# gutiKristian/VolumeRendering

Hardware: AMD Instinct MI355X
Metric: Gsamples/s (higher is better)
Workload: dtype f32

## Files before the change

include/vr.h:

```cpp
#ifndef VR_H_
#define VR_H_

#include <stdint.h>
#include <stddef.h>

#ifdef __cplusplus
extern "C" {
#endif

#define VR_ABI_VERSION 1

typedef enum vr_status {
    VR_OK = 0,
    VR_ERR_INVALID_ARG = -1,
    VR_ERR_HIP = -2,
    VR_ERR_NOT_READY = -3,
    VR_ERR_UNSUPPORTED = -4,
    VR_ERR_OOM = -5
} vr_status;

typedef enum vr_variant {
    VR_VARIANT_BASIC = 0,
    VR_VARIANT_LIGHT = 1,
    VR_VARIANT_VOLUME_MASK = 2,
    VR_VARIANT_THREE_FILES = 3,
    VR_VARIANT_MULTI_CTRT = 4,
    VR_VARIANT_TF_CALIB = 5,
    VR_VARIANT_ILLUSTRATIVE = 6,
    VR_VARIANT_LIGHT_INSHADER = 7,
    VR_VARIANT_MIP = 8,
    VR_VARIANT_MINIP = 9,
    VR_VARIANT_AVERAGE = 10,
    VR_VARIANT_ISO = 11,
    VR_VARIANT_COUNT = 12
} vr_variant;

#define VR_MAX_VOLUMES 3
#define VR_MAX_TFS 2


typedef struct vr_uniforms {
    float model[16];
    float view[16];
    float proj[16];
    float view_inv[16];
    float proj_inv[16];
    float camera_pos[3];
    int32_t fragment_mode;
    int32_t steps_count;
    float step_size;
    float clip_x[2];
    float clip_y[2];
    float clip_z[2];
    int32_t toggles[4];
    float light_pos[4];
    float light_ambient[4];
    float light_diffuse[4];
} vr_uniforms;

typedef struct vr_ctx vr_ctx;


int vr_create(vr_ctx** out, uint32_t width, uint32_t height, int device_id);

int vr_resize(vr_ctx* ctx, uint32_t width, uint32_t height);

void vr_destroy(vr_ctx* ctx);

const char* vr_last_error(const vr_ctx* ctx);

int vr_abi_version(void);


int vr_volume_upload(vr_ctx* ctx, int slot, const float* vec4_voxels, uint16_t nx, uint16_t ny, uint16_t nz);

int vr_volume_upload_device(vr_ctx* ctx, int slot, const void* d_vec4_voxels, uint16_t nx, uint16_t ny, uint16_t nz);

int vr_volume_upload_raw16(vr_ctx* ctx, int slot, const uint16_t* raw, uint16_t nx, uint16_t ny, uint16_t nz);
int vr_volume_upload_raw32(vr_ctx* ctx, int slot, const uint32_t* raw, uint16_t nx, uint16_t ny, uint16_t nz);
int vr_volume_normalize(vr_ctx* ctx, int slot, int normalization_value, int* used_value);
int vr_volume_precompute_gradient(vr_ctx* ctx, int slot, int norm_to_zero_one);
int vr_volume_download(vr_ctx* ctx, int slot, float* vec4_voxels);

int vr_tf_upload(vr_ctx* ctx, int slot, const float* opacity, const float* color_rgba, uint32_t resolution);

int vr_tf_upload_opacity(vr_ctx* ctx, int slot, const float* opacity, uint32_t resolution);
int vr_tf_upload_color(vr_ctx* ctx, int slot, const float* color_rgba, uint32_t resolution);

int vr_tf_upload_opacity_async(vr_ctx* ctx, int slot, const float* opacity, uint32_t resolution, void* stream);
int vr_tf_upload_color_async(vr_ctx* ctx, int slot, const float* color_rgba, uint32_t resolution, void* stream);

int vr_set_uniforms(vr_ctx* ctx, const vr_uniforms* u);


int vr_render(vr_ctx* ctx, int variant);

int vr_render_tiles(vr_ctx* ctx, int variant, int rank, int world);
int vr_tile_count(const vr_ctx* ctx, int rank, int world);

int vr_render_async(vr_ctx* ctx, int variant, void* d_frame, void* stream);

void* vr_stream(vr_ctx* ctx, int index);

int vr_hint_frames_in_flight(vr_ctx* ctx, int frames);
int vr_render_tiles_async(vr_ctx* ctx, int variant, int rank, int world, void* d_tiles, void* stream);

int vr_unpack_tiles_async(vr_ctx* ctx, const void* d_gathered, int world, void* d_frame, void* stream);

int vr_render_batch_async(vr_ctx* ctx, int variant, int n_frames, const vr_uniforms* uniforms, void* const* d_frames, void* stream);
int vr_render_tiles_batch_async(vr_ctx* ctx, int variant, int rank, int world, int n_frames, const vr_uniforms* uniforms,
                                void* const* d_tiles, void* stream);

int vr_unpack_tiles_strided_async(vr_ctx* ctx, const void* d_gathered, int world, int rank_stride_tiles, void* d_frame, void* stream);

int vr_download(vr_ctx* ctx, float* frag_rgba, uint8_t* present_bgra8, uint64_t* composited_samples);

int vr_present_async(vr_ctx* ctx, const void* d_frame, void* d_bgra8, void* stream);

int vr_present_tiles_async(vr_ctx* ctx, const void* d_gathered, int world, int rank_stride_tiles, void* d_bgra8, void* stream);

int vr_present_packed_async(vr_ctx* ctx, const void* d_tiles_rgba, int n_tiles, void* d_tiles_bgra8, void* stream);
int vr_unpack_tiles_bgra8_async(vr_ctx* ctx, const void* d_gathered_bgra8, int world, int rank_stride_tiles, void* d_bgra8, void* stream);

int vr_download_tiles(vr_ctx* ctx, float* tiles_rgba, uint64_t* composited_samples);


int vr_last_timing(vr_ctx* ctx, float* kernel_ms, float* total_ms);

int vr_kernel_times(vr_ctx* ctx, float* out_ms, int capacity);

#define VR_TIMING_RECORDS 0
#define VR_TIMING_EVENTS 1
int vr_set_kernel_timing(vr_ctx* ctx, int mode);
int vr_reset_kernel_times(vr_ctx* ctx);

int vr_viewport(const vr_ctx* ctx, uint32_t* width, uint32_t* height, int* device_id);

void* vr_frame_device_ptr(vr_ctx* ctx);

int vr_last_covered_pixels(vr_ctx* ctx, uint64_t* covered);

int vr_last_counters(vr_ctx* ctx, uint64_t out[3]);

int vr_last_block_trace(vr_ctx* ctx, uint64_t* out, int capacity);

int vr_set_kernel_flavour(vr_ctx* ctx, int flavour);

int vr_kernel_choice(vr_ctx* ctx, int flavours[6], float ms_per_launch[6], int* chosen);

#define VR_ARITH_SEPARATE 0
#define VR_ARITH_FUSED 1
int vr_set_arithmetic(vr_ctx* ctx, int mode);

int vr_set_iso_value(vr_ctx* ctx, float iso);

int vr_set_shadows(vr_ctx* ctx, int grid_divisor, float opacity_scale);

int vr_shadow_volume(vr_ctx* ctx, float* out, size_t capacity, int dims[3]);

int vr_set_volume_layout(vr_ctx* ctx, int mode);
int vr_volume_layout(vr_ctx* ctx, int slot, int* flags);

int vr_last_kernel_flavour(vr_ctx* ctx);

int vr_skip_field(vr_ctx* ctx, int variant, uint8_t* dist, size_t capacity, int dims[3], int box[6], uint64_t* active);

int64_t vr_unbounded_box_launches(vr_ctx* ctx);

#ifdef __cplusplus
}
#endif
#endif
```

volumerendering_amd/build.py:

```python
from __future__ import annotations

import os
import shutil
import subprocess

HERE = os.path.dirname(os.path.abspath(__file__))
CSRC = os.path.join(HERE, "csrc")
HIPCC = shutil.which("hipcc") or "/opt/rocm/bin/hipcc"

HIP_ARCH = os.environ.get("VR_HIP_ARCH", "gfx950:xnack-")
HIP_FLAGS = ["-O3", "--offload-arch=" + HIP_ARCH, "-ffp-contract=off", "-fno-fast-math", "-fPIC", "-shared",
             "-std=c++17", "-Wall", "-Wno-unused-function"]
HOST_FLAGS = ["-O2", "-std=c++20", "-fPIC", "-shared", "-ffp-contract=off", "-fno-fast-math", "-Wall"]


def _newer(target: str, sources: list[str]) -> bool:
    if not os.path.exists(target):
        return True
    t = os.path.getmtime(target)
    return any(os.path.getmtime(s) > t for s in sources)


def _sources(d: str, exts: tuple[str, ...]) -> list[str]:
    out = []
    for dp, _, fs in os.walk(d):
        out += [os.path.join(dp, f) for f in fs if f.endswith(exts)]
    return sorted(out)


def build_hip(force: bool = False) -> str:
    target = os.path.join(HERE, "libvr_hip.so")
    hdrs = [os.path.join(CSRC, f) for f in ("vr_kernels.h", "vr_dp.h", "vr_pw.h", "vr_p2.h", "vr_lt.h", "vr_proj.h", "vr_iso.h", "vr_shadow.h", "vr_device.h", "vr_launch.h")]
    hdrs.append(os.path.join(os.path.dirname(HERE), "include", "vr.h"))
    flags = [f for f in HIP_FLAGS if f != "-shared"] + os.environ.get("VR_EXTRA_HIPCC_FLAGS", "").split()
    stamp = os.path.join(CSRC, ".build_flags")
    want = " ".join(flags)
    if not os.path.exists(stamp) or open(stamp).read() != want:
        force = True
    objs, procs = [], []
    for name in ("vr_api", "vr_fused"):
        src, obj = os.path.join(CSRC, name + ".hip"), os.path.join(CSRC, name + ".o")
        objs.append(obj)
        if force or _newer(obj, hdrs + [src]):
            procs.append((name, subprocess.Popen([HIPCC, *flags, "-c", "-o", obj, src])))
    for name, pr in procs:
        if pr.wait() != 0:
            raise subprocess.CalledProcessError(pr.returncode, f"hipcc {name}.hip")
    if procs or force or _newer(target, objs):
        subprocess.run([HIPCC, "--offload-arch=" + HIP_ARCH, "-fPIC", "-shared", "-o", target, *objs], check=True)
    with open(stamp, "w") as fh:
        fh.write(want)
    return target


def build_host(force: bool = False) -> str | None:
    hostdir = os.path.join(CSRC, "host")
    cpps = _sources(hostdir, (".cpp",))
    if not cpps:
        return None
    target = os.path.join(HERE, "libvr_host.so")
    deps = _sources(hostdir, (".cpp", ".h")) + [os.path.join(os.path.dirname(HERE), "include", "vr.h")]
    if force or _newer(target, deps):
        subprocess.run(["g++", *HOST_FLAGS, "-I", os.path.join(os.path.dirname(HERE), "include"), "-o", target, *cpps,
                        "-L", HERE, "-lvr_hip", "-Wl,-rpath,$ORIGIN"], check=True)
    return target


def build_mgpu(force: bool = False) -> str:
    target = os.path.join(HERE, "libvr_mgpu.so")
    src = os.path.join(CSRC, "mgpu", "vr_mgpu.cpp")
    inc = os.path.join(os.path.dirname(HERE), "include")
    deps = [src, os.path.join(inc, "vr_mgpu.h"), os.path.join(inc, "vr.h")]
    rocm = os.environ.get("ROCM_PATH", "/opt/rocm")
    if force or _newer(target, deps):
        subprocess.run(["g++", "-O2", "-std=c++17", "-fPIC", "-shared", "-Wall", "-D__HIP_PLATFORM_AMD__", "-I", inc,
                        "-I", os.path.join(rocm, "include"), "-o", target, src, "-L", HERE, "-lvr_hip",
                        "-L", os.path.join(rocm, "lib"), "-lamdhip64", "-lrccl",
                        "-Wl,-rpath,$ORIGIN", "-Wl,-rpath," + os.path.join(rocm, "lib")], check=True)
    return target


def build_all(force: bool = False):
    build_hip(force)
    build_host(force)
    build_mgpu(force)
```

volumerendering_amd/capi.py:

```python
from __future__ import annotations

import ctypes as C
import os

import numpy as np

_HERE = os.path.dirname(os.path.abspath(__file__))
LIB_PATH = os.path.join(_HERE, "libvr_hip.so")

VR_OK = 0
VR_ERR_INVALID_ARG = -1
VR_ERR_HIP = -2
VR_ERR_NOT_READY = -3
VR_ERR_UNSUPPORTED = -4
VR_ERR_OOM = -5

BASIC, LIGHT, VOLUME_MASK, THREE_FILES, MULTI_CTRT, TF_CALIB, ILLUSTRATIVE, LIGHT_INSHADER = range(8)
MIP, MINIP, AVERAGE = 8, 9, 10
ISO = 11
VARIANT_NAMES = ["BASIC", "LIGHT", "VOLUME_MASK", "THREE_FILES", "MULTI_CTRT", "TF_CALIB", "ILLUSTRATIVE", "LIGHT_INSHADER",
                 "MIP", "MINIP", "AVERAGE", "ISO"]
TILE = 64
ARITH_SEPARATE, ARITH_FUSED = 0, 1

ABI_SYMBOLS = [
    "vr_create", "vr_resize", "vr_destroy", "vr_last_error", "vr_abi_version", "vr_volume_upload",
    "vr_volume_upload_device", "vr_volume_upload_raw16", "vr_volume_upload_raw32", "vr_volume_normalize",
    "vr_volume_precompute_gradient", "vr_volume_download", "vr_tf_upload", "vr_tf_upload_opacity", "vr_tf_upload_color", "vr_set_uniforms", "vr_render", "vr_render_tiles", "vr_tile_count",
    "vr_render_async", "vr_render_tiles_async", "vr_unpack_tiles_async", "vr_download", "vr_download_tiles",
    "vr_render_batch_async", "vr_render_tiles_batch_async", "vr_unpack_tiles_strided_async",
    "vr_last_timing", "vr_kernel_times", "vr_reset_kernel_times", "vr_frame_device_ptr", "vr_last_covered_pixels", "vr_last_counters", "vr_set_kernel_flavour", "vr_last_block_trace", "vr_last_kernel_flavour",
    "vr_set_volume_layout", "vr_volume_layout", "vr_viewport", "vr_set_arithmetic", "vr_present_async", "vr_stream", "vr_hint_frames_in_flight",
    "vr_set_kernel_timing", "vr_present_tiles_async", "vr_kernel_choice",
    "vr_present_packed_async", "vr_unpack_tiles_bgra8_async",
    "vr_tf_upload_opacity_async", "vr_tf_upload_color_async", "vr_skip_field", "vr_unbounded_box_launches",
    "vr_set_iso_value", "vr_set_shadows", "vr_shadow_volume",
]


class Uniforms(C.Structure):
    _fields_ = [
        ("model", C.c_float * 16), ("view", C.c_float * 16), ("proj", C.c_float * 16),
        ("view_inv", C.c_float * 16), ("proj_inv", C.c_float * 16),
        ("camera_pos", C.c_float * 3),
        ("fragment_mode", C.c_int32), ("steps_count", C.c_int32), ("step_size", C.c_float),
        ("clip_x", C.c_float * 2), ("clip_y", C.c_float * 2), ("clip_z", C.c_float * 2),
        ("toggles", C.c_int32 * 4),
        ("light_pos", C.c_float * 4), ("light_ambient", C.c_float * 4), ("light_diffuse", C.c_float * 4),
    ]


class VrError(RuntimeError):
    def __init__(self, code: int, msg: str):
        super().__init__(f"vr error {code}: {msg}")
        self.code = code


_lib = None


def load() -> C.CDLL:
    global _lib
    if _lib is not None:
        return _lib
    if not os.path.exists(LIB_PATH):
        raise RuntimeError(
            f"{LIB_PATH} is missing: build it with `python -c 'import __graft_entry__ as g; g.build()'` "
            "(hipcc --offload-arch=gfx950). There is no CPU fallback.")
    lib = C.CDLL(LIB_PATH)
    vp, i32, u32, u16 = C.c_void_p, C.c_int, C.c_uint32, C.c_uint16
    fp = C.POINTER(C.c_float)
    lib.vr_create.argtypes = [C.POINTER(vp), u32, u32, i32]
    lib.vr_resize.argtypes = [vp, u32, u32]
    lib.vr_destroy.argtypes = [vp]
    lib.vr_destroy.restype = None
    lib.vr_last_error.argtypes = [vp]
    lib.vr_last_error.restype = C.c_char_p
    lib.vr_abi_version.argtypes = []
    lib.vr_volume_upload.argtypes = [vp, i32, vp, u16, u16, u16]
    lib.vr_volume_upload_device.argtypes = [vp, i32, vp, u16, u16, u16]
    lib.vr_volume_upload_raw16.argtypes = [vp, i32, vp, u16, u16, u16]
    lib.vr_volume_upload_raw32.argtypes = [vp, i32, vp, u16, u16, u16]
    lib.vr_volume_normalize.argtypes = [vp, i32, i32, C.POINTER(C.c_int)]
    lib.vr_volume_precompute_gradient.argtypes = [vp, i32, i32]
    lib.vr_volume_download.argtypes = [vp, i32, vp]
    lib.vr_tf_upload.argtypes = [vp, i32, vp, vp, u32]
    lib.vr_tf_upload_opacity.argtypes = [vp, i32, vp, u32]
    lib.vr_tf_upload_color.argtypes = [vp, i32, vp, u32]
    lib.vr_tf_upload_opacity_async.argtypes = [vp, i32, vp, u32, vp]
    lib.vr_tf_upload_color_async.argtypes = [vp, i32, vp, u32, vp]
    lib.vr_skip_field.argtypes = [vp, i32, vp, C.c_size_t, C.POINTER(C.c_int * 3), C.POINTER(C.c_int * 6), C.POINTER(C.c_uint64)]
    lib.vr_unbounded_box_launches.argtypes = [vp]
    lib.vr_unbounded_box_launches.restype = C.c_int64
    lib.vr_set_uniforms.argtypes = [vp, C.POINTER(Uniforms)]
    lib.vr_render.argtypes = [vp, i32]
    lib.vr_render_tiles.argtypes = [vp, i32, i32, i32]
    lib.vr_tile_count.argtypes = [vp, i32, i32]
    lib.vr_render_async.argtypes = [vp, i32, vp, vp]
    lib.vr_render_tiles_async.argtypes = [vp, i32, i32, i32, vp, vp]
    lib.vr_unpack_tiles_async.argtypes = [vp, vp, i32, vp, vp]
    lib.vr_render_batch_async.argtypes = [vp, i32, i32, C.POINTER(Uniforms), C.POINTER(vp), vp]
    lib.vr_render_tiles_batch_async.argtypes = [vp, i32, i32, i32, i32, C.POINTER(Uniforms), C.POINTER(vp), vp]
    lib.vr_unpack_tiles_strided_async.argtypes = [vp, vp, i32, i32, vp, vp]
    lib.vr_download.argtypes = [vp, vp, vp, C.POINTER(C.c_uint64)]
    lib.vr_download_tiles.argtypes = [vp, vp, C.POINTER(C.c_uint64)]
    lib.vr_last_timing.argtypes = [vp, fp, fp]
    lib.vr_kernel_times.argtypes = [vp, vp, i32]
    lib.vr_reset_kernel_times.argtypes = [vp]
    lib.vr_set_kernel_timing.argtypes = [vp, i32]
    lib.vr_frame_device_ptr.argtypes = [vp]
    lib.vr_frame_device_ptr.restype = vp
    lib.vr_last_covered_pixels.argtypes = [vp, C.POINTER(C.c_uint64)]
    lib.vr_last_counters.argtypes = [vp, C.POINTER(C.c_uint64 * 3)]
    lib.vr_last_block_trace.argtypes = [vp, C.c_void_p, C.c_int]
    lib.vr_set_kernel_flavour.argtypes = [vp, i32]
    lib.vr_last_kernel_flavour.argtypes = [vp]
    lib.vr_set_volume_layout.argtypes = [vp, i32]
    lib.vr_set_arithmetic.argtypes = [vp, i32]
    lib.vr_set_iso_value.argtypes = [vp, C.c_float]
    lib.vr_set_shadows.argtypes = [vp, i32, C.c_float]
    lib.vr_shadow_volume.argtypes = [vp, vp, C.c_size_t, C.POINTER(C.c_int * 3)]
    lib.vr_present_async.argtypes = [vp, vp, vp, vp]
    lib.vr_present_tiles_async.argtypes = [vp, vp, C.c_int, C.c_int, vp, vp]
    lib.vr_hint_frames_in_flight.argtypes = [vp, i32]
    lib.vr_present_packed_async.argtypes = [vp, vp, C.c_int, vp, vp]
    lib.vr_unpack_tiles_bgra8_async.argtypes = [vp, vp, C.c_int, C.c_int, vp, vp]
    lib.vr_kernel_choice.argtypes = [vp, C.POINTER(C.c_int), C.POINTER(C.c_float), C.POINTER(C.c_int)]
    lib.vr_stream.argtypes = [vp, i32]
    lib.vr_stream.restype = vp
    lib.vr_volume_layout.argtypes = [vp, i32, C.POINTER(C.c_int)]
    _lib = lib
    return lib


def _f32(a) -> np.ndarray:
    a = np.ascontiguousarray(a, dtype=np.float32)
    return a


class Context:

    def __init__(self, width: int, height: int, device_id: int = 0):
        self.lib = load()
        self.h = C.c_void_p()
        rc = self.lib.vr_create(C.byref(self.h), width, height, device_id)
        if rc != VR_OK:
            raise VrError(rc, (self.lib.vr_last_error(None) or b"").decode())
        self.width, self.height = width, height

    def _chk(self, rc: int):
        if rc < 0:
            raise VrError(rc, (self.lib.vr_last_error(self.h) or b"").decode())
        return rc

    def close(self):
        if self.h:
            self.lib.vr_destroy(self.h)
            self.h = C.c_void_p()

    def __enter__(self):
        return self

    def __exit__(self, *a):
        self.close()

    def __del__(self):
        try:
            self.close()
        except Exception:
            pass

    def resize(self, w: int, h: int):
        self._chk(self.lib.vr_resize(self.h, w, h))
        self.width, self.height = w, h

    def volume_upload(self, slot: int, vec4: np.ndarray):
        v = _f32(vec4)
        assert v.ndim == 4 and v.shape[3] == 4, v.shape
        nz, ny, nx = v.shape[:3]
        self._chk(self.lib.vr_volume_upload(self.h, slot, v.ctypes.data, nx, ny, nz))

    def volume_upload_device(self, slot: int, dptr: int, nx: int, ny: int, nz: int):
        self._chk(self.lib.vr_volume_upload_device(self.h, slot, dptr, nx, ny, nz))

    def volume_upload_raw(self, slot: int, raw: np.ndarray):
        raw = np.ascontiguousarray(raw)
        nz, ny, nx = raw.shape
        fn = {np.dtype(np.uint16): self.lib.vr_volume_upload_raw16, np.dtype(np.uint32): self.lib.vr_volume_upload_raw32}[raw.dtype]
        self._chk(fn(self.h, slot, raw.ctypes.data, nx, ny, nz))
        self._shapes = getattr(self, "_shapes", {})
        self._shapes[slot] = (nz, ny, nx)

    def volume_normalize(self, slot: int, value: int = 0) -> int:
        used = C.c_int(0)
        self._chk(self.lib.vr_volume_normalize(self.h, slot, value, C.byref(used)))
        return int(used.value)

    def volume_precompute_gradient(self, slot: int, norm_to_zero_one: bool = False):
        self._chk(self.lib.vr_volume_precompute_gradient(self.h, slot, int(norm_to_zero_one)))

    def volume_download(self, slot: int, shape) -> np.ndarray:
        out = np.empty(tuple(shape) + (4,), dtype=np.float32)
        self._chk(self.lib.vr_volume_download(self.h, slot, out.ctypes.data))
        return out

    def tf_upload(self, slot: int, opacity: np.ndarray, color_rgba: np.ndarray):
        o, c = _f32(opacity), _f32(color_rgba)
        if c.size == 4 * o.size:
            self._chk(self.lib.vr_tf_upload(self.h, slot, o.ctypes.data, c.ctypes.data, o.size))
        else:
            self._chk(self.lib.vr_tf_upload_opacity(self.h, slot, o.ctypes.data, o.size))
            self._chk(self.lib.vr_tf_upload_color(self.h, slot, c.ctypes.data, c.size // 4))

    def tf_upload_async(self, slot: int, opacity: np.ndarray | None = None, color: np.ndarray | None = None, stream: int = 0):
        if opacity is not None:
            o = _f32(opacity)
            self._chk(self.lib.vr_tf_upload_opacity_async(self.h, slot, o.ctypes.data, o.size, stream))
        if color is not None:
            c = _f32(color)
            self._chk(self.lib.vr_tf_upload_color_async(self.h, slot, c.ctypes.data, c.size // 4, stream))

    def skip_field(self, variant: int):
        dims, box, active = (C.c_int * 3)(), (C.c_int * 6)(), C.c_uint64(0)
        n = self._chk(self.lib.vr_skip_field(self.h, variant, None, 0, C.byref(dims), C.byref(box), C.byref(active)))
        out = np.zeros(n, dtype=np.uint8)
        self._chk(self.lib.vr_skip_field(self.h, variant, out.ctypes.data, n, C.byref(dims), C.byref(box), C.byref(active)))
        return out.reshape(dims[2], dims[1], dims[0]), tuple(int(x) for x in box), int(active.value)

    def unbounded_box_launches(self) -> int:
        return self._chk(self.lib.vr_unbounded_box_launches(self.h))

    def set_uniforms(self, u: Uniforms):
        self._chk(self.lib.vr_set_uniforms(self.h, C.byref(u)))

    def render(self, variant: int):
        self._chk(self.lib.vr_render(self.h, variant))

    def render_tiles(self, variant: int, rank: int, world: int):
        self._chk(self.lib.vr_render_tiles(self.h, variant, rank, world))

    def tile_count(self, rank: int, world: int) -> int:
        return self._chk(self.lib.vr_tile_count(self.h, rank, world))

    def render_async(self, variant: int, d_frame: int = 0, stream: int = 0):
        self._chk(self.lib.vr_render_async(self.h, variant, d_frame, stream))

    def render_tiles_async(self, variant: int, rank: int, world: int, d_tiles: int, stream: int = 0):
        self._chk(self.lib.vr_render_tiles_async(self.h, variant, rank, world, d_tiles, stream))

    def unpack_tiles_async(self, d_gathered: int, world: int, d_frame: int = 0, stream: int = 0):
        self._chk(self.lib.vr_unpack_tiles_async(self.h, d_gathered, world, d_frame, stream))

    def unpack_tiles_strided_async(self, d_gathered: int, world: int, rank_stride_tiles: int, d_frame: int = 0, stream: int = 0):
        self._chk(self.lib.vr_unpack_tiles_strided_async(self.h, d_gathered, world, rank_stride_tiles, d_frame, stream))

    @staticmethod
    def _batch_args(uniforms, buffers):
        n = len(uniforms)
        assert n == len(buffers)
        return n, (Uniforms * n)(*uniforms), (C.c_void_p * n)(*buffers)

    def render_batch_async(self, variant: int, uniforms, d_frames, stream: int = 0):
        n, us, bufs = self._batch_args(uniforms, d_frames)
        self._chk(self.lib.vr_render_batch_async(self.h, variant, n, us, bufs, stream))

    def render_tiles_batch_async(self, variant: int, rank: int, world: int, uniforms, d_tiles, stream: int = 0):
        n, us, bufs = self._batch_args(uniforms, d_tiles)
        self._chk(self.lib.vr_render_tiles_batch_async(self.h, variant, rank, world, n, us, bufs, stream))

    def download(self, present: bool = False):
        frag = np.empty((self.height, self.width, 4), dtype=np.float32)
        bgra = np.empty((self.height, self.width, 4), dtype=np.uint8) if present else None
        n = C.c_uint64(0)
        self._chk(self.lib.vr_download(self.h, frag.ctypes.data, bgra.ctypes.data if present else None, C.byref(n)))
        return frag, bgra, int(n.value)

    def samples(self) -> int:
        n = C.c_uint64(0)
        self._chk(self.lib.vr_download(self.h, None, None, C.byref(n)))
        return int(n.value)

    def download_tiles(self, n_tiles: int):
        tiles = np.empty((n_tiles, TILE, TILE, 4), dtype=np.float32)
        n = C.c_uint64(0)
        self._chk(self.lib.vr_download_tiles(self.h, tiles.ctypes.data, C.byref(n)))
        return tiles, int(n.value)

    def last_timing(self):
        k, t = C.c_float(0), C.c_float(0)
        self._chk(self.lib.vr_last_timing(self.h, C.byref(k), C.byref(t)))
        return float(k.value), float(t.value)

    def kernel_times(self, capacity: int = 256) -> np.ndarray:
        out = np.zeros(capacity, dtype=np.float32)
        n = self._chk(self.lib.vr_kernel_times(self.h, out.ctypes.data, capacity))
        return out[:n].copy()

    def reset_kernel_times(self):
        self._chk(self.lib.vr_reset_kernel_times(self.h))

    def set_kernel_timing(self, events: bool):
        self._chk(self.lib.vr_set_kernel_timing(self.h, 1 if events else 0))

    def covered_pixels(self) -> int:
        n = C.c_uint64(0)
        self._chk(self.lib.vr_last_covered_pixels(self.h, C.byref(n)))
        return int(n.value)

    def counters(self):
        out = (C.c_uint64 * 3)()
        self._chk(self.lib.vr_last_counters(self.h, C.byref(out)))
        return int(out[0]), int(out[1]), int(out[2])

    def block_trace(self):
        n = self.lib.vr_last_block_trace(self.h, None, 0)
        if n < 0:
            self._chk(n)
        out = np.zeros((max(n, 0), 6), dtype=np.uint64)
        if n > 0:
            self._chk(min(0, self.lib.vr_last_block_trace(self.h, out.ctypes.data_as(C.c_void_p), n)))
        return out

    def frame_device_ptr(self) -> int:
        return int(self.lib.vr_frame_device_ptr(self.h) or 0)

    def last_kernel_flavour(self) -> int:
        return self._chk(self.lib.vr_last_kernel_flavour(self.h))

    def kernel_choice(self):
        fl, ms, ch = (C.c_int * 6)(), (C.c_float * 6)(), C.c_int(-1)
        n = self.lib.vr_kernel_choice(self.h, fl, ms, C.byref(ch))
        if n < 0:
            self._chk(n)
        return [int(x) for x in fl[:n]], [float(x) for x in ms[:n]], int(ch.value)

    def hint_frames_in_flight(self, frames: int):
        self._chk(self.lib.vr_hint_frames_in_flight(self.h, frames))

    def stream(self, index: int) -> int:
        s = self.lib.vr_stream(self.h, index)
        if not s:
            raise VrError(VR_ERR_HIP, "vr_stream: no stream available")
        return int(s)

    def present_async(self, d_bgra8: int, d_frame: int = 0, stream: int = 0):
        self._chk(self.lib.vr_present_async(self.h, d_frame, d_bgra8, stream))

    def present_tiles_async(self, d_gathered: int, world: int, d_bgra8: int, rank_stride_tiles: int = 0, stream: int = 0):
        self._chk(self.lib.vr_present_tiles_async(self.h, d_gathered, world, rank_stride_tiles, d_bgra8, stream))

    def set_arithmetic(self, mode: int):
        self._chk(self.lib.vr_set_arithmetic(self.h, mode))

    def set_iso_value(self, iso: float):
        self._chk(self.lib.vr_set_iso_value(self.h, iso))

    def set_shadows(self, divisor: int, scale: float = 1.0):
        self._chk(self.lib.vr_set_shadows(self.h, divisor, scale))

    def shadow_volume(self):
        dims = (C.c_int * 3)()
        n = self._chk(self.lib.vr_shadow_volume(self.h, None, 0, C.byref(dims)))
        out = np.zeros(n, dtype=np.float32)
        self._chk(self.lib.vr_shadow_volume(self.h, out.ctypes.data, n, C.byref(dims)))
        return out.reshape(dims[2], dims[1], dims[0]), (int(dims[0]), int(dims[1]), int(dims[2]))

    def set_volume_layout(self, mode: int):
        self._chk(self.lib.vr_set_volume_layout(self.h, mode))

    def volume_layout(self, slot: int) -> int:
        f = C.c_int(0)
        self._chk(self.lib.vr_volume_layout(self.h, slot, C.byref(f)))
        return int(f.value)

    def set_kernel_flavour(self, flavour: int):
        self._chk(self.lib.vr_set_kernel_flavour(self.h, flavour))
```

volumerendering_amd/csrc/vr_api.hip:

```cpp
#include "../../include/vr.h"
#include "vr_launch.h"

namespace vrf {
void launch_march(const vr::LaunchDesc& L, hipStream_t s, const vr::MarchBatch& B);
void launch_shadow_build(const vr::MarchParams& P, float* out, float sigma, bool skip, bool off32, hipStream_t s);
}

#include <cmath>
#include <cstdio>
#include <cstdlib>
#include <cstring>
#include <new>
#include <string>
#include <vector>

using namespace vr;

namespace {

thread_local std::string g_create_error;

struct Timing {
    hipEvent_t ev_begin = nullptr, ev_k0 = nullptr, ev_k1 = nullptr, ev_end = nullptr;
    bool valid = false;
};

constexpr int kRing = 256;
struct KernelRing {
    hipEvent_t k0[kRing] = {}, k1[kRing] = {};
    long long head = 0;
};

}

constexpr int kInFlight = 8;
constexpr int kStreams = 4;
constexpr int kOrderRing = 16;
constexpr int kGen = 4;
constexpr int kStage = 8;
constexpr int kEditSeen = 8;
constexpr int kShadowRing = 4;

struct GenBuf {
    void* d = nullptr;
    size_t cap = 0;
    long long reader[kInFlight];
    GenBuf() { written(); }
    void written()
    {
        for (auto& r : reader) r = -1;
    }
};

struct vr_ctx {
    int device = 0;
    uint32_t W = 0, H = 0;
    hipStream_t stream = nullptr;
    DevVolume vol[VR_MAX_VOLUMES] = {};
    size_t vol_bytes[VR_MAX_VOLUMES] = {};
    float2* vol_bricks[VR_MAX_VOLUMES] = {};
    float* vol_dens[VR_MAX_VOLUMES] = {};
    size_t vol_dens_cap[VR_MAX_VOLUMES] = {};
    float4* vol_bricked[VR_MAX_VOLUMES] = {};
    float* vol_bdens[VR_MAX_VOLUMES] = {};
    size_t vol_bricked_cap[VR_MAX_VOLUMES] = {};
    bool vol_grad_derived[VR_MAX_VOLUMES] = {};
    int arith = VR_ARITH_SEPARATE;
    int layout_mode = 0;
    float2* merged_bricks = nullptr;
    bool merged_stale = true;
    unsigned char* brick_dist = nullptr;
    GenBuf field[kGen];
    int field_cur = 0;
    unsigned char* dist_tmp = nullptr;
    size_t tmp_cap = 0;
    int dist_bn[3] = {0, 0, 0};
    const void* dist_records = nullptr;
    unsigned long long dist_epoch = ~0ull;
    int dist_z = -2, dist_res = 0, dist_rgb = -1;
    unsigned long long brick_epoch = 0;
    int tf_zero_prefix[VR_MAX_TFS] = {-1, -1};
    bool tf_color_finite[VR_MAX_TFS] = {false, false};
    bool tf_opacity_finite[VR_MAX_TFS] = {false, false};
    DevTF tf[VR_MAX_TFS] = {};
    GenBuf tf_buf[VR_MAX_TFS][2][kGen];
    int tf_cur[VR_MAX_TFS][2] = {};
    hipEvent_t edit_ev = nullptr;
    hipStream_t edit_stream = nullptr;
    unsigned long long edit_gen = 0, drained_gen = 0;
    struct EditSeen {
        hipStream_t s = nullptr;
        unsigned long long gen = 0;
    } edit_seen[kEditSeen];
    int seen_next = 0;
    struct Stage {
        void* h = nullptr;
        size_t cap = 0;
        hipEvent_t done = nullptr;
        bool used = false;
    } stage[kStage];
    unsigned stage_next = 0;
    std::vector<void*> retired_dev, retired_host;
    SkipSummary* h_skip = nullptr;
    SkipSumDev* d_skip_sum = nullptr;
    unsigned long long skip_gen = 0;
    bool skip_pending = false;
    int skip_box[6] = {0x7fffffff, 0x7fffffff, 0x7fffffff, -1, -1, -1};
    unsigned long long skip_active = 0;
    long long unbounded_launches = 0;
    vr_uniforms u = {};
    bool have_uniforms = false;
    float4* d_frame = nullptr;
    float4* d_tiles = nullptr;
    size_t tiles_cap = 0;
    int last_tiles = 0;
    uint32_t* d_present = nullptr;
    unsigned long long* d_counters = nullptr;
    unsigned long long* d_block_counts[kInFlight] = {};
    size_t block_counts_cap[kInFlight] = {};
    hipEvent_t slot_done[kInFlight] = {};
    bool slot_used[kInFlight] = {};
    unsigned* d_pw_heads = nullptr;
    bool pw_heads_dirty[kInFlight] = {};
    struct OrderSlot {
        unsigned* buf = nullptr;
        size_t cap = 0;
        hipStream_t stream = nullptr;
        hipEvent_t sorted = nullptr;
        unsigned long long key = 0, seq = 0;
        unsigned long long scene_key = 0;
        bool valid = false;
    } order_ring[kOrderRing];
    unsigned long long* h_span = nullptr;
    bool ring_events[kRing] = {};
    unsigned long long* h_end = nullptr;
    unsigned* h_chain = nullptr;
    struct Tune {
        unsigned long long key = 0;
        unsigned long long shape = 0;
        int n = 0, cand[6] = {};
        int cur = 0, issued = 0;
        int per = 3, settle = 4;
        long long launch[6][16] = {};
        int choice = -1;
        unsigned chain_ref = 0;
        float cost[6] = {};
        unsigned long long used = 0;
    } tune[8];
    unsigned long long tune_clock = 0;
    unsigned long long tf_epoch = 0;
    int tune_mode = 1;
    int frames_in_flight = 1;
    unsigned long long order_seq = 0;
    hipStream_t flight[kStreams] = {};
    int n_flight = 0;
    hipStream_t order_stream = nullptr;
    int cnt_buf = 0;
    bool cnt_pending = false;
    int cnt_blocks = 0;
    bool event_timing = false;
    size_t cnt_offset = 0;
    unsigned long long* h_counters = nullptr;
    Timing tm;
    KernelRing ring;
    int flavour = 0;
    int n_cus = 256;
    int default_flavour = 0;
    int last_flavour = 0;
    unsigned p2_window = 0;
    double active_fraction = 1.0;
    float abox[6] = {-3.0e38f, -3.0e38f, -3.0e38f, 3.0e38f, 3.0e38f, 3.0e38f};
    float2* proj_rec = nullptr;
    size_t proj_rec_cap = 0;
    float2* proj_range = nullptr;
    unsigned long long proj_epoch = ~0ull;
    hipEvent_t proj_ev = nullptr;
    hipStream_t proj_stream = nullptr;
    bool proj_pending = false;
    hipStream_t proj_seen[kEditSeen] = {};
    int proj_seen_next = 0;
    bool last_proj = false;
    float iso = 0.5f;
    int shadow_div = 0;
    float shadow_sigma = 1.0f;
    unsigned long long opacity_edits = 0;
    struct ShadowKey {
        unsigned long long epoch = 0, opacity = 0;
        uint32_t light[3] = {}, box[6] = {}, sigma = 0;
        int div = 0, arith = 0;
        bool operator==(const ShadowKey& o) const
        {
            return epoch == o.epoch && opacity == o.opacity && std::memcmp(light, o.light, sizeof light) == 0 &&
                   std::memcmp(box, o.box, sizeof box) == 0 && sigma == o.sigma && div == o.div && arith == o.arith;
        }
    };
    struct ShadowVol {
        GenBuf buf;
        ShadowKey key;
        bool valid = false;
        hipEvent_t built = nullptr;
        hipStream_t stream = nullptr;
        bool pending = false;
        hipStream_t seen[kEditSeen] = {};
        int seen_next = 0;
        unsigned long long used = 0;
    } shadow[kShadowRing];
    unsigned long long shadow_clock = 0;
    int shadow_cur = -1;
    std::string err;
};

namespace {

bool removed_flavour(int f) { return f == 2 || f == 3 || f == 4 || f == 5 || f == 9 || f == 14; }

int fail(vr_ctx* c, int code, const std::string& msg)
{
    if (c) c->err = msg;
    else g_create_error = msg;
    return code;
}

#define VR_HIP(c, call)                                                                               \
    do {                                                                                              \
        hipError_t e__ = (call);                                                                      \
        if (e__ != hipSuccess)                                                                        \
            return fail((c), e__ == hipErrorOutOfMemory ? VR_ERR_OOM : VR_ERR_HIP,                    \
                        std::string(#call) + " (vr_api.hip:" + std::to_string(__LINE__) + "): " + hipGetErrorString(e__));                          \
    } while (0)

int refresh_bricks(vr_ctx* c, int slot);

int tiles_x_of(const vr_ctx* c) { return (int)((c->W + kTile - 1) / kTile); }
int tiles_y_of(const vr_ctx* c) { return (int)((c->H + kTile - 1) / kTile); }

int tile_count(const vr_ctx* c, int rank, int world)
{
    int total = tiles_x_of(c) * tiles_y_of(c);
    if (rank >= total) return 0;
    return (total - rank + world - 1) / world;
}

bool is_identity(const float* m)
{
    for (int i = 0; i < 16; ++i)
        if (m[i] != ((i % 5 == 0) ? 1.0f : 0.0f)) return false;
    return true;
}

bool is_projection(int variant) { return variant == VR_VARIANT_MIP || variant == VR_VARIANT_MINIP || variant == VR_VARIANT_AVERAGE; }

void variant_needs(int variant, int* nvol, int* ntf)
{
    switch (variant) {
    case VR_VARIANT_BASIC:
    case VR_VARIANT_LIGHT:
    case VR_VARIANT_LIGHT_INSHADER:
    case VR_VARIANT_MIP:
    case VR_VARIANT_MINIP:
    case VR_VARIANT_AVERAGE:
    case VR_VARIANT_ISO: *nvol = 1; *ntf = 1; break;
    case VR_VARIANT_VOLUME_MASK: *nvol = 3; *ntf = 2; break;
    case VR_VARIANT_THREE_FILES: *nvol = 2; *ntf = 2; break;
    case VR_VARIANT_MULTI_CTRT: *nvol = 2; *ntf = 2; break;
    case VR_VARIANT_ILLUSTRATIVE: *nvol = 2; *ntf = 2; break;
    default: *nvol = 2; *ntf = 1; break;
    }
}

int alloc_frame(vr_ctx* c)
{
    VR_HIP(c, hipSetDevice(c->device));
    if (c->d_frame) (void)hipFree(c->d_frame);
    if (c->d_present) (void)hipFree(c->d_present);
    c->d_frame = nullptr;
    c->d_present = nullptr;
    size_t n = (size_t)c->W * c->H;
    VR_HIP(c, hipMalloc(&c->d_frame, n * sizeof(float4)));
    VR_HIP(c, hipMalloc(&c->d_present, n * sizeof(uint32_t)));
    VR_HIP(c, hipMemsetAsync(c->d_frame, 0, n * sizeof(float4), c->stream));
    return VR_OK;
}

bool invert4(const float* m, double* o)
{
    double a[16], inv[16];
    for (int i = 0; i < 16; ++i) a[i] = m[i];
    inv[0] = a[5] * a[10] * a[15] - a[5] * a[11] * a[14] - a[9] * a[6] * a[15] + a[9] * a[7] * a[14] + a[13] * a[6] * a[11] - a[13] * a[7] * a[10];
// ... 202 lines not shown
           ((unsigned long long)c->W << 40) ^ ((unsigned long long)c->H << 24);
}

bool tf0_fits_lds(const vr_ctx* c) { return c->tf[0].res_o == c->tf[0].res_c && c->tf[0].res_o + 2 <= 8192; }

int check_render_args(vr_ctx* c, int variant, int rank, int world, int n_frames, const vr_uniforms* batch_u, void* const* batch_out,
                      int* nvol, bool* off32)
{
    if (variant < 0 || variant >= VR_VARIANT_COUNT) return fail(c, VR_ERR_INVALID_ARG, "vr_render: bad variant");
    if (world < 1 || rank < 0 || rank >= world) return fail(c, VR_ERR_INVALID_ARG, "vr_render: bad rank/world");
    if (n_frames < 1 || n_frames > kBatchMax) return fail(c, VR_ERR_INVALID_ARG, "vr_render: 1 .. 4 frames per launch");
    if (batch_u) {
        if (!batch_out) return fail(c, VR_ERR_INVALID_ARG, "vr_render: a batch needs its output buffers");
        for (int f = 0; f < n_frames; ++f) {
            if (!batch_out[f]) return fail(c, VR_ERR_INVALID_ARG, "vr_render: output buffer " + std::to_string(f) + " of the batch is NULL");
            if (batch_u[f].steps_count < 0) return fail(c, VR_ERR_INVALID_ARG, "vr_render: negative steps_count");
            if (!is_identity(batch_u[f].model))
                return fail(c, VR_ERR_UNSUPPORTED, "vr_render: model matrix must be the identity (App/src/Application.cpp:489-492)");
        }
    } else {
        if (n_frames != 1) return fail(c, VR_ERR_INVALID_ARG, "vr_render: several frames per launch need their uniforms");
        if (!c->have_uniforms) return fail(c, VR_ERR_NOT_READY, "vr_render: vr_set_uniforms has not been called");
    }
    int ntf;
    variant_needs(variant, nvol, &ntf);
    *off32 = true;
    for (int i = 0; i < *nvol; ++i) {
        if (!c->vol[i].data) return fail(c, VR_ERR_NOT_READY, "vr_render: volume slot " + std::to_string(i) + " is empty");
        if (c->vol_bytes[i] > 0xFFFFFFFFull) *off32 = false;
    }
    for (int i = 0; i < ntf; ++i)
        if (!c->tf[i].opacity || !c->tf[i].color)
            return fail(c, VR_ERR_NOT_READY, "vr_render: TF slot " + std::to_string(i) + " is empty");
    if ((batch_u ? batch_u[0] : c->u).steps_count < 0) return fail(c, VR_ERR_INVALID_ARG, "vr_render: negative steps_count");
    return VR_OK;
}

void fill_launch_params(const vr_ctx* c, MarchParams& P, const vr_uniforms& u0, int rank, int world, bool packed)
{
    std::memset(&P, 0, sizeof P);
    P.W = (int)c->W;
    P.H = (int)c->H;
    fill_frame_params(P, u0);
    for (int i = 0; i < VR_MAX_VOLUMES; ++i) {
        P.vol[i] = c->vol[i];
        const bool plane = c->layout_mode != 1 && c->vol_dens[i] && c->vol[i].data;
        P.vol[i].dens = plane ? c->vol_dens[i] : nullptr;
        P.vol[i].a_base = plane ? reinterpret_cast<const char*>(c->vol_dens[i]) : reinterpret_cast<const char*>(c->vol[i].data) + 12;
        P.vol[i].a_shift = plane ? 2 : 4;
        P.vol[i].bricked = 0;
        P.vol[i].brick_row = P.vol[i].brick_slab = 0;
        const size_t lin_bytes = c->vol_bytes[i];
        P.vol[i].data_bytes = lin_bytes > 0xFFFFFFFFull ? 0xFFFFFFFFu : (unsigned)lin_bytes;
    }
    for (int i = 0; i < VR_MAX_TFS; ++i) P.tf[i] = c->tf[i];
    P.rank = rank;
    P.world = world;
    P.tiles_x = tiles_x_of(c);
    P.tiles_y = tiles_y_of(c);
    P.n_tiles = tile_count(c, rank, world);
    P.packed = packed ? 1 : 0;
    P.n_blocks = P.n_tiles * kBlocksPerTile;
    P.iso = c->iso;
}

void use_bricked_copies(const vr_ctx* c, MarchParams& P)
{
    for (int i = 0; i < VR_MAX_VOLUMES; ++i) {
        if (!c->vol[i].data || !c->vol_bricked[i] || !c->vol_bdens[i]) continue;
        const BrickedGrid g = bricked_grid(c->vol[i]);
        if (g.slots > 0xFFFFFFFFull) continue;
        P.vol[i].data = c->vol_bricked[i];
        P.vol[i].a_base = reinterpret_cast<const char*>(c->vol_bdens[i]);
        P.vol[i].a_shift = 2;
        P.vol[i].bricked = 1;
        P.vol[i].brick_row = g.nbx * kVbN;
        P.vol[i].brick_slab = g.nbx * g.nby * kVbN;
        P.vol[i].data_bytes = g.slots * 16 > 0xFFFFFFFFull ? 0xFFFFFFFFu : (unsigned)(g.slots * 16);
    }
}

struct Eligibility {
    bool p2_ok;
    unsigned p2_lds;
    bool lut_ok;
    unsigned lut_lds;
    bool can_skip;
    bool whole_frame;
    unsigned chain_known;
};

unsigned last_chain(const vr_ctx* c, unsigned long long skey)
{
    unsigned chain = 0;
    if (!c->h_chain) return chain;
    unsigned long long best_seq = 0;
    for (int i = 0; i < kOrderRing; ++i) {
        const unsigned v = *(volatile unsigned*)&c->h_chain[i];
        if (v != 0 && c->order_ring[i].scene_key == skey && c->order_ring[i].seq + 1 > best_seq) {
            best_seq = c->order_ring[i].seq + 1;
            chain = v;
        }
    }
    return chain;
}

Eligibility eligibility(const vr_ctx* c, int requested, int variant, int n_frames, int rank, int world, bool packed, const vr_uniforms* batch_u)
{
    Eligibility E = {};
    const int sv = variant == VR_VARIANT_VOLUME_MASK ? 2 : 0;
    E.p2_ok = (variant == VR_VARIANT_LIGHT || variant == VR_VARIANT_BASIC || variant == VR_VARIANT_VOLUME_MASK) && tf0_fits_lds(c) &&
              c->layout_mode == 0 && c->vol_bricked[sv] && c->vol_bdens[sv];
    if (E.p2_ok) {
        const DevVolume& v = c->vol[sv];
        const BrickedGrid g = bricked_grid(v);
        const size_t slab = (size_t)g.nbx * g.nby * kVbN, window = variant == VR_VARIANT_BASIC ? 0x3fffffffull : 0x0fffffffull;
        const size_t lds = (size_t)(c->tf[0].res_o + 2) * 16 + ((size_t)v.nx + v.ny + v.nz + 3) * 8;
        E.p2_ok = g.slots <= 0xFFFFFFFFull && slab < (1u << 24) && (c->p2_window ? c->p2_window / slab >= 3 : window / slab >= 4) && lds <= 160u * 1024u;
        E.p2_lds = (unsigned)lds;
    }
    E.lut_ok = (variant == VR_VARIANT_LIGHT || variant == VR_VARIANT_BASIC || variant == VR_VARIANT_LIGHT_INSHADER) && c->layout_mode == 0 &&
               c->vol_bricked[0] && c->vol_bdens[0];
    if (E.lut_ok) {
        E.lut_lds = (unsigned)(((size_t)c->vol[0].nx + c->vol[0].ny + c->vol[0].nz + 6) * 4);
        E.lut_ok = bricked_grid(c->vol[0]).slots <= 0xFFFFFFFFull && E.lut_lds <= 32u * 1024u;
    }
    E.can_skip = (variant == VR_VARIANT_BASIC || variant == VR_VARIANT_LIGHT || variant == VR_VARIANT_THREE_FILES ||
                  variant == VR_VARIANT_VOLUME_MASK || variant == VR_VARIANT_LIGHT_INSHADER) &&
                 requested != 1 && c->vol_bricks[sv] && c->tf_zero_prefix[0] >= 0 && c->tf_color_finite[0];
    for (int f = 0; f < n_frames; ++f) E.can_skip = E.can_skip && all_finite(batch_u ? batch_u[f].light_pos : c->u.light_pos, 12);
    E.can_skip = E.can_skip && skip_bricks(c->vol[sv].nx) * (long long)skip_bricks(c->vol[sv].ny) < (1 << 23);
    if (variant == VR_VARIANT_THREE_FILES) E.can_skip = E.can_skip && c->tf_color_finite[1] && c->tf_opacity_finite[1];
    if (variant == VR_VARIANT_VOLUME_MASK)
        E.can_skip = E.can_skip && c->vol_bricks[0] && c->vol[0].nx == c->vol[2].nx && c->vol[0].ny == c->vol[2].ny &&
                     c->vol[0].nz == c->vol[2].nz;
    E.whole_frame = rays_per_lane(c, rank, world, 1) >= 4.5;
    E.chain_known = requested == 0 ? last_chain(c, scene_key(c, variant, rank, world, packed)) : 0;
    return E;
}

void drained(vr_ctx* c)
{
    for (void* p : c->retired_dev) (void)hipFree(p);
    for (void* p : c->retired_host) (void)hipHostFree(p);
    c->retired_dev.clear();
    c->retired_host.clear();
    c->drained_gen = c->edit_gen;
    c->proj_pending = false;
    for (auto& e : c->shadow) e.pending = false;
}

int reuse_wait(vr_ctx* c, hipStream_t s, const GenBuf& b)
{
    for (int k = 0; k < kInFlight; ++k)
        if (b.reader[k] >= 0 && (unsigned long long)b.reader[k] + kInFlight >= c->order_seq)
            VR_HIP(c, hipStreamWaitEvent(s, c->slot_done[k], 0));
    return VR_OK;
}

int wait_for_edits(vr_ctx* c, hipStream_t s)
{
    if (c->edit_gen <= c->drained_gen) return VR_OK;
    vr_ctx::EditSeen* e = nullptr;
    for (auto& x : c->edit_seen)
        if (x.s == s) e = &x;
    if (e && e->gen >= c->edit_gen) return VR_OK;
    if (s != c->edit_stream) VR_HIP(c, hipStreamWaitEvent(s, c->edit_ev, 0));
    if (!e) e = &c->edit_seen[c->seen_next++ % kEditSeen];
    e->s = s;
    e->gen = c->edit_gen;
    return VR_OK;
}

void mark_reads(vr_ctx* c, const MarchParams& P)
{
    for (int i = 0; i < VR_MAX_TFS; ++i)
        for (int k = 0; k < 2; ++k) {
            GenBuf& b = c->tf_buf[i][k][c->tf_cur[i][k]];
            if (b.d) b.reader[c->order_seq % kInFlight] = (long long)c->order_seq;
        }
    if (P.brick_dist) c->field[c->field_cur].reader[c->order_seq % kInFlight] = (long long)c->order_seq;
    if (c->shadow_cur >= 0) c->shadow[c->shadow_cur].buf.reader[c->order_seq % kInFlight] = (long long)c->order_seq;
}

int build_field(vr_ctx* c, hipStream_t s, const float2* rec, const int bn[3], int use_rgb, int zero_prefix, int res_o, unsigned char* field,
                int slot, unsigned long long gen)
{
    const int nb = bn[0] * bn[1] * bn[2];
    hipLaunchKernelGGL(brick_active_kernel, dim3((unsigned)((nb + 255) / 256)), dim3(256), 0, s, rec, field, nb, use_rgb, zero_prefix, res_o);
    const long long waves = (long long)((bn[0] + 63) >> 6) * bn[1] * bn[2];
    hipLaunchKernelGGL(brick_dist_x_kernel, dim3((unsigned)((waves + 3) / 4)), dim3(256), 0, s, field, bn[0], bn[1] * bn[2]);
    const unsigned tx = (unsigned)((bn[0] + kDistCols - 1) / kDistCols);
    hipLaunchKernelGGL((brick_dist_axis_kernel<false>), dim3(tx, (unsigned)((bn[1] + kDistRows - 1) / kDistRows), (unsigned)bn[2]), dim3(256),
                       0, s, field, c->dist_tmp, bn[0], bn[1], (size_t)bn[0], (size_t)bn[0] * bn[1], (SkipSumDev*)nullptr,
                       (SkipSummary*)nullptr, 0ull);
    hipLaunchKernelGGL((brick_dist_axis_kernel<true>), dim3(tx, (unsigned)((bn[2] + kDistRows - 1) / kDistRows), (unsigned)bn[1]), dim3(256),
                       0, s, c->dist_tmp, field, bn[0], bn[2], (size_t)bn[0] * bn[1], (size_t)bn[0], c->d_skip_sum + slot, c->h_skip + slot, gen);
    VR_HIP(c, hipGetLastError());
    return VR_OK;
}

void adopt_skip(vr_ctx* c, const float bs[3])
{
    if (!c->skip_pending) return;
    const volatile SkipSummary& h = c->h_skip[c->field_cur];
    if (h.gen != c->skip_gen) return;
    __atomic_thread_fence(__ATOMIC_ACQUIRE);
    const long long nb = (long long)c->dist_bn[0] * c->dist_bn[1] * c->dist_bn[2];
    c->skip_active = h.count;
    c->active_fraction = nb > 0 ? (double)h.count / (double)nb : 1.0;
    for (int a = 0; a < 6; ++a) c->skip_box[a] = h.box[a];
    for (int a = 0; a < 3; ++a) {
        if (c->skip_box[3 + a] < 0) {
            c->abox[a] = 3.0e38f;
            c->abox[3 + a] = -3.0e38f;
        } else {
            c->abox[a] = (float)(((double)c->skip_box[a] - 1.0 + (double)kBrickHalf) / (double)bs[a]);
            c->abox[3 + a] = (float)(((double)c->skip_box[3 + a] + 2.0 + (double)kBrickHalf) / (double)bs[a]);
        }
    }
    c->skip_pending = false;
}

int grow(vr_ctx* c, void** d, size_t* cap, size_t bytes, bool drain)
{
    if (bytes <= *cap) return VR_OK;
    if (*d) {
        if (drain) (void)hipFree(*d);
        else c->retired_dev.push_back(*d);
    }
    *d = nullptr;
    *cap = 0;
    VR_HIP(c, hipMalloc(d, bytes));
    *cap = bytes;
    return VR_OK;
}

int prepare_skip(vr_ctx* c, int variant, hipStream_t s, MarchParams& P)
{
    const int sv = variant == VR_VARIANT_VOLUME_MASK ? 2 : 0;
    P.skip_vol = sv;
    P.bnx = skip_bricks(c->vol[sv].nx);
    P.bny = skip_bricks(c->vol[sv].ny);
    P.bnz = skip_bricks(c->vol[sv].nz);
    P.bsx = (float)c->vol[sv].nx * kBrickInv;
    P.bsy = (float)c->vol[sv].ny * kBrickInv;
    P.bsz = (float)c->vol[sv].nz * kBrickInv;
    P.tf_zero_prefix = c->tf_zero_prefix[0];
    P.bricks = c->vol_bricks[sv];
    P.use_rgb = 0;
    const int nb = P.bnx * P.bny * P.bnz;
    if (variant == VR_VARIANT_VOLUME_MASK) {
        if (c->merged_stale || !c->merged_bricks) {
            if (c->merged_bricks) (void)hipFree(c->merged_bricks);
            c->merged_bricks = nullptr;
            VR_HIP(c, hipMalloc(&c->merged_bricks, (size_t)nb * sizeof(float2)));
            hipLaunchKernelGGL(merge_bricks_kernel, dim3((unsigned)((nb + 255) / 256)), dim3(256), 0, s, c->vol_bricks[2],
                               c->vol_bricks[0], c->merged_bricks, nb);
            VR_HIP(c, hipGetLastError());
            c->merged_stale = false;
        }
        P.bricks = c->merged_bricks;
        P.use_rgb = 1;
    }
    const float bs[3] = {P.bsx, P.bsy, P.bsz};
    if (c->dist_records != (const void*)P.bricks || c->dist_epoch != c->brick_epoch || c->dist_z != P.tf_zero_prefix ||
        c->dist_res != c->tf[0].res_o || c->dist_rgb != P.use_rgb || !c->brick_dist) {
        VR_HIP(c, hipDeviceSynchronize());
        drained(c);
        GenBuf& g = c->field[c->field_cur];
        c->brick_dist = nullptr;
        if (const int rc = grow(c, &g.d, &g.cap, (size_t)nb, true)) return rc;
        if (const int rc = grow(c, (void**)&c->dist_tmp, &c->tmp_cap, (size_t)nb, true)) return rc;
        const int bn[3] = {P.bnx, P.bny, P.bnz};
        if (const int rc = build_field(c, s, P.bricks, bn, P.use_rgb, P.tf_zero_prefix, c->tf[0].res_o, (unsigned char*)g.d, c->field_cur,
                                       ++c->skip_gen))
            return rc;
        VR_HIP(c, hipStreamSynchronize(s));
        g.written();
        c->brick_dist = (unsigned char*)g.d;
        c->skip_pending = true;
        for (int a = 0; a < 3; ++a) c->dist_bn[a] = bn[a];
        c->dist_records = (const void*)P.bricks;
        c->dist_epoch = c->brick_epoch;
        c->dist_z = P.tf_zero_prefix;
        c->dist_res = c->tf[0].res_o;
        c->dist_rgb = P.use_rgb;
    }
    adopt_skip(c, bs);
    P.brick_dist = c->brick_dist;
    if (c->skip_pending) {
        const float unbounded[6] = {-3.0e38f, -3.0e38f, -3.0e38f, 3.0e38f, 3.0e38f, 3.0e38f};
        for (int a = 0; a < 6; ++a) P.abox[a] = unbounded[a];
    } else {
        for (int a = 0; a < 6; ++a) P.abox[a] = c->abox[a];
    }
    return VR_OK;
}

const float2* prepare_proj(vr_ctx* c, hipStream_t s, MarchParams& P)
{
    const DevVolume& v = c->vol[0];
    P.skip_vol = 0;
    P.bnx = skip_bricks(v.nx);
    P.bny = skip_bricks(v.ny);
    P.bnz = skip_bricks(v.nz);
    P.bsx = (float)v.nx * kBrickInv;
    P.bsy = (float)v.ny * kBrickInv;
    P.bsz = (float)v.nz * kBrickInv;
    const size_t nb = (size_t)P.bnx * P.bny * P.bnz;
    if (c->proj_epoch != c->brick_epoch || !c->proj_rec || !c->proj_range) {
        if (grow(c, (void**)&c->proj_rec, &c->proj_rec_cap, nb * sizeof(float2), false)) return nullptr;
        if (!c->proj_range && hipMalloc(&c->proj_range, sizeof(float2)) != hipSuccess) {
            c->proj_range = nullptr;
            fail(c, VR_ERR_OOM, "vr_render: no memory for the projection's volume range");
            return nullptr;
        }
        if (!c->proj_ev && hipEventCreateWithFlags(&c->proj_ev, hipEventDisableTiming) != hipSuccess) {
            c->proj_ev = nullptr;
            fail(c, VR_ERR_HIP, "vr_render: hipEventCreateWithFlags failed");
            return nullptr;
        }
        hipLaunchKernelGGL(brick_range_kernel, dim3((unsigned)nb), dim3(64), 0, s, v.data, v.nx, v.ny, v.nz, P.bnx, P.bny, c->proj_rec);
        hipLaunchKernelGGL(range_reduce_kernel, dim3(1), dim3(1024), 0, s, (const float2*)c->proj_rec, (int)nb, c->proj_range);
        if (hipGetLastError() != hipSuccess || hipEventRecord(c->proj_ev, s) != hipSuccess) {
            fail(c, VR_ERR_HIP, "vr_render: the projection's brick ranges could not be enqueued");
            return nullptr;
        }
        c->proj_epoch = c->brick_epoch;
        c->proj_stream = s;
        c->proj_pending = true;
        for (auto& x : c->proj_seen) x = nullptr;
    } else if (c->proj_pending && s != c->proj_stream) {
        bool seen = false;
        for (auto x : c->proj_seen) seen = seen || x == s;
// ... 24 lines not shown
}

size_t shadow_grid(const vr_ctx* c, int g[3])
{
    const int n[3] = {c->vol[0].nx, c->vol[0].ny, c->vol[0].nz};
    for (int a = 0; a < 3; ++a) g[a] = (n[a] + c->shadow_div - 1) / c->shadow_div;
    return (size_t)g[0] * g[1] * g[2];
}

int prepare_shadow(vr_ctx* c, hipStream_t s, MarchParams& P, const vr_ctx::ShadowKey& key, bool skip, bool off32)
{
    int g[3];
    const size_t texels = shadow_grid(c, g);
    int e = -1;
    for (int i = 0; i < kShadowRing; ++i)
        if (c->shadow[i].valid && c->shadow[i].key == key) e = i;
    bool build = e < 0;
    if (build) {
        e = 0;
        for (int i = 1; i < kShadowRing; ++i)
            if (c->shadow[i].used < c->shadow[e].used) e = i;
    }
    vr_ctx::ShadowVol& v = c->shadow[e];
    if (build) {
        v.valid = false;
        const bool fresh = texels * sizeof(float) > v.buf.cap;
        if (const int rc = grow(c, &v.buf.d, &v.buf.cap, texels * sizeof(float), false)) return rc;
        if (!v.built) VR_HIP(c, hipEventCreateWithFlags(&v.built, hipEventDisableTiming));
        if (!fresh) {
            if (const int rc = reuse_wait(c, s, v.buf)) return rc;
            if (v.pending && v.stream != s) VR_HIP(c, hipStreamWaitEvent(s, v.built, 0));
        }
    }
    DevVolume& lv = P.vol[1];
    lv = DevVolume{};
    lv.data = nullptr;
    lv.dens = (const float*)v.buf.d;
    lv.a_base = (const char*)v.buf.d;
    lv.a_shift = 2;
    lv.nx = g[0];
    lv.ny = g[1];
    lv.nz = g[2];
    lv.bricked = 0;
    lv.lut = 0;
    lv.data_bytes = (unsigned)(texels * sizeof(float));
    if (build) {
        if (c->arith == VR_ARITH_FUSED) vrf::launch_shadow_build(P, (float*)v.buf.d, c->shadow_sigma, skip, off32, s);
        else vr::launch_shadow_build(P, (float*)v.buf.d, c->shadow_sigma, skip, off32, s);
        VR_HIP(c, hipGetLastError());
        VR_HIP(c, hipEventRecord(v.built, s));
        v.buf.written();
        v.key = key;
        v.valid = true;
        v.stream = s;
        v.pending = true;
        for (auto& x : v.seen) x = nullptr;
    } else if (v.pending && s != v.stream) {
        bool seen = false;
        for (auto x : v.seen) seen = seen || x == s;
        if (!seen) {
            VR_HIP(c, hipStreamWaitEvent(s, v.built, 0));
            v.seen[v.seen_next++ % kEditSeen] = s;
        }
    }
    v.used = ++c->shadow_clock;
    c->shadow_cur = e;
    return VR_OK;
}

int choose_flavour(vr_ctx* c, int fl, int variant, int n_frames, int rank, int world, bool packed, const Eligibility& E)
{
    if (is_projection(variant)) return fl == 1 ? 20 : 19;
    if (variant == VR_VARIANT_ISO) return fl == 1 ? 22 : 21;
    if (variant == VR_VARIANT_LIGHT && c->shadow_div != 0) return fl == 1 ? 24 : 23;
    const bool auto_choice = fl == 0;
    const double rays = rays_per_lane(c, rank, world, c->frames_in_flight * n_frames);
    const bool short_chains = E.chain_known != 0 && E.chain_known - 1 < 128;
    if (auto_choice) {
        fl = (rays >= 4.5 || (short_chains && rays >= 1.2)) ? 6 : (rays >= 2.0 ? 11 : 10);
    }
    if ((fl == 12 || fl == 13) && n_frames != 1) fl = 6;
    if ((fl == 16 || fl == 17) && !E.p2_ok) fl = n_frames != 1 ? 6 : (fl == 16 ? 13 : 12);
    if (fl == 18 && !E.lut_ok) fl = 6;
    if (fl == 16 && variant == VR_VARIANT_VOLUME_MASK) fl = 17;
    if (fl == 15 && (n_frames != 1 || variant != VR_VARIANT_LIGHT)) fl = 6;
    if (variant == VR_VARIANT_ILLUSTRATIVE && (fl == 7 || fl == 8 || fl == 10 || fl == 11)) fl = 6;
    if (variant == VR_VARIANT_LIGHT_INSHADER && fl != 1 && fl != 12 && fl != 13 && fl != 18) fl = 6;
    if ((fl == 16 || fl == 17) && variant == VR_VARIANT_VOLUME_MASK && !E.can_skip)
        fl = n_frames != 1 ? 6 : 12;
    if (!auto_choice) return fl;

    const bool p2_variant = variant == VR_VARIANT_LIGHT || variant == VR_VARIANT_BASIC || (variant == VR_VARIANT_VOLUME_MASK && E.can_skip);
    const bool nothing_to_skip = !E.can_skip || c->active_fraction >= 0.9;
    if (fl == 6 && E.whole_frame && E.p2_ok && p2_variant) {
        if (nothing_to_skip && variant != VR_VARIANT_VOLUME_MASK) fl = 16;
        else if (!short_chains) fl = 17;
    }
    if (!c->tune_mode) return fl;
    int cand[6], n = 0;
    auto add = [&](int f) {
        for (int i = 0; i < n; ++i)
            if (cand[i] == f) return;
        if (n < 6) cand[n++] = f;
    };
    add(fl);
    if (E.p2_ok && p2_variant) add((nothing_to_skip && variant != VR_VARIANT_VOLUME_MASK) || !E.can_skip ? 16 : 17);
    add(6);
    if (E.lut_ok && E.lut_lds <= 8u * 1024u) add(18);
    const bool dp_variant = variant != VR_VARIANT_ILLUSTRATIVE && variant != VR_VARIANT_LIGHT_INSHADER;
    if (!E.whole_frame && dp_variant) add(rays >= 2.0 ? 11 : 10);
    else if (n_frames == 1 && (variant == VR_VARIANT_LIGHT || variant == VR_VARIANT_BASIC)) add(12);
    const unsigned long long shape = 0x9E3779B97F4A7C15ull * (((unsigned long long)variant << 56) ^ ((unsigned long long)world << 48) ^ ((unsigned long long)rank << 40) ^
                                                             ((unsigned long long)c->W << 24) ^ ((unsigned long long)c->H << 8) ^ (packed ? 0x80ull : 0ull) ^
                                                             ((unsigned long long)n_frames << 4) ^ (unsigned long long)c->frames_in_flight) | 1ull;
    const unsigned long long key = (shape ^ (c->brick_epoch * 0xD6E8FEB86659FD93ull) ^ (c->tf_epoch << 20) ^ ((unsigned long long)c->arith << 1) ^
                                    ((unsigned long long)c->layout_mode << 2)) | 1ull;
    const bool measurable = c->h_span && c->h_end && !c->event_timing;
    return tune_pick(c, key, shape, cand, n, E.chain_known, measurable);
}

struct KernelForm {
    LaunchDesc::Family family;
    int lanes;
    bool pipe;
    bool p2_skip;
    bool lut;
    unsigned pw_threads;
};

KernelForm kernel_form(int fl, int variant)
{
    using D = LaunchDesc;
    switch (fl) {
    case 7: return {D::kDp, 4, false, false, false, 0u};
    case 8: return {D::kDp, 2, false, false, false, 0u};
    case 10: return {D::kDp, 4, true, false, false, 0u};
    case 11: return {D::kDp, 2, true, false, false, 0u};
    case 12: return {D::kPw, 0, false, false, false, 1024u};
    case 13: return {D::kPw, 0, true, false, false, 1024u};
    case 15: return {D::kLt, 0, false, false, false, 0u};
    case 16: return {D::kP2, 0, false, false, false, 512u};
    case 17: return {D::kP2, 0, false, true, false, variant == VR_VARIANT_BASIC ? 1024u : 768u};
    case 18: return {D::kPlain, 0, false, false, true, 0u};
    case 19:
    case 20: return {D::kProj, 0, false, false, false, 0u};
    case 21:
    case 22: return {D::kIso, 0, false, false, false, 0u};
    case 23:
    case 24: return {D::kShadow, 0, false, false, false, 0u};
    default: return {D::kPlain, 0, false, false, false, 0u};
    }
}

int take_record_slot(vr_ctx* c, hipStream_t s, size_t n_records, int* cb, const vr_ctx::OrderSlot** slot_sort)
{
    const int k = (int)(c->order_seq % (unsigned long long)kInFlight);
    *cb = k;
    if (c->slot_used[k]) VR_HIP(c, hipEventSynchronize(c->slot_done[k]));
    *slot_sort = nullptr;
    if (c->order_seq >= (unsigned long long)kInFlight) {
        const vr_ctx::OrderSlot& po = c->order_ring[(c->order_seq - kInFlight) % kOrderRing];
        if (po.valid && po.seq + kInFlight == c->order_seq) *slot_sort = &po;
    }
    if (n_records > c->block_counts_cap[k]) {
        if (*slot_sort) VR_HIP(c, hipStreamWaitEvent(s, (*slot_sort)->sorted, 0));
        *slot_sort = nullptr;
        if (c->d_block_counts[k]) (void)hipFree(c->d_block_counts[k]);
        c->d_block_counts[k] = nullptr;
        c->block_counts_cap[k] = 0;
        VR_HIP(c, hipMalloc(&c->d_block_counts[k], n_records * kBlockRecord * sizeof(unsigned long long)));
        VR_HIP(c, hipMemsetAsync(c->d_block_counts[k], 0, n_records * kBlockRecord * sizeof(unsigned long long), s));
        c->block_counts_cap[k] = n_records;
    }
    return VR_OK;
}

int wait_for_order(vr_ctx* c, hipStream_t s, bool ordered, unsigned long long okey, const vr_ctx::OrderSlot* slot_sort, const unsigned** order)
{
    *order = nullptr;
    if (ordered) {
        const vr_ctx::OrderSlot* best = nullptr;
        const unsigned long long age = (unsigned long long)(c->frames_in_flight + 2 > 3 ? c->frames_in_flight + 2 : 3);
        for (const auto& o : c->order_ring)
            if (o.valid && o.key == okey && o.seq + age + 1 >= c->order_seq && o.seq + age <= c->order_seq && (!best || o.seq > best->seq))
                best = &o;
        if (best) {
            VR_HIP(c, hipStreamWaitEvent(s, best->sorted, 0));
            if (slot_sort && best->seq >= slot_sort->seq) slot_sort = nullptr;
            *order = best->buf;
        }
    }
    if (slot_sort) VR_HIP(c, hipStreamWaitEvent(s, slot_sort->sorted, 0));
    return VR_OK;
}

int enqueue_sort(vr_ctx* c, hipStream_t s, int cb, bool ordered, unsigned long long okey, unsigned long long skey, unsigned n_blocks, int ring,
                 bool time_with_events, bool pw)
{
    vr_ctx::OrderSlot& o = c->order_ring[c->order_seq % kOrderRing];
    if (ordered) {
        o.valid = false;
        if (n_blocks > o.cap) {
            if (o.buf) (void)hipFree(o.buf);
            o.buf = nullptr;
            o.cap = 0;
            VR_HIP(c, hipMalloc(&o.buf, (size_t)n_blocks * sizeof(unsigned)));
            o.cap = n_blocks;
        }
        o.stream = s;
        o.key = okey;
        o.scene_key = skey;
        o.seq = c->order_seq;
        if (c->h_chain) c->h_chain[c->order_seq % kOrderRing] = 0;
    }
    VR_HIP(c, hipEventRecord(c->slot_done[cb], s));
    c->slot_used[cb] = true;
    if (ordered) {
        VR_HIP(c, hipStreamWaitEvent(c->order_stream, c->slot_done[cb], 0));
        hipLaunchKernelGGL(order_blocks_kernel, dim3(1), dim3(1024), 0, c->order_stream, c->d_block_counts[cb], (int)n_blocks, o.buf,
                           c->h_chain ? c->h_chain + (c->order_seq % kOrderRing) : (unsigned*)nullptr,
                           (c->h_span && !time_with_events) ? c->h_span + ring : (unsigned long long*)nullptr,
                           pw ? c->d_pw_heads + (size_t)cb * 8 * 64 : (unsigned*)nullptr,
                           (c->h_span && c->h_end && !time_with_events) ? c->h_end + ring : (unsigned long long*)nullptr);
        VR_HIP(c, hipGetLastError());
        if (pw) c->pw_heads_dirty[cb] = false;
        VR_HIP(c, hipEventRecord(o.sorted, c->order_stream));
        o.valid = true;
    }
    ++c->order_seq;
    return VR_OK;
}

const MarchBatch& fill_batch(MarchParams& P, int n_frames, const vr_uniforms* batch_u, void* const* batch_out, unsigned blocks_per_frame)
{
    static thread_local MarchBatch B;
    P.batch_n = (unsigned)n_frames;
    B.frame[0] = P;
    for (int f = 1; f < n_frames; ++f) {
        MarchParams& Pf = B.frame[f];
        Pf = P;
        fill_frame_params(Pf, batch_u[f]);
        Pf.out = (float4*)batch_out[f];
        Pf.block_counts = P.block_counts + (size_t)f * blocks_per_frame * kBlockRecord;
    }
    B.n_frames = (unsigned)n_frames;
    return B;
}

int enqueue_render(vr_ctx* c, int variant, int rank, int world, bool packed, float4* out, hipStream_t s, bool frame_events,
                   int n_frames = 1, const vr_uniforms* batch_u = nullptr, void* const* batch_out = nullptr)
{
    int nvol;
    bool off32;
    if (const int rc = check_render_args(c, variant, rank, world, n_frames, batch_u, batch_out, &nvol, &off32)) return rc;
    const bool shadowed = variant == VR_VARIANT_LIGHT && c->shadow_div != 0;
    vr_ctx::ShadowKey shadow_k;
    if (shadowed) {
        shadow_k = shadow_key(c, batch_u ? batch_u[0] : c->u);
        for (int f = 1; f < n_frames; ++f)
            if (!(shadow_key(c, batch_u[f]) == shadow_k))
                return fail(c, VR_ERR_UNSUPPORTED, "vr_render: the frames of a shadowed batch must share the light and the clip box");
        int g[3];
        if (shadow_grid(c, g) * sizeof(float) >= (1ull << 32))
            return fail(c, VR_ERR_UNSUPPORTED, "vr_render: the light volume would take 4 GiB or more (a larger divisor)");
    }
    c->shadow_cur = -1;
    if (batch_u) out = (float4*)batch_out[0];
    VR_HIP(c, hipSetDevice(c->device));
    (void)hipGetLastError();
    if (const int rc = wait_for_edits(c, s)) return rc;

    MarchParams P;
    fill_launch_params(c, P, batch_u ? batch_u[0] : c->u, rank, world, packed);
    const int requested = c->flavour == 0 ? c->default_flavour : c->flavour;
    const Eligibility E = eligibility(c, requested, variant, n_frames, rank, world, packed, batch_u);
    if (E.can_skip) {
        if (const int rc = prepare_skip(c, variant, s, P)) return rc;
        if (c->skip_pending) ++c->unbounded_launches;
    }
    const int fl = choose_flavour(c, requested, variant, n_frames, rank, world, packed, E);
    c->last_flavour = fl;
    const KernelForm form = kernel_form(fl, variant);
    c->last_proj = form.family == LaunchDesc::kProj || form.family == LaunchDesc::kIso || form.family == LaunchDesc::kShadow;
    const float2* vrange = nullptr;
    if (fl == 19 || fl == 21) {
        vrange = prepare_proj(c, s, P);
        if (!vrange) return VR_ERR_HIP;
    }

    if (c->layout_mode == 0) use_bricked_copies(c, P);
    if (form.lut && P.vol[0].bricked) P.vol[0].lut = 1;
    for (int i = 0; i < nvol; ++i)
        if (P.vol[i].bricked && bricked_grid(P.vol[i]).slots * 16 > 0xFFFFFFFFull) off32 = false;

    if (packed && !out) {
        size_t need = (size_t)P.n_tiles * kTile * kTile;
        if (need > c->tiles_cap) {
            if (c->d_tiles) (void)hipFree(c->d_tiles);
            c->d_tiles = nullptr;
            c->tiles_cap = 0;
            VR_HIP(c, hipMalloc(&c->d_tiles, (need ? need : 1) * sizeof(float4)));
            c->tiles_cap = need;
        }
        out = c->d_tiles;
    } else if (!out) {
        out = c->d_frame;
    }
    P.out = out;
    c->last_tiles = packed ? P.n_tiles : 0;

    if (frame_events) VR_HIP(c, hipEventRecord(c->tm.ev_begin, s));
    const bool shadow_skip = form.family == LaunchDesc::kShadow && fl == 23 && P.brick_dist != nullptr;
    if (P.n_blocks > 0) {
        if (shadowed)
            if (const int rc = prepare_shadow(c, s, P, shadow_k, shadow_skip, off32)) return rc;
        const int dp = form.family == LaunchDesc::kDp ? form.lanes : 0, wpb = dp && P.n_tiles * dp * 64 > 16384 ? 4 : 1;
        const dim3 block((unsigned)(64 * wpb));
        const dim3 grid((unsigned)(dp ? P.n_tiles * dp * 64 / wpb : (P.n_tiles + 7) / 8 * 8 * (64 / wpb)));
        if (n_frames > 1 && grid.x % 8u != 0) return fail(c, VR_ERR_INVALID_ARG, "vr_render: launch shape cannot carry several frames");
        const bool pw = form.family == LaunchDesc::kPw || form.family == LaunchDesc::kP2;
        int cb;
        const vr_ctx::OrderSlot* slot_sort;
        if (const int rc = take_record_slot(c, s, (size_t)grid.x * (size_t)n_frames, &cb, &slot_sort)) return rc;
        P.block_counts = c->d_block_counts[cb];
        c->cnt_buf = cb;
        const unsigned long long okey = ((unsigned long long)grid.x << 32) ^ ((unsigned long long)block.x << 20) ^
                                        ((unsigned long long)variant << 16) ^ ((unsigned long long)world << 8) ^ (unsigned long long)rank ^
                                        (packed ? 1ull << 63 : 0ull);
        const bool ordered = grid.x <= (unsigned)kOrderMaxBlocks && grid.x % 8u == 0;
        if (const int rc = wait_for_order(c, s, ordered, okey, slot_sort, &P.order)) return rc;

        const int ring = (int)(c->ring.head % kRing);
        if (frame_events) VR_HIP(c, hipEventRecord(c->tm.ev_k0, s));
        const bool time_with_events = !(ordered && c->h_span) || c->event_timing;
        c->ring_events[ring] = time_with_events;
        if (c->h_span) c->h_span[ring] = 0;
        if (c->h_end) c->h_end[ring] = 0;
        if (time_with_events) VR_HIP(c, hipEventRecord(c->ring.k0[ring], s));
        const MarchBatch& B = fill_batch(P, n_frames, batch_u, batch_out, grid.x);
        LaunchDesc L = {};
        L.variant = variant;
        L.family = form.family;
        L.off32 = off32;
        L.lanes = form.lanes;
        L.pipe = form.pipe;
        L.lds_bytes = P.vol[0].lut ? E.lut_lds : 0u;
        L.grid = dim3(grid.x * (unsigned)n_frames);
        L.block = block;
        L.vrange = vrange;
        L.proj_skip = vrange != nullptr || shadow_skip;
        if (pw) {
            const bool p2 = form.family == LaunchDesc::kP2;
            const unsigned per_wg = form.pw_threads / 64u, wgs = (grid.x * (unsigned)n_frames + per_wg - 1u) / per_wg;
            L.ltf = tf0_fits_lds(c);
            L.p2_skip = form.p2_skip && P.brick_dist != nullptr;
            L.p2_win = p2 && (!off32 || c->p2_window != 0);
            L.lds_bytes = p2 ? E.p2_lds : (L.ltf ? (unsigned)(c->tf[0].res_o + 2) * 16u : 0u);
            L.queue = PwQueue{c->d_pw_heads + (size_t)cb * 8 * 64, grid.x, c->p2_window};
            L.grid = dim3(wgs < (unsigned)c->n_cus ? wgs : (unsigned)c->n_cus);
            L.block = dim3(form.pw_threads);
            if (c->pw_heads_dirty[cb]) VR_HIP(c, hipMemsetAsync(L.queue.heads, 0, 8 * 64 * sizeof(unsigned), s));
            c->pw_heads_dirty[cb] = true;
        }
        if (c->arith == VR_ARITH_FUSED) vrf::launch_march(L, s, B);
        else vr::launch_march(L, s, B);
        VR_HIP(c, hipGetLastError());
        mark_reads(c, P);
        if (time_with_events) VR_HIP(c, hipEventRecord(c->ring.k1[ring], s));

        if (const int rc = enqueue_sort(c, s, cb, ordered, okey, scene_key(c, variant, rank, world, packed), grid.x, ring, time_with_events, pw))
            return rc;
        if (frame_events) VR_HIP(c, hipEventRecord(c->tm.ev_k1, s));
        ++c->ring.head;
        c->cnt_blocks = (int)grid.x;
        c->cnt_offset = (size_t)(n_frames - 1) * grid.x * kBlockRecord;
    } else {
        c->cnt_blocks = 0;
        c->cnt_offset = 0;
        if (frame_events) {
            VR_HIP(c, hipEventRecord(c->tm.ev_k0, s));
            VR_HIP(c, hipEventRecord(c->tm.ev_k1, s));
        }
    }
    c->cnt_pending = true;
    if (frame_events) VR_HIP(c, hipEventRecord(c->tm.ev_end, s));
    c->tm.valid = frame_events;
    return VR_OK;
}

int fetch_counters(vr_ctx* c)
{
    if (!c->cnt_pending) return VR_OK;
    VR_HIP(c, hipSetDevice(c->device));
    (void)hipGetLastError();
    if (c->cnt_blocks > 0) {
        VR_HIP(c, hipEventSynchronize(c->slot_done[c->cnt_buf]));
        hipLaunchKernelGGL(sum_block_counts_kernel, dim3(1), dim3(256), 0, c->stream, c->d_block_counts[c->cnt_buf] + c->cnt_offset,
                           c->cnt_blocks, c->d_counters);
        VR_HIP(c, hipGetLastError());
        VR_HIP(c, hipMemcpyAsync(c->h_counters, c->d_counters, 3 * sizeof(unsigned long long), hipMemcpyDeviceToHost,
                                 c->stream));
        VR_HIP(c, hipStreamSynchronize(c->stream));
    } else {
        c->h_counters[0] = c->h_counters[1] = c->h_counters[2] = 0;
    }
    c->cnt_pending = false;
    return VR_OK;
}

int refresh_bricks(vr_ctx* c, int slot)
{
    (void)hipGetLastError();
    const DevVolume& v = c->vol[slot];
    if (c->vol_bricks[slot]) (void)hipFree(c->vol_bricks[slot]);
    c->vol_bricks[slot] = nullptr;
    c->merged_stale = true;
    ++c->brick_epoch;
    for (auto& e : c->shadow) e.valid = false;
    const int bnx = skip_bricks(v.nx), bny = skip_bricks(v.ny), bnz = skip_bricks(v.nz);
    const size_t nbricks = (size_t)bnx * bny * bnz;
    VR_HIP(c, hipMalloc(&c->vol_bricks[slot], nbricks * sizeof(float2)));
    hipLaunchKernelGGL(brick_max_kernel, dim3((unsigned)nbricks), dim3(64), 0, c->stream, v.data, v.nx, v.ny, v.nz, bnx, bny,
                       c->vol_bricks[slot]);
    VR_HIP(c, hipGetLastError());
    const size_t n = (size_t)v.nx * v.ny * v.nz;
    c->vol_grad_derived[slot] = false;
    if (n > c->vol_dens_cap[slot]) {
        if (c->vol_dens[slot]) (void)hipFree(c->vol_dens[slot]);
        c->vol_dens[slot] = nullptr;
        c->vol_dens_cap[slot] = 0;
        VR_HIP(c, hipMalloc(&c->vol_dens[slot], n * sizeof(float)));
        c->vol_dens_cap[slot] = n;
    }
    hipLaunchKernelGGL(extract_density_kernel, dim3(4096), dim3(256), 0, c->stream, v.data, c->vol_dens[slot], n);
    VR_HIP(c, hipGetLastError());
    unsigned* d_flag = reinterpret_cast<unsigned*>(c->d_counters);
    VR_HIP(c, hipMemsetAsync(d_flag, 0, sizeof(unsigned), c->stream));
    hipLaunchKernelGGL(verify_gradient_kernel, dim3((unsigned)((v.nx + 255) / 256), (unsigned)v.ny, (unsigned)v.nz), dim3(256), 0,
                       c->stream, v.data, c->vol_dens[slot], v.nx, v.ny, v.nz, d_flag);
    VR_HIP(c, hipGetLastError());
    unsigned flag = 1;
    VR_HIP(c, hipMemcpyAsync(&flag, d_flag, sizeof flag, hipMemcpyDeviceToHost, c->stream));
    VR_HIP(c, hipStreamSynchronize(c->stream));
    c->vol_grad_derived[slot] = flag == 0;
    c->vol[slot].dens = c->vol_dens[slot];
    {
        const BrickedGrid g = bricked_grid(v);
        const size_t slots = g.slots;
        if (slots > c->vol_bricked_cap[slot]) {
            if (c->vol_bricked[slot]) (void)hipFree(c->vol_bricked[slot]);
            if (c->vol_bdens[slot]) (void)hipFree(c->vol_bdens[slot]);
            c->vol_bricked[slot] = nullptr;
            c->vol_bdens[slot] = nullptr;
            c->vol_bricked_cap[slot] = 0;
            if (hipMalloc(&c->vol_bricked[slot], slots * sizeof(float4)) != hipSuccess) c->vol_bricked[slot] = nullptr;
            if (c->vol_bricked[slot] && hipMalloc(&c->vol_bdens[slot], slots * sizeof(float)) != hipSuccess) {
                (void)hipFree(c->vol_bricked[slot]);
                c->vol_bricked[slot] = nullptr;
                c->vol_bdens[slot] = nullptr;
            }
            (void)hipGetLastError();
            c->vol_bricked_cap[slot] = c->vol_bricked[slot] ? slots : 0;
        }
        if (!c->vol_bricked[slot]) {
            VR_HIP(c, hipStreamSynchronize(c->stream));
            return VR_OK;
        }
        hipLaunchKernelGGL(rebrick_kernel, dim3(8192), dim3(256), 0, c->stream, v.data, c->vol_bricked[slot], c->vol_bdens[slot], v.nx,
                           v.ny, v.nz, g.nbx, g.nby, slots);
        VR_HIP(c, hipGetLastError());
        VR_HIP(c, hipStreamSynchronize(c->stream));
    }
    return VR_OK;
}

int check_slot(vr_ctx* c, int slot, const char* who)
{
    if (!c) return VR_ERR_INVALID_ARG;
    if (slot < 0 || slot >= VR_MAX_VOLUMES) return fail(c, VR_ERR_INVALID_ARG, std::string(who) + ": bad slot");
    if (!c->vol[slot].data) return fail(c, VR_ERR_NOT_READY, std::string(who) + ": volume slot is empty");
    VR_HIP(c, hipSetDevice(c->device));
    VR_HIP(c, hipDeviceSynchronize());
    drained(c);
    (void)hipGetLastError();
    return VR_OK;
// ... 5 lines not shown
    if (!c) return VR_ERR_INVALID_ARG;
    if (slot < 0 || slot >= VR_MAX_VOLUMES) return fail(c, VR_ERR_INVALID_ARG, "vr_volume_upload_raw: bad slot");
    if (!raw) return fail(c, VR_ERR_INVALID_ARG, "vr_volume_upload_raw: data is NULL");
    if (nx == 0 || ny == 0 || nz == 0) return fail(c, VR_ERR_INVALID_ARG, "vr_volume_upload_raw: empty volume");
    const size_t n = (size_t)nx * ny * nz;
    if (n > 0xFFFFFFFFull) return fail(c, VR_ERR_INVALID_ARG, "vr_volume_upload_raw: more than 2^32 voxels");
    VR_HIP(c, hipSetDevice(c->device));
    VR_HIP(c, hipDeviceSynchronize());
    drained(c);
    (void)hipGetLastError();
    const size_t bytes = n * sizeof(float4);
    if (c->vol[slot].data && c->vol_bytes[slot] != bytes) {
        (void)hipFree(const_cast<float4*>(c->vol[slot].data));
        c->vol[slot] = DevVolume{};
        c->vol_bytes[slot] = 0;
    }
    float4* d = const_cast<float4*>(c->vol[slot].data);
    if (!d) VR_HIP(c, hipMalloc(&d, bytes));
    T* d_raw = nullptr;
    hipError_t e = hipMalloc(&d_raw, n * sizeof(T));
    if (e == hipSuccess) e = hipMemcpyAsync(d_raw, raw, n * sizeof(T), hipMemcpyHostToDevice, c->stream);
    if (e == hipSuccess) {
        hipLaunchKernelGGL((broadcast_raw_kernel<T>), dim3(2048), dim3(256), 0, c->stream, d_raw, d, n);
        e = hipGetLastError();
    }
    if (e == hipSuccess) e = hipStreamSynchronize(c->stream);
    if (d_raw) (void)hipFree(d_raw);
    if (e != hipSuccess) {
        if (!c->vol[slot].data) (void)hipFree(d);
        return fail(c, e == hipErrorOutOfMemory ? VR_ERR_OOM : VR_ERR_HIP,
                    std::string("vr_volume_upload_raw: ") + hipGetErrorString(e));
    }
    c->vol[slot].data = d;
    c->vol[slot].nx = nx;
    c->vol[slot].ny = ny;
    c->vol[slot].nz = nz;
    c->vol_bytes[slot] = bytes;
    return refresh_bricks(c, slot);
}

}

extern "C" {

int vr_volume_upload_raw16(vr_ctx* c, int slot, const uint16_t* raw, uint16_t nx, uint16_t ny, uint16_t nz)
{
    return upload_raw(c, slot, raw, nx, ny, nz);
}
int vr_volume_upload_raw32(vr_ctx* c, int slot, const uint32_t* raw, uint16_t nx, uint16_t ny, uint16_t nz)
{
    return upload_raw(c, slot, raw, nx, ny, nz);
}

int vr_volume_normalize(vr_ctx* c, int slot, int normalization_value, int* used_value)
{
    int rc = check_slot(c, slot, "vr_volume_normalize");
    if (rc != VR_OK) return rc;
    float4* d = const_cast<float4*>(c->vol[slot].data);
    const size_t n = (size_t)c->vol[slot].nx * c->vol[slot].ny * c->vol[slot].nz;
    if (normalization_value == 0) {
        unsigned* d_max = reinterpret_cast<unsigned*>(c->d_counters);
        VR_HIP(c, hipMemsetAsync(d_max, 0, sizeof(unsigned), c->stream));
        hipLaunchKernelGGL(max_component_kernel, dim3(2048), dim3(256), 0, c->stream, d, n, 0, d_max);
        VR_HIP(c, hipGetLastError());
        unsigned bits = 0;
        VR_HIP(c, hipMemcpyAsync(&bits, d_max, sizeof bits, hipMemcpyDeviceToHost, c->stream));
        VR_HIP(c, hipStreamSynchronize(c->stream));
        float mx;
        std::memcpy(&mx, &bits, sizeof mx);
        normalization_value = (int)(size_t)mx;
    }
    if (used_value) *used_value = normalization_value;
    hipLaunchKernelGGL(normalize_kernel, dim3(2048), dim3(256), 0, c->stream, d, n, normalization_value);
    VR_HIP(c, hipGetLastError());
    return refresh_bricks(c, slot);
}

int vr_volume_precompute_gradient(vr_ctx* c, int slot, int norm_to_zero_one)
{
    int rc = check_slot(c, slot, "vr_volume_precompute_gradient");
    if (rc != VR_OK) return rc;
    float4* d = const_cast<float4*>(c->vol[slot].data);
    const DevVolume& v = c->vol[slot];
    const size_t n = (size_t)v.nx * v.ny * v.nz;
    unsigned* d_max = reinterpret_cast<unsigned*>(c->d_counters);
    VR_HIP(c, hipMemsetAsync(d_max, 0, sizeof(unsigned), c->stream));
    dim3 block(256), grid((unsigned)((v.nx + 255) / 256), (unsigned)v.ny, (unsigned)v.nz);
    hipLaunchKernelGGL(gradient_kernel, grid, block, 0, c->stream, d, v.nx, v.ny, v.nz, norm_to_zero_one ? 1 : 0, d_max);
    VR_HIP(c, hipGetLastError());
    if (norm_to_zero_one) {
        hipLaunchKernelGGL(scale_gradient_kernel, dim3(2048), dim3(256), 0, c->stream, d, n, d_max);
        VR_HIP(c, hipGetLastError());
    }
    return refresh_bricks(c, slot);
}

int vr_volume_download(vr_ctx* c, int slot, float* vec4_voxels)
{
    int rc = check_slot(c, slot, "vr_volume_download");
    if (rc != VR_OK) return rc;
    if (!vec4_voxels) return fail(c, VR_ERR_INVALID_ARG, "vr_volume_download: destination is NULL");
    VR_HIP(c, hipMemcpy(vec4_voxels, c->vol[slot].data, c->vol_bytes[slot], hipMemcpyDeviceToHost));
    return VR_OK;
}

int vr_abi_version(void) { return VR_ABI_VERSION; }

const char* vr_last_error(const vr_ctx* ctx) { return ctx ? ctx->err.c_str() : g_create_error.c_str(); }

int vr_create(vr_ctx** out, uint32_t width, uint32_t height, int device_id)
{
    if (!out) return fail(nullptr, VR_ERR_INVALID_ARG, "vr_create: out is NULL");
    *out = nullptr;
    if (width == 0 || height == 0 || width > 32768 || height > 32768)
        return fail(nullptr, VR_ERR_INVALID_ARG, "vr_create: bad viewport size");
    int ndev = 0;
    hipError_t e = hipGetDeviceCount(&ndev);
    if (e != hipSuccess || ndev <= 0)
        return fail(nullptr, VR_ERR_HIP, std::string("vr_create: no HIP device available (") +
                                             (e != hipSuccess ? hipGetErrorString(e) : "device count 0") +
                                             "); this library has no CPU fallback");
    if (device_id < 0 || device_id >= ndev) return fail(nullptr, VR_ERR_INVALID_ARG, "vr_create: bad device_id");
    vr_ctx* c = new (std::nothrow) vr_ctx();
    if (!c) return fail(nullptr, VR_ERR_OOM, "vr_create: out of host memory");
    c->device = device_id;
    c->W = width;
    c->H = height;
    auto bail = [&](int code) {
        g_create_error = c->err;
        vr_destroy(c);
        return code;
    };
    int rc;
    auto hip_ok = [&](hipError_t he, const char* what) {
        if (he == hipSuccess) return true;
        c->err = std::string(what) + ": " + hipGetErrorString(he);
        return false;
    };
    if (!hip_ok(hipSetDevice(device_id), "hipSetDevice")) return bail(VR_ERR_HIP);
    if (!hip_ok(hipStreamCreateWithFlags(&c->stream, hipStreamNonBlocking), "hipStreamCreate")) return bail(VR_ERR_HIP);
    {
        int cus = 0;
        if (hipDeviceGetAttribute(&cus, hipDeviceAttributeMultiprocessorCount, device_id) == hipSuccess && cus > 0) c->n_cus = cus;
    }
    if (const char* e = getenv("VR_EXP_FLAVOUR")) {
        const int f = atoi(e);
        if (f >= 0 && f <= 18 && !removed_flavour(f)) c->default_flavour = f;
    }
    if (const char* e = getenv("VR_EXP_P2_WINDOW")) {
        const long long w = atoll(e);
        if (w > 0 && w <= 0x3fffffffll) c->p2_window = (unsigned)w;
    }
    if (const char* e = getenv("VR_EXP_TUNE")) c->tune_mode = atoi(e);
    if (!hip_ok(hipMalloc(&c->d_pw_heads, (size_t)kInFlight * 8 * 64 * sizeof(unsigned)), "hipMalloc(queue heads)")) return bail(VR_ERR_HIP);
    if (!hip_ok(hipMemset(c->d_pw_heads, 0, (size_t)kInFlight * 8 * 64 * sizeof(unsigned)), "hipMemset(queue heads)")) return bail(VR_ERR_HIP);
    if (!hip_ok(hipEventCreate(&c->tm.ev_begin), "hipEventCreate")) return bail(VR_ERR_HIP);
    if (!hip_ok(hipEventCreate(&c->tm.ev_k0), "hipEventCreate")) return bail(VR_ERR_HIP);
    if (!hip_ok(hipEventCreate(&c->tm.ev_k1), "hipEventCreate")) return bail(VR_ERR_HIP);
    if (!hip_ok(hipEventCreate(&c->tm.ev_end), "hipEventCreate")) return bail(VR_ERR_HIP);
    for (int i = 0; i < kRing; ++i)
        if (!hip_ok(hipEventCreate(&c->ring.k0[i]), "hipEventCreate") || !hip_ok(hipEventCreate(&c->ring.k1[i]), "hipEventCreate"))
            return bail(VR_ERR_HIP);
    for (int i = 0; i < kInFlight; ++i)
        if (!hip_ok(hipEventCreateWithFlags(&c->slot_done[i], hipEventDisableTiming), "hipEventCreate")) return bail(VR_ERR_HIP);
    for (auto& o : c->order_ring)
        if (!hip_ok(hipEventCreateWithFlags(&o.sorted, hipEventDisableTiming), "hipEventCreate")) return bail(VR_ERR_HIP);
    if (!hip_ok(hipStreamCreateWithFlags(&c->order_stream, hipStreamNonBlocking), "hipStreamCreate")) return bail(VR_ERR_HIP);
    if (!hip_ok(hipEventCreateWithFlags(&c->edit_ev, hipEventDisableTiming), "hipEventCreate")) return bail(VR_ERR_HIP);
    for (auto& st : c->stage)
        if (!hip_ok(hipEventCreateWithFlags(&st.done, hipEventDisableTiming), "hipEventCreate")) return bail(VR_ERR_HIP);
    if (!hip_ok(hipHostMalloc((void**)&c->h_skip, kGen * sizeof(SkipSummary), hipHostMallocDefault), "hipHostMalloc")) return bail(VR_ERR_HIP);
    std::memset(c->h_skip, 0, kGen * sizeof(SkipSummary));
    if (!hip_ok(hipMalloc(&c->d_skip_sum, kGen * sizeof(SkipSumDev)), "hipMalloc(skip summary)")) return bail(VR_ERR_HIP);
    if (!hip_ok(hipMemset(c->d_skip_sum, 0, kGen * sizeof(SkipSumDev)), "hipMemset(skip summary)")) return bail(VR_ERR_HIP);
    if (hipHostMalloc((void**)&c->h_span, kRing * sizeof(unsigned long long), hipHostMallocDefault) == hipSuccess)
        std::memset(c->h_span, 0, kRing * sizeof(unsigned long long));
    else
        c->h_span = nullptr;
    if (hipHostMalloc((void**)&c->h_end, kRing * sizeof(unsigned long long), hipHostMallocDefault) == hipSuccess)
        std::memset(c->h_end, 0, kRing * sizeof(unsigned long long));
    else
        c->h_end = nullptr;
    if (hipHostMalloc((void**)&c->h_chain, kOrderRing * sizeof(unsigned), hipHostMallocDefault) == hipSuccess)
        std::memset(c->h_chain, 0, kOrderRing * sizeof(unsigned));
    else
        c->h_chain = nullptr;
    if (!hip_ok(hipMalloc(&c->d_counters, 3 * sizeof(unsigned long long)), "hipMalloc(counters)")) return bail(VR_ERR_HIP);
    if (!hip_ok(hipHostMalloc((void**)&c->h_counters, 3 * sizeof(unsigned long long), hipHostMallocDefault),
                "hipHostMalloc"))
        return bail(VR_ERR_HIP);
    c->h_counters[0] = c->h_counters[1] = c->h_counters[2] = 0;
    rc = alloc_frame(c);
    if (rc != VR_OK) return bail(rc);
    *out = c;
    return VR_OK;
}

int vr_resize(vr_ctx* c, uint32_t width, uint32_t height)
{
    if (!c) return VR_ERR_INVALID_ARG;
    if (width == 0 || height == 0 || width > 32768 || height > 32768)
        return fail(c, VR_ERR_INVALID_ARG, "vr_resize: bad viewport size");
    (void)hipSetDevice(c->device);
    (void)hipDeviceSynchronize();
    drained(c);
    c->W = width;
    c->H = height;
    return alloc_frame(c);
}

void vr_destroy(vr_ctx* c)
{
    if (!c) return;
    (void)hipSetDevice(c->device);
    (void)hipDeviceSynchronize();
    drained(c);
    for (int i = 0; i < VR_MAX_VOLUMES; ++i)
        if (c->vol[i].data) (void)hipFree(const_cast<float4*>(c->vol[i].data));
    for (int i = 0; i < VR_MAX_VOLUMES; ++i)
        if (c->vol_bricks[i]) (void)hipFree(c->vol_bricks[i]);
    for (int i = 0; i < VR_MAX_VOLUMES; ++i) {
        if (c->vol_dens[i]) (void)hipFree(c->vol_dens[i]);
        if (c->vol_bricked[i]) (void)hipFree(c->vol_bricked[i]);
        if (c->vol_bdens[i]) (void)hipFree(c->vol_bdens[i]);
    }
    if (c->merged_bricks) (void)hipFree(c->merged_bricks);
    if (c->proj_rec) (void)hipFree(c->proj_rec);
    if (c->proj_range) (void)hipFree(c->proj_range);
    if (c->proj_ev) (void)hipEventDestroy(c->proj_ev);
    for (auto& e : c->shadow) {
        if (e.buf.d) (void)hipFree(e.buf.d);
        if (e.built) (void)hipEventDestroy(e.built);
    }
    for (auto& g : c->field)
        if (g.d) (void)hipFree(g.d);
    if (c->dist_tmp) (void)hipFree(c->dist_tmp);
    for (auto& slot : c->tf_buf)
        for (auto& kind : slot)
            for (auto& g : kind)
                if (g.d) (void)hipFree(g.d);
    for (auto& st : c->stage) {
        if (st.h) (void)hipHostFree(st.h);
        if (st.done) (void)hipEventDestroy(st.done);
    }
    if (c->edit_ev) (void)hipEventDestroy(c->edit_ev);
    if (c->h_skip) (void)hipHostFree(c->h_skip);
    if (c->d_skip_sum) (void)hipFree(c->d_skip_sum);
    if (c->d_frame) (void)hipFree(c->d_frame);
    if (c->d_tiles) (void)hipFree(c->d_tiles);
    if (c->d_present) (void)hipFree(c->d_present);
    if (c->d_counters) (void)hipFree(c->d_counters);
    if (c->d_pw_heads) (void)hipFree(c->d_pw_heads);
    for (auto* b : c->d_block_counts)
        if (b) (void)hipFree(b);
    if (c->h_counters) (void)hipHostFree(c->h_counters);
    for (int i = 0; i < kRing; ++i) {
        if (c->ring.k0[i]) (void)hipEventDestroy(c->ring.k0[i]);
        if (c->ring.k1[i]) (void)hipEventDestroy(c->ring.k1[i]);
    }
    for (auto e : c->slot_done)
        if (e) (void)hipEventDestroy(e);
    for (auto& o : c->order_ring) {
        if (o.sorted) (void)hipEventDestroy(o.sorted);
        if (o.buf) (void)hipFree(o.buf);
    }
    if (c->order_stream) (void)hipStreamDestroy(c->order_stream);
    if (c->h_chain) (void)hipHostFree(c->h_chain);
    if (c->h_span) (void)hipHostFree(c->h_span);
    if (c->h_end) (void)hipHostFree(c->h_end);
    for (int k = 0; k < c->n_flight; ++k) (void)hipStreamDestroy(c->flight[k]);
    if (c->tm.ev_begin) (void)hipEventDestroy(c->tm.ev_begin);
    if (c->tm.ev_k0) (void)hipEventDestroy(c->tm.ev_k0);
    if (c->tm.ev_k1) (void)hipEventDestroy(c->tm.ev_k1);
    if (c->tm.ev_end) (void)hipEventDestroy(c->tm.ev_end);
    if (c->stream) (void)hipStreamDestroy(c->stream);
    delete c;
}

static int volume_upload_common(vr_ctx* c, int slot, const void* src, bool src_is_device, uint16_t nx, uint16_t ny,
                                uint16_t nz)
{
    if (!c) return VR_ERR_INVALID_ARG;
    if (slot < 0 || slot >= VR_MAX_VOLUMES) return fail(c, VR_ERR_INVALID_ARG, "vr_volume_upload: bad slot");
    if (!src) return fail(c, VR_ERR_INVALID_ARG, "vr_volume_upload: data is NULL");
    if (nx == 0 || ny == 0 || nz == 0) return fail(c, VR_ERR_INVALID_ARG, "vr_volume_upload: empty volume");
    unsigned long long voxels = (unsigned long long)nx * ny * nz;
    if (voxels > 0xFFFFFFFFull) return fail(c, VR_ERR_INVALID_ARG, "vr_volume_upload: more than 2^32 voxels");
    size_t bytes = (size_t)voxels * sizeof(float4);
    VR_HIP(c, hipSetDevice(c->device));
    VR_HIP(c, hipDeviceSynchronize());
    drained(c);
    if (c->vol[slot].data && c->vol_bytes[slot] != bytes) {
        (void)hipFree(const_cast<float4*>(c->vol[slot].data));
        c->vol[slot] = DevVolume{};
        c->vol_bytes[slot] = 0;
    }
    float4* d = const_cast<float4*>(c->vol[slot].data);
    if (!d) VR_HIP(c, hipMalloc(&d, bytes));
    hipError_t e = hipMemcpyAsync(d, src, bytes, src_is_device ? hipMemcpyDeviceToDevice : hipMemcpyHostToDevice, c->stream);
    if (e == hipSuccess) e = hipStreamSynchronize(c->stream);
    if (e != hipSuccess) {
        if (!c->vol[slot].data) (void)hipFree(d);
        return fail(c, VR_ERR_HIP, std::string("vr_volume_upload: copy failed: ") + hipGetErrorString(e));
    }
    c->vol[slot].data = d;
    c->vol[slot].nx = nx;
    c->vol[slot].ny = ny;
    c->vol[slot].nz = nz;
    c->vol_bytes[slot] = bytes;
    return refresh_bricks(c, slot);
}

int vr_volume_upload(vr_ctx* c, int slot, const float* vec4_voxels, uint16_t nx, uint16_t ny, uint16_t nz)
{
    return volume_upload_common(c, slot, vec4_voxels, false, nx, ny, nz);
}

int vr_volume_upload_device(vr_ctx* c, int slot, const void* d_vec4_voxels, uint16_t nx, uint16_t ny, uint16_t nz)
{
    return volume_upload_common(c, slot, d_vec4_voxels, true, nx, ny, nz);
}

static int tf_check(vr_ctx* c, int slot, const float* table, uint32_t R, const char* who)
{
    if (slot < 0 || slot >= VR_MAX_TFS) return fail(c, VR_ERR_INVALID_ARG, std::string(who) + ": bad slot");
    if (!table) return fail(c, VR_ERR_INVALID_ARG, std::string(who) + ": table is NULL");
    if (R == 0 || R > (1u << 24)) return fail(c, VR_ERR_INVALID_ARG, std::string(who) + ": bad resolution");
    return VR_OK;
}

static void tf_set_current(vr_ctx* c, int slot, const float* table, uint32_t R, bool is_color)
{
    ++c->tf_epoch;
    const GenBuf& g = c->tf_buf[slot][is_color ? 1 : 0][c->tf_cur[slot][is_color ? 1 : 0]];
    if (is_color) {
        c->tf[slot].color = (const float4*)g.d;
        c->tf[slot].res_c = (int)R;
        c->tf_color_finite[slot] = all_finite(table, (int)(4 * R));
    } else {
        if (slot == 0) ++c->opacity_edits;
        c->tf[slot].opacity = (const float*)g.d;
        c->tf[slot].res_o = (int)R;
        int z = -1;
        c->tf_opacity_finite[slot] = all_finite(table, (int)R);
        if (c->tf_opacity_finite[slot])
            while (z + 1 < (int)R && table[z + 1] == 0.0f) ++z;
        c->tf_zero_prefix[slot] = z;
    }
}

static int tf_upload_one(vr_ctx* c, int slot, const float* table, uint32_t R, bool is_color)
{
    if (!c) return VR_ERR_INVALID_ARG;
    if (const int rc = tf_check(c, slot, table, R, "vr_tf_upload")) return rc;
    VR_HIP(c, hipSetDevice(c->device));
    VR_HIP(c, hipDeviceSynchronize());
    drained(c);
    const int comps = is_color ? 4 : 1;
    GenBuf& g = c->tf_buf[slot][is_color ? 1 : 0][c->tf_cur[slot][is_color ? 1 : 0]];
    if (is_color) {
        c->tf[slot].color = nullptr;
        c->tf[slot].res_c = 0;
    } else {
        c->tf[slot].opacity = nullptr;
        c->tf[slot].res_o = 0;
    }
    if (const int rc = grow(c, &g.d, &g.cap, ((size_t)R + 2) * comps * sizeof(float), true)) return rc;
    float* d = (float*)g.d;
    const size_t texel = comps * sizeof(float);
    VR_HIP(c, hipMemcpyAsync(d + comps, table, R * texel, hipMemcpyHostToDevice, c->stream));
    VR_HIP(c, hipMemcpyAsync(d, table, texel, hipMemcpyHostToDevice, c->stream));
    VR_HIP(c, hipMemcpyAsync(d + ((size_t)R + 1) * comps, table + comps * ((size_t)R - 1), texel, hipMemcpyHostToDevice, c->stream));
    VR_HIP(c, hipStreamSynchronize(c->stream));
    g.written();
    tf_set_current(c, slot, table, R, is_color);
    return VR_OK;
}

static void rebuild_field_async(vr_ctx* c, hipStream_t s)
{
    const int z = c->tf_zero_prefix[0], res = c->tf[0].res_o;
    if (!c->brick_dist || (c->dist_z == z && c->dist_res == res) || c->dist_epoch != c->brick_epoch) return;
    if (c->dist_rgb ? (c->merged_stale || c->dist_records != (const void*)c->merged_bricks) : c->dist_records != (const void*)c->vol_bricks[0])
        return;
    const int b = (c->field_cur + 1) % kGen;
    GenBuf& g = c->field[b];
    const size_t nb = (size_t)c->dist_bn[0] * c->dist_bn[1] * c->dist_bn[2];
    const bool fresh = nb > g.cap;
    if (grow(c, &g.d, &g.cap, nb, false) != VR_OK || grow(c, (void**)&c->dist_tmp, &c->tmp_cap, nb, false) != VR_OK ||
        (!fresh && reuse_wait(c, s, g) != VR_OK) ||
        build_field(c, s, (const float2*)c->dist_records, c->dist_bn, c->dist_rgb, z, res, (unsigned char*)g.d, b, c->skip_gen + 1) != VR_OK) {
        (void)hipGetLastError();
        return;
    }
    ++c->skip_gen;
    g.written();
    c->field_cur = b;
    c->brick_dist = (unsigned char*)g.d;
    c->skip_pending = true;
    c->dist_z = z;
    c->dist_res = res;
}

static int tf_upload_async(vr_ctx* c, int slot, const float* table, uint32_t R, bool is_color, void* stream)
{
    if (!c) return VR_ERR_INVALID_ARG;
    if (const int rc = tf_check(c, slot, table, R, is_color ? "vr_tf_upload_color_async" : "vr_tf_upload_opacity_async")) return rc;
    VR_HIP(c, hipSetDevice(c->device));
    (void)hipGetLastError();
    hipStream_t s = stream ? (hipStream_t)stream : c->stream;
    const int comps = is_color ? 4 : 1, kind = is_color ? 1 : 0;
    const size_t texel = comps * sizeof(float), bytes = ((size_t)R + 2) * texel;
    vr_ctx::Stage& st = c->stage[c->stage_next % kStage];
    if (st.used) VR_HIP(c, hipEventSynchronize(st.done));
    st.used = false;
    if (bytes > st.cap) {
        if (st.h) c->retired_host.push_back(st.h);
        st.h = nullptr;
        st.cap = 0;
// ... 122 lines not shown
    VR_HIP(c, hipSetDevice(c->device));
    (void)hipGetLastError();
    hipStream_t s = stream ? (hipStream_t)stream : c->stream;
    float4* frame = d_frame ? (float4*)d_frame : c->d_frame;
    dim3 block(64, 4), grid((c->W + 63) / 64, (c->H + 3) / 4);
    hipLaunchKernelGGL(unpack_tiles_kernel, grid, block, 0, s, (const float4*)d_gathered, frame, (int)c->W, (int)c->H,
                       tiles_x_of(c), world, rank_stride_tiles);
    VR_HIP(c, hipGetLastError());
    return VR_OK;
}

int vr_unpack_tiles_async(vr_ctx* c, const void* d_gathered, int world, void* d_frame, void* stream)
{
    if (!c) return VR_ERR_INVALID_ARG;
    if (world < 1) return fail(c, VR_ERR_INVALID_ARG, "vr_unpack_tiles_async: bad arguments");
    return vr_unpack_tiles_strided_async(c, d_gathered, world, tile_count(c, 0, world), d_frame, stream);
}

int vr_present_async(vr_ctx* c, const void* d_frame, void* d_bgra8, void* stream)
{
    if (!c) return VR_ERR_INVALID_ARG;
    if (!d_bgra8) return fail(c, VR_ERR_INVALID_ARG, "vr_present_async: destination is NULL");
    VR_HIP(c, hipSetDevice(c->device));
    (void)hipGetLastError();
    hipStream_t s = stream ? (hipStream_t)stream : c->stream;
    const size_t n = (size_t)c->W * c->H;
    hipLaunchKernelGGL(present_kernel, dim3((unsigned)((n + 255) / 256)), dim3(256), 0, s,
                       d_frame ? (const float4*)d_frame : c->d_frame, (uint32_t*)d_bgra8, (int)n);
    VR_HIP(c, hipGetLastError());
    return VR_OK;
}

int vr_present_tiles_async(vr_ctx* c, const void* d_gathered, int world, int rank_stride_tiles, void* d_bgra8, void* stream)
{
    if (!c) return VR_ERR_INVALID_ARG;
    if (!d_gathered || !d_bgra8 || world < 1) return fail(c, VR_ERR_INVALID_ARG, "vr_present_tiles_async: bad arguments");
    const int tpr = tile_count(c, 0, world);
    if (rank_stride_tiles <= 0) rank_stride_tiles = tpr;
    if (rank_stride_tiles < tpr) return fail(c, VR_ERR_INVALID_ARG, "vr_present_tiles_async: stride smaller than a segment");
    VR_HIP(c, hipSetDevice(c->device));
    (void)hipGetLastError();
    hipStream_t s = stream ? (hipStream_t)stream : c->stream;
    dim3 block(64, 4), grid((c->W + 63) / 64, (c->H + 3) / 4);
    hipLaunchKernelGGL(present_tiles_kernel, grid, block, 0, s, (const float4*)d_gathered, (uint32_t*)d_bgra8, (int)c->W, (int)c->H,
                       tiles_x_of(c), world, rank_stride_tiles);
    VR_HIP(c, hipGetLastError());
    return VR_OK;
}

int vr_present_packed_async(vr_ctx* c, const void* d_tiles_rgba, int n_tiles, void* d_tiles_bgra8, void* stream)
{
    if (!c) return VR_ERR_INVALID_ARG;
    if (!d_tiles_rgba || !d_tiles_bgra8 || n_tiles < 0) return fail(c, VR_ERR_INVALID_ARG, "vr_present_packed_async: bad arguments");
    if (n_tiles == 0) return VR_OK;
    VR_HIP(c, hipSetDevice(c->device));
    (void)hipGetLastError();
    hipStream_t s = stream ? (hipStream_t)stream : c->stream;
    const size_t n = (size_t)n_tiles * kTile * kTile;
    if (n > 0x7fffffffull) return fail(c, VR_ERR_INVALID_ARG, "vr_present_packed_async: too many tiles");
    hipLaunchKernelGGL(present_kernel, dim3((unsigned)((n + 255) / 256)), dim3(256), 0, s, (const float4*)d_tiles_rgba, (uint32_t*)d_tiles_bgra8, (int)n);
    VR_HIP(c, hipGetLastError());
    return VR_OK;
}

int vr_unpack_tiles_bgra8_async(vr_ctx* c, const void* d_gathered_bgra8, int world, int rank_stride_tiles, void* d_bgra8, void* stream)
{
    if (!c) return VR_ERR_INVALID_ARG;
    if (!d_gathered_bgra8 || !d_bgra8 || world < 1) return fail(c, VR_ERR_INVALID_ARG, "vr_unpack_tiles_bgra8_async: bad arguments");
    const int tpr = tile_count(c, 0, world);
    if (rank_stride_tiles <= 0) rank_stride_tiles = tpr;
    if (rank_stride_tiles < tpr) return fail(c, VR_ERR_INVALID_ARG, "vr_unpack_tiles_bgra8_async: stride smaller than a segment");
    VR_HIP(c, hipSetDevice(c->device));
    (void)hipGetLastError();
    hipStream_t s = stream ? (hipStream_t)stream : c->stream;
    dim3 block(64, 4), grid((c->W + 63) / 64, (c->H + 3) / 4);
    hipLaunchKernelGGL(unpack_tiles_u32_kernel, grid, block, 0, s, (const uint32_t*)d_gathered_bgra8, (uint32_t*)d_bgra8, (int)c->W, (int)c->H,
                       tiles_x_of(c), world, rank_stride_tiles);
    VR_HIP(c, hipGetLastError());
    return VR_OK;
}

int vr_download(vr_ctx* c, float* frag_rgba, uint8_t* present_bgra8, uint64_t* composited_samples)
{
    if (!c) return VR_ERR_INVALID_ARG;
    VR_HIP(c, hipSetDevice(c->device));
    VR_HIP(c, hipStreamSynchronize(c->stream));
    size_t n = (size_t)c->W * c->H;
    if (frag_rgba) VR_HIP(c, hipMemcpy(frag_rgba, c->d_frame, n * sizeof(float4), hipMemcpyDeviceToHost));
    if (present_bgra8) {
        (void)hipGetLastError();
        hipLaunchKernelGGL(present_kernel, dim3((unsigned)((n + 255) / 256)), dim3(256), 0, c->stream, c->d_frame,
                           c->d_present, (int)n);
        VR_HIP(c, hipGetLastError());
        VR_HIP(c, hipStreamSynchronize(c->stream));
        VR_HIP(c, hipMemcpy(present_bgra8, c->d_present, n * sizeof(uint32_t), hipMemcpyDeviceToHost));
    }
    if (composited_samples) {
        int rc = fetch_counters(c);
        if (rc != VR_OK) return rc;
        *composited_samples = c->h_counters[0];
    }
    return VR_OK;
}

int vr_download_tiles(vr_ctx* c, float* tiles_rgba, uint64_t* composited_samples)
{
    if (!c) return VR_ERR_INVALID_ARG;
    VR_HIP(c, hipSetDevice(c->device));
    VR_HIP(c, hipStreamSynchronize(c->stream));
    if (tiles_rgba && c->last_tiles > 0)
        VR_HIP(c, hipMemcpy(tiles_rgba, c->d_tiles, (size_t)c->last_tiles * kTile * kTile * sizeof(float4),
                            hipMemcpyDeviceToHost));
    if (composited_samples) {
        int rc = fetch_counters(c);
        if (rc != VR_OK) return rc;
        *composited_samples = c->h_counters[0];
    }
    return VR_OK;
}

int vr_last_timing(vr_ctx* c, float* kernel_ms, float* total_ms)
{
    if (!c) return VR_ERR_INVALID_ARG;
    if (!c->tm.valid) return fail(c, VR_ERR_NOT_READY, "vr_last_timing: no vr_render / vr_render_tiles since the context was created or an *_async call");
    VR_HIP(c, hipSetDevice(c->device));
    VR_HIP(c, hipEventSynchronize(c->tm.ev_end));
    float k = 0.0f, t = 0.0f;
    VR_HIP(c, hipEventElapsedTime(&k, c->tm.ev_k0, c->tm.ev_k1));
    VR_HIP(c, hipEventElapsedTime(&t, c->tm.ev_begin, c->tm.ev_end));
    if (kernel_ms) *kernel_ms = k;
    if (total_ms) *total_ms = t;
    return VR_OK;
}

int vr_kernel_times(vr_ctx* c, float* out_ms, int capacity)
{
    if (!c) return VR_ERR_INVALID_ARG;
    if (!out_ms || capacity < 0) return fail(c, VR_ERR_INVALID_ARG, "vr_kernel_times: bad arguments");
    VR_HIP(c, hipSetDevice(c->device));
    long long have = c->ring.head < kRing ? c->ring.head : kRing;
    int n = (int)(have < capacity ? have : capacity);
    bool synced = false;
    for (int i = 0; i < n; ++i) {
        int slot = (int)((c->ring.head - n + i) % kRing);
        if (!c->ring_events[slot]) {
            if (!synced) VR_HIP(c, hipStreamSynchronize(c->order_stream));
            synced = true;
            const unsigned long long ticks = *(volatile unsigned long long*)&c->h_span[slot];
            out_ms[i] = ticks ? (float)((double)(ticks - 1) * 1.0e-5) : 0.0f;
            continue;
        }
        VR_HIP(c, hipEventSynchronize(c->ring.k1[slot]));
        VR_HIP(c, hipEventElapsedTime(&out_ms[i], c->ring.k0[slot], c->ring.k1[slot]));
    }
    return n;
}

int vr_set_kernel_timing(vr_ctx* c, int mode)
{
    if (!c) return VR_ERR_INVALID_ARG;
    if (mode != VR_TIMING_RECORDS && mode != VR_TIMING_EVENTS) return fail(c, VR_ERR_INVALID_ARG, "vr_set_kernel_timing: bad mode");
    c->event_timing = mode == VR_TIMING_EVENTS;
    return VR_OK;
}

int vr_reset_kernel_times(vr_ctx* c)
{
    if (!c) return VR_ERR_INVALID_ARG;
    VR_HIP(c, hipSetDevice(c->device));
    VR_HIP(c, hipStreamSynchronize(c->order_stream));
    c->ring.head = 0;
    return VR_OK;
}

void* vr_frame_device_ptr(vr_ctx* c) { return c ? (void*)c->d_frame : nullptr; }

int vr_viewport(const vr_ctx* c, uint32_t* width, uint32_t* height, int* device_id)
{
    if (!c) return VR_ERR_INVALID_ARG;
    if (width) *width = c->W;
    if (height) *height = c->H;
    if (device_id) *device_id = c->device;
    return VR_OK;
}

int vr_last_covered_pixels(vr_ctx* c, uint64_t* covered)
{
    if (!c || !covered) return VR_ERR_INVALID_ARG;
    VR_HIP(c, hipSetDevice(c->device));
    VR_HIP(c, hipStreamSynchronize(c->stream));
    int rc = fetch_counters(c);
    if (rc != VR_OK) return rc;
    *covered = c->h_counters[1];
    return VR_OK;
}

int vr_last_counters(vr_ctx* c, uint64_t out[3])
{
    if (!c || !out) return VR_ERR_INVALID_ARG;
    VR_HIP(c, hipSetDevice(c->device));
    VR_HIP(c, hipStreamSynchronize(c->stream));
    int rc = fetch_counters(c);
    if (rc != VR_OK) return rc;
    out[0] = c->h_counters[0];
    out[1] = c->h_counters[1];
    out[2] = c->h_counters[2];
    return VR_OK;
}

int vr_last_block_trace(vr_ctx* c, uint64_t* out, int capacity)
{
    if (!c || capacity < 0 || (capacity > 0 && !out)) return VR_ERR_INVALID_ARG;
    VR_HIP(c, hipSetDevice(c->device));
    VR_HIP(c, hipDeviceSynchronize());
    const int n = c->cnt_blocks < capacity ? c->cnt_blocks : capacity;
    if (n > 0) {
        const unsigned long long* src = c->d_block_counts[c->cnt_buf] + c->cnt_offset;
        VR_HIP(c, hipMemcpy(out, src, (size_t)n * kBlockRecord * sizeof(unsigned long long), hipMemcpyDeviceToHost));
    }
    return c->cnt_blocks;
}

int vr_last_kernel_flavour(vr_ctx* c)
{
    if (!c) return VR_ERR_INVALID_ARG;
    return c->last_flavour;
}

int vr_skip_field(vr_ctx* c, int variant, uint8_t* dist, size_t capacity, int dims[3], int box[6], uint64_t* active)
{
    if (!c) return VR_ERR_INVALID_ARG;
    if (variant < 0 || variant >= VR_VARIANT_COUNT) return fail(c, VR_ERR_INVALID_ARG, "vr_skip_field: bad variant");
    if (capacity > 0 && !dist) return fail(c, VR_ERR_INVALID_ARG, "vr_skip_field: dist is NULL");
    int nvol, ntf;
    variant_needs(variant, &nvol, &ntf);
    for (int i = 0; i < nvol; ++i)
        if (!c->vol[i].data) return fail(c, VR_ERR_NOT_READY, "vr_skip_field: volume slot " + std::to_string(i) + " is empty");
    for (int i = 0; i < ntf; ++i)
        if (!c->tf[i].opacity || !c->tf[i].color) return fail(c, VR_ERR_NOT_READY, "vr_skip_field: TF slot " + std::to_string(i) + " is empty");
    VR_HIP(c, hipSetDevice(c->device));
    VR_HIP(c, hipDeviceSynchronize());
    drained(c);
    (void)hipGetLastError();
    const Eligibility E = eligibility(c, 0, variant, 1, 0, 1, false, nullptr);
    if (!E.can_skip) return fail(c, VR_ERR_NOT_READY, "vr_skip_field: launches of this variant do not skip empty space now");
    MarchParams P;
    std::memset(&P, 0, sizeof P);
    if (const int rc = prepare_skip(c, variant, c->stream, P)) return rc;
    VR_HIP(c, hipStreamSynchronize(c->stream));
    const float bs[3] = {P.bsx, P.bsy, P.bsz};
    adopt_skip(c, bs);
    if (c->skip_pending) return fail(c, VR_ERR_HIP, "vr_skip_field: the field's count and box did not arrive");
    const size_t n = (size_t)c->dist_bn[0] * c->dist_bn[1] * c->dist_bn[2];
    if (capacity > 0) VR_HIP(c, hipMemcpy(dist, c->brick_dist, capacity < n ? capacity : n, hipMemcpyDeviceToHost));
    if (dims)
        for (int a = 0; a < 3; ++a) dims[a] = c->dist_bn[a];
    if (box)
        for (int a = 0; a < 6; ++a) box[a] = c->skip_box[a];
    if (active) *active = c->skip_active;
    return (int)n;
}

int64_t vr_unbounded_box_launches(vr_ctx* c)
{
    if (!c) return VR_ERR_INVALID_ARG;
    return c->unbounded_launches;
}

static float spin_span_ms(hipStream_t a, hipStream_t b, hipEvent_t e0, hipEvent_t e1)
{
    const unsigned long long ticks = 15000;
    (void)hipStreamSynchronize(a);
    if (b) (void)hipStreamSynchronize(b);
    (void)hipEventRecord(e0, a);
    hipLaunchKernelGGL(spin_kernel, dim3(1), dim3(64), 0, a, ticks, (unsigned*)nullptr);
    if (b) hipLaunchKernelGGL(spin_kernel, dim3(1), dim3(64), 0, b, ticks, (unsigned*)nullptr);
    (void)hipEventRecord(e1, b ? b : a);
    (void)hipStreamSynchronize(a);
    if (b) (void)hipStreamSynchronize(b);
    float ms = 0.0f;
    if (hipEventElapsedTime(&ms, e0, e1) != hipSuccess) return -1.0f;
    return ms;
}

static bool streams_overlap(hipStream_t a, hipStream_t b, hipEvent_t e0, hipEvent_t e1, float one_ms)
{
    for (int attempt = 0; attempt < 2; ++attempt) {
        const float ms = spin_span_ms(a, b, e0, e1);
        if (getenv("VR_DEBUG_STREAMS")) fprintf(stderr, "[vr_stream] pair %p %p: %.3f ms (one spin %.3f ms)\n", (void*)a, (void*)b, ms, one_ms);
        if (ms < 0.0f || one_ms <= 0.0f) return true;
        if (ms < one_ms + 0.075f) return true;
    }
    return false;
}

void* vr_stream(vr_ctx* c, int index)
{
    if (!c || index < 0 || index >= kStreams) return nullptr;
    if (c->n_flight == 0) {
        if (hipSetDevice(c->device) != hipSuccess) return nullptr;
        (void)hipGetLastError();
        hipEvent_t e0 = nullptr, e1 = nullptr;
        if (hipEventCreate(&e0) != hipSuccess || hipEventCreate(&e1) != hipSuccess) return nullptr;
        float one_ms = -1.0f;
        hipStream_t rejected[12];
        int n_rejected = 0;
// ... 140 lines not shown
```

volumerendering_amd/csrc/vr_device.h:

```cpp
#pragma once
#include <hip/hip_runtime.h>
#include <stdint.h>

namespace vr {

constexpr int kTile = 64;
constexpr int kBlockEdge = 16;
constexpr int kBlockRecord = 6;
constexpr int kBlocksPerTile = (kTile / kBlockEdge) * (kTile / kBlockEdge);
#ifndef VR_BRICK_SHIFT
#define VR_BRICK_SHIFT 2
#endif
constexpr int kBrickShift = VR_BRICK_SHIFT;
constexpr int kBrickCells = 1 << kBrickShift;
constexpr float kBrickInv = 1.0f / (float)kBrickCells;
constexpr float kBrickHalf = 0.5f / (float)kBrickCells;
#ifndef VR_DIST_MAX
#define VR_DIST_MAX 128
#endif
constexpr int kDistMax = VR_DIST_MAX;
static_assert(kDistMax >= 2 && kDistMax <= 128, "the distance-field builder (vr_kernels.h) is exact for caps up to 128");

struct SkipSummary {
    unsigned long long gen;
    unsigned long long count;
    int box[6];
};
#ifndef VR_VOX_BRICK_SHIFT
#define VR_VOX_BRICK_SHIFT 2
#endif
constexpr unsigned kVbS = VR_VOX_BRICK_SHIFT;
constexpr unsigned kVbM = (1u << kVbS) - 1u;
constexpr unsigned kVbN = 1u << (3u * kVbS);

struct DevVolume {
    const float4* data;
    const float* dens;
    const char* a_base;
    int a_shift;
    int nx, ny, nz;
    int bricked;
    unsigned brick_row, brick_slab;
    unsigned data_bytes;
    int lut;
};

struct DevTF {
    const float* opacity;
    const float4* color;
    int res_o, res_c;
};

struct MarchParams {
    float proj_inv[16];
    float view_inv[16];
    int W, H;
    int fragment_mode;
    int steps_count;
    float step_size;
    float bmin[3], bmax[3];
    int toggle_varstep, toggle_jitter;
    float light_pos[3], light_amb[3], light_dif[3];
    float camera_pos[3];
    DevVolume vol[3];
    DevTF tf[2];
    int rank, world, tiles_x, tiles_y, n_tiles;
    int packed;
    int rect[4];
    int n_blocks;
    const float2* bricks;
    int use_rgb;
    const unsigned char* brick_dist;
    int skip_vol;
    float abox[6];
    int bnx, bny, bnz;
    float bsx, bsy, bsz;
    int tf_zero_prefix;
    const unsigned* order;
    float4* out;
    unsigned long long* block_counts;
    unsigned batch_n;
    float iso;
};

constexpr int kBatchMax = 4;
struct MarchBatch {
    MarchParams frame[kBatchMax];
    unsigned n_frames;
};

struct PwQueue {
    unsigned* heads;
    unsigned n_items;
    unsigned p2_window;
};

struct LaunchDesc {
    enum Family { kPlain, kDp, kPw, kP2, kLt, kProj, kIso, kShadow };
    int variant;
    Family family;
    bool off32;
    int lanes;
    bool pipe;
    bool ltf;
    bool p2_skip;
    bool p2_win;
    unsigned lds_bytes;
    PwQueue queue;
    dim3 grid, block;
    const float2* vrange;
    bool proj_skip;
};

}
```

volumerendering_amd/csrc/vr_kernels.h:

```cpp
#pragma once
#include "vr_device.h"

#ifndef VR_KNS
#define VR_KNS vr
#endif
#ifndef VR_FUSED
#define VR_FUSED 0
#endif

namespace VR_KNS {
using namespace vr;

enum Variant : int { V_BASIC = 0, V_LIGHT = 1, V_VOLUME_MASK = 2, V_THREE_FILES = 3, V_MULTI_CTRT = 4, V_TF_CALIB = 5,
                     V_ILLUSTRATIVE = 6, V_LIGHT_INSHADER = 7 };

struct f3 {
    float x, y, z;
};

__device__ __forceinline__ f3 mk3(float x, float y, float z) { return f3{x, y, z}; }
__device__ __forceinline__ float mad(float a, float b, float c)
{
#if VR_FUSED
    return __builtin_fmaf(a, b, c);
// ... 726 lines not shown
        float rt = tex3_a<OFF32>(P.vol[1], p);
        TfSample tct = tf_lookup0<LTF>(P, ct.w);
        TfSample trt = tf_lookup(P.tf[1], rt);
        float om = 1.0f - trt.opacity;
        f3 col = mk3(mad(trt.rgb.x, trt.opacity, tct.rgb.x * om), mad(trt.rgb.y, trt.opacity, tct.rgb.y * om),
                     mad(trt.rgb.z, trt.opacity, tct.rgb.z * om));
        f3 g = mk3(ct.x, ct.y, ct.z);
        f3 N = normalize3(g);
        f3 s3 = shade(N, w, mk3(0.0f, -5.0f, 0.0f), mk3(P.light_dif[0], P.light_dif[1], P.light_dif[2]),
                      mk3(P.light_amb[0], P.light_amb[1], P.light_amb[2]), 3.5f, 0.5f);
        o.rgb = mk3(col.x * s3.x, col.y * s3.y, col.z * s3.z);
        f3 L = normalize3(mk3(0.0f - w.x, -5.0f - w.y, 0.0f - w.z));
        f3 Vv = normalize3(mk3(P.camera_pos[0] - w.x, P.camera_pos[1] - w.y, P.camera_pos[2] - w.z));
        f3 H = normalize3(mk3(Vv.x + L.x, Vv.y + L.y, Vv.z + L.z));
        float s = (0.5f + 2.5f * length3(mk3(L.x * g.x, L.y * g.y, L.z * g.z))) +
                  1.0f * pow_rep(length3(mk3(H.x * g.x, H.y * g.y, H.z * g.z)), 1.0f);
        float dist = length3(mk3(p.x - start.x, p.y - start.y, p.z - start.z));
        if (dist > 1.0f) dist = 1.0f;
        float inner = pow_rep(((5.0f * s) * (1.0f - dist)) * (1.0f - dst_a), 0.8f);
        o.a = tct.opacity * pow_rep(length3(g), inner);
    } else {
        float density = tex3_a<OFF32>(P.vol[0], p);
        float4 mask = tex3_nearest<OFF32>(P.vol[1], p);
        TfSample t = tf_lookup0<LTF>(P, density);
        if (mask.x > 0.0f) {
            t.rgb = mk3(1.0f, 1.0f, 0.0f);
            t.opacity = 0.1f;
        }
        o.rgb = t.rgb;
        o.a = t.opacity;
    }
    return o;
}
__device__ __forceinline__ bool opacity_is_zero(const MarchParams& P, float d)
{
    const int jo = padded_texel(floorf(mad(d, (float)P.tf[0].res_o, -0.5f)), P.tf[0].res_o);
    return (d - d == 0.0f) && jo <= P.tf_zero_prefix;
}

template <bool UNI = false, bool MASKED = false, bool SHADOW = false>
__device__ __forceinline__ void shade_blend_packed(f3 lpos, f3 dif, f3 amb, float kD, float kA, f3 w, v2f zw, v2f gxy, const TfFetch& tq, float4& dst,
                                                   bool masked = false, f3 trt_rgb = f3{0.0f, 0.0f, 0.0f}, float trt_a = 0.0f, float S = 1.0f)
{
    v2f Lxy = v2f{lpos.x - w.x, lpos.y - w.y};
    float Lz = lpos.z - w.z;
#if VR_FUSED
    const v2f inv = inv_sqrt_exact2<UNI>(mad(zw.x, zw.x, mad(gxy.y, gxy.y, gxy.x * gxy.x)), mad(Lz, Lz, mad(Lxy.y, Lxy.y, Lxy.x * Lxy.x)));
#else
    const v2f g2 = gxy * gxy, l2 = Lxy * Lxy;
    const v2f inv = inv_sqrt_exact2<UNI>((g2.x + g2.y) + zw.x * zw.x, (l2.x + l2.y) + Lz * Lz);
#endif
    const float inv_g = inv.x, inv_l = inv.y;
    const v2f Nxy = gxy * inv_g;
    const float Nz = zw.x * inv_g;
    Lxy = Lxy * inv_l;
    Lz = Lz * inv_l;
#if VR_FUSED
    float m = max0(mad(Nz, Lz, mad(Nxy.y, Lxy.y, Nxy.x * Lxy.x)));
#else
    const v2f nl = Nxy * Lxy;
    float m = max0((nl.x + nl.y) + Nz * Lz);
#endif
    if constexpr (SHADOW) m = m * S;
    const v2f sh_rg = mad2(v2f{dif.x, dif.y} * m, v2f{kD, kD}, v2f{amb.x, amb.y} * kA);
    const float sh_b = mad(dif.z * m, kD, amb.z * kA);
    float opacity = lerpf(tq.o0, tq.o1, tq.fo);
    const v2f c_rg = lerp2(v2f{tq.c0.x, tq.c0.y}, v2f{tq.c1.x, tq.c1.y}, tq.fc);
    const float c_b = lerpf(tq.c0.z, tq.c1.z, tq.fc);
    v2f rgb_rg = c_rg * sh_rg;
    float rgb_b = c_b * sh_b;
    if constexpr (MASKED) {
        rgb_rg = masked ? v2f{trt_rgb.x, trt_rgb.y} : rgb_rg;
        rgb_b = masked ? trt_rgb.z : rgb_b;
        opacity = masked ? trt_a : opacity;
    }
    const v2f src_rg = rgb_rg * opacity;
    const float src_b = rgb_b * opacity;
    const float om = 1.0f - dst.w;
    const v2f d_rg = mad2(src_rg, v2f{om, om}, v2f{dst.x, dst.y});
    dst.x = d_rg.x;
    dst.y = d_rg.y;
    dst.z = mad(om, src_b, dst.z);
    dst.w = mad(om, opacity, dst.w);
}
template <bool UNI = false>
__device__ __forceinline__ void light_shade_blend(const MarchParams& P, f3 w, v2f zw, v2f gxy, const TfFetch& tq, float4& dst)
{
    shade_blend_packed<UNI>(mk3(P.light_pos[0], P.light_pos[1], P.light_pos[2]), mk3(P.light_dif[0], P.light_dif[1], P.light_dif[2]),
                            mk3(P.light_amb[0], P.light_amb[1], P.light_amb[2]), 2.5f, 0.5f, w, zw, gxy, tq, dst);
}

template <int V, bool OFF32, bool ZSKIP = false, bool LTF = false>
__device__ __forceinline__ void sample_and_blend(const MarchParams& P, f3 p, f3 w, float4& dst, f3 start, float ss)
{
    if constexpr (V == V_BASIC && ZSKIP) {
        const float density = tex3_a<OFF32>(P.vol[0], p);
        if (vr_ballot(!opacity_is_zero(P, density)) == 0) return;
        const TfSample t = tf_lookup0<LTF>(P, density);
        blend(t.rgb, t.opacity, dst);
    } else if constexpr (V == V_LIGHT) {
        Fetch4 q;
        float fx, fy, fz;
        fetch_rgba<OFF32>(P.vol[0], p, q, fx, fy, fz);
        const v2f zw = interp_zw(q, fx, fy, fz);
        if constexpr (ZSKIP) {
            if (vr_ballot(!opacity_is_zero(P, zw.y)) == 0) return;
        }
        const TfFetch tq = tf_fetch0<LTF>(P, zw.y);
        const v2f gxy = interp_xy(q, fx, fy, fz);
        light_shade_blend(P, w, zw, gxy, tq, dst);
    } else {
        if constexpr (ZSKIP && (V == V_VOLUME_MASK || V == V_THREE_FILES || V == V_LIGHT_INSHADER)) {
            if constexpr (V == V_VOLUME_MASK) {
                const float4 ct = tex3_rgba<OFF32>(P.vol[2], p);
                float4 mask;
                float rt;
                bool any_masked;
                fetch_mask_and_dose<OFF32>(P, p, mask, rt, any_masked);
                const bool inert = !(mask.x > 0.0f || mask.y > 0.0f || mask.z > 0.0f) && opacity_is_zero(P, ct.w);
                if (vr_ballot(!inert) == 0) return;
                const Src s = src_volume_mask<LTF>(P, w, mask, rt, ct, any_masked);
                blend(s.rgb, s.a, dst);
            } else if constexpr (V == V_THREE_FILES) {
                const float ct = tex3_a<OFF32>(P.vol[0], p);
                const float rt = tex3_a<OFF32>(P.vol[1], p);
                if (vr_ballot(!opacity_is_zero(P, ct)) == 0) return;
                const Src s = src_three_files<LTF>(P, ct, rt);
                blend(s.rgb, s.a, dst);
            } else {
                const float density = tex3_a<OFF32>(P.vol[0], p);
                if (vr_ballot(!opacity_is_zero(P, density)) == 0) return;
                const Src s = src_inshader<OFF32, LTF>(P, p, w, ss, density);
                blend(s.rgb, s.a, dst);
            }
            return;
        }
        const Src s = sample_src<V, OFF32, LTF>(P, p, w, start, dst.w, ss);
        blend(s.rgb, s.a, dst);
    }
}

struct PixelSlot {
    int px, py;
    int out_index;
    bool active;
    bool in_launch;
};

__device__ __forceinline__ unsigned batch_group(unsigned g, unsigned n)
{
    return n == 1 ? g : (n == 2 ? g >> 1 : (n == 3 ? g / 3u : g >> 2));
}

__device__ __forceinline__ int logical_block(const MarchParams& P)
{
    const unsigned b = (batch_group(blockIdx.x >> 3, P.batch_n) << 3) | (blockIdx.x & 7u);
    if (P.order == nullptr) return (int)b;
    return (int)__builtin_amdgcn_readfirstlane((int)P.order[b]);
}

template <bool BATCH>
__device__ __forceinline__ const MarchParams& frame_params(const MarchBatch& B)
{
    if constexpr (!BATCH) return B.frame[0];
    const unsigned g = blockIdx.x >> 3, n = B.n_frames;
    return B.frame[g - batch_group(g, n) * n];
}

__device__ __forceinline__ PixelSlot map_pixel_at(const MarchParams& P, int lb, int wpb, int wib)
{
    PixelSlot s;
    int n, pk;
    if (wpb == 1) {
        n = lb / 64;
        const int l = lb % 64, hi = l >> 3;
        pk = (((l & 7) | ((hi & 1) << 3)) << 2) | (hi >> 1);
    } else {
        const int bpt = 64 / wpb;
        n = lb / bpt;
        pk = (lb % bpt) * wpb + wib;
    }
    const int sub = pk >> 2;
    const bool in_launch = n < P.n_tiles;
    const int t = P.rank + n * P.world;
    const int ty = t / P.tiles_x, tx = t - ty * P.tiles_x;
    const int wave = pk & 3, lane = threadIdx.x & 63;
    const int lx = ((wave & 1) << 3) + (lane & 7);
    const int ly = ((wave >> 1) << 3) + (lane >> 3);
    const int tpx = ((sub & 3) << 4) + lx, tpy = ((sub >> 2) << 4) + ly;
    s.px = tx * kTile + tpx;
    s.py = ty * kTile + tpy;
    s.in_launch = in_launch;
    s.active = in_launch && (s.px < P.W) && (s.py < P.H);
    s.out_index = P.packed ? (n * (kTile * kTile) + tpy * kTile + tpx) : (s.py * P.W + s.px);
    return s;
}
__device__ __forceinline__ PixelSlot map_pixel(const MarchParams& P)
{
    return map_pixel_at(P, logical_block(P), (int)(blockDim.x >> 6), (int)(threadIdx.x >> 6));
}

template <bool FMED = true>
__device__ __forceinline__ int brick_of(const MarchParams& P, f3 p)
{
    int bx, by, bz;
    if constexpr (FMED) {
        bx = (int)__builtin_amdgcn_fmed3f(mad(p.x, P.bsx, -kBrickHalf), 0.0f, (float)(P.bnx - 1));
        by = (int)__builtin_amdgcn_fmed3f(mad(p.y, P.bsy, -kBrickHalf), 0.0f, (float)(P.bny - 1));
        bz = (int)__builtin_amdgcn_fmed3f(mad(p.z, P.bsz, -kBrickHalf), 0.0f, (float)(P.bnz - 1));
    } else {
        bx = clampi((int)floorf(mad(p.x, P.bsx, -kBrickHalf)), 0, P.bnx - 1);
        by = clampi((int)floorf(mad(p.y, P.bsy, -kBrickHalf)), 0, P.bny - 1);
        bz = clampi((int)floorf(mad(p.z, P.bsz, -kBrickHalf)), 0, P.bnz - 1);
    }
    return __mul24(__mul24(bz, P.bny) + by, P.bnx) + bx;
}
__device__ __forceinline__ unsigned dist_at(const MarchParams& P, int bid)
{
    return *(reinterpret_cast<const unsigned char*>(P.brick_dist) + (unsigned)bid);
}
__device__ __forceinline__ float2 brick_record(const MarchParams& P, int bid)
{
    return *reinterpret_cast<const float2*>(reinterpret_cast<const char*>(P.bricks) + ((unsigned)bid << 3));
}
__device__ __forceinline__ bool brick_inert(const MarchParams& P, float2 rec)
{
    if (P.use_rgb && !(rec.y <= 0.0f)) return false;
    if (rec.x <= 0.0f) return P.tf_zero_prefix >= 0;
    return floorf(rec.x * (float)P.tf[0].res_o - 0.5f) + 2.0f <= (float)P.tf_zero_prefix;
}

__device__ __forceinline__ void store_block_counts(const MarchParams& P, unsigned blends, unsigned covered, unsigned fetched,
                                                   unsigned long long t_start)
{
    __shared__ unsigned long long part[4][3];
    unsigned long long packed_cnt = ((unsigned long long)covered << 40) | (unsigned long long)blends;
    unsigned long long fetched_cnt = fetched;
    unsigned crit = fetched;
#pragma unroll
    for (int off = 32; off > 0; off >>= 1) {
        packed_cnt += __shfl_down(packed_cnt, off, 64);
        fetched_cnt += __shfl_down(fetched_cnt, off, 64);
        crit = max(crit, (unsigned)__shfl_down((int)crit, off, 64));
    }
    if ((threadIdx.x & 63) == 0) {
        part[threadIdx.x >> 6][0] = packed_cnt;
        part[threadIdx.x >> 6][1] = fetched_cnt;
        part[threadIdx.x >> 6][2] = crit;
    }
    __syncthreads();
    if (threadIdx.x == 0) {
        unsigned long long pc = 0, fc = 0, cr = 0;
        for (int i = 0; i < (int)(blockDim.x >> 6); ++i) {
            pc += part[i][0];
            fc += part[i][1];
            cr = part[i][2] > cr ? part[i][2] : cr;
        }
        unsigned long long* o = P.block_counts + (size_t)logical_block(P) * kBlockRecord;
        o[0] = pc & ((1ull << 40) - 1);
        o[1] = pc >> 40;
        o[2] = fc;
        o[3] = t_start;
        o[4] = wall_clock64();
        o[5] = (unsigned long long)__builtin_amdgcn_s_getreg((4) | (0 << 6) | (31 << 11)) |
               ((unsigned long long)(__builtin_amdgcn_s_getreg((20) | (0 << 6) | (31 << 11)) & 0x7fu) << 32) | (cr << 40);
    }
}

__device__ __forceinline__ void store_wave_counts(const MarchParams& P, int rec, unsigned blends, unsigned covered, unsigned fetched,
                                                  unsigned long long t_start)
{
    unsigned long long packed_cnt = ((unsigned long long)covered << 40) | (unsigned long long)blends;
    unsigned long long fetched_cnt = fetched;
    unsigned crit = fetched;
#pragma unroll
    for (int off = 32; off > 0; off >>= 1) {
        packed_cnt += __shfl_down(packed_cnt, off, 64);
        fetched_cnt += __shfl_down(fetched_cnt, off, 64);
        crit = max(crit, (unsigned)__shfl_down((int)crit, off, 64));
    }
    if ((threadIdx.x & 63) == 0) {
        unsigned long long* o = P.block_counts + (size_t)rec * kBlockRecord;
        o[0] = packed_cnt & ((1ull << 40) - 1);
        o[1] = packed_cnt >> 40;
        o[2] = fetched_cnt;
        o[3] = t_start;
        o[4] = wall_clock64();
        o[5] = (unsigned long long)__builtin_amdgcn_s_getreg((4) | (0 << 6) | (31 << 11)) |
               ((unsigned long long)(__builtin_amdgcn_s_getreg((20) | (0 << 6) | (31 << 11)) & 0x7fu) << 32) |
               ((unsigned long long)crit << 40);
    }
}

__device__ __forceinline__ float steps_inside_axis(float p, float s, float b0, float b1)
{
    const float e = fmaxf(fmaxf(fabsf(b0), fabsf(b1)), fabsf(p)) * 1.1920929e-7f;
    if (s > 0.0f) return (b1 - p) / (s + e);
    if (s < 0.0f) return (p - b0) / (e - s);
    return 3.0e38f;
}
__device__ __forceinline__ int steps_inside(f3 p, f3 step, float bx0, float by0, float bz0, float bx1, float by1, float bz1)
{
    const bool in0 = p.x >= bx0 && p.x <= bx1 && p.y >= by0 && p.y <= by1 && p.z >= bz0 && p.z <= bz1;
    const float f = fminf(fminf(steps_inside_axis(p.x, step.x, bx0, bx1), steps_inside_axis(p.y, step.y, by0, by1)),
                          fminf(steps_inside_axis(p.z, step.z, bz0, bz1), 1.0e6f)) * 0.999f - 2.0f;
    return (in0 && f > 0.0f) ? (int)f : 0;
}

constexpr int kApproachMax = 1024;
__device__ __forceinline__ void steps_near_box(f3 p, f3 s, const float* box, int n_steps, int& k0, int& k1)
{
// ... 240 lines not shown
{
    const MarchParams& P = frame_params<BATCH>(B);
    const unsigned long long t_start = wall_clock64();
    PixelSlot slot = map_pixel(P);
    float4 dst = make_float4(0.0f, 0.0f, 0.0f, 0.0f);
    unsigned blends = 0, covered = 0, fetched = 0;
    if (B.frame[0].vol[0].lut) {
        const bool may_hit = slot.active && slot.px >= P.rect[0] && slot.px <= P.rect[2] && slot.py >= P.rect[1] && slot.py <= P.rect[3];
        if (__syncthreads_or(may_hit ? 1 : 0)) {
            lut_fill(B.frame[0].vol[0]);
            __syncthreads();
        }
    }

    march_packet<V, OFF32, SKIP, LEAP, false>(P, slot, dst, blends, covered, fetched);

    if (slot.active || (P.packed && slot.in_launch)) P.out[slot.out_index] = dst;

    store_block_counts(P, blends, covered, fetched, t_start);
}

#if !VR_FUSED
__global__ __launch_bounds__(64) void brick_max_kernel(const float4* __restrict__ vol, int nx, int ny, int nz, int bnx,
                                                       int bny, float2* __restrict__ out)
{
    const int b = blockIdx.x;
    const int bx = b % bnx, by = (b / bnx) % bny, bz = b / (bnx * bny);
    const int x0 = bx << kBrickShift, y0 = by << kBrickShift, z0 = bz << kBrickShift;
    const int ex = min(kBrickCells + 1, nx - x0), ey = min(kBrickCells + 1, ny - y0), ez = min(kBrickCells + 1, nz - z0);
    float m = -INFINITY, mc = -INFINITY;
    bool has_nan = false, has_nan_c = false;
    for (int t = threadIdx.x; t < ex * ey * ez; t += 64) {
        int lx = t % ex, ly = (t / ex) % ey, lz = t / (ex * ey);
        float4 v = vol[((size_t)(z0 + lz) * ny + (y0 + ly)) * nx + (x0 + lx)];
        if (!(v.w - v.w == 0.0f)) has_nan = true;
        else if (v.w > m) m = v.w;
        if (v.x != v.x || v.y != v.y || v.z != v.z) has_nan_c = true;
        else mc = fmaxf(mc, fmaxf(v.x, fmaxf(v.y, v.z)));
    }
#pragma unroll
    for (int off = 32; off > 0; off >>= 1) {
        m = fmaxf(m, __shfl_down(m, off, 64));
        mc = fmaxf(mc, __shfl_down(mc, off, 64));
        const int other = __shfl_down((int)has_nan, off, 64), other_c = __shfl_down((int)has_nan_c, off, 64);
        has_nan = has_nan || other != 0;
        has_nan_c = has_nan_c || other_c != 0;
    }
    if (threadIdx.x == 0) out[b] = make_float2(has_nan ? NAN : m, has_nan_c ? NAN : mc);
}

__device__ __forceinline__ unsigned unorm8(float v)
{
    if (!(v > 0.0f)) v = 0.0f;
    if (v > 1.0f) v = 1.0f;
    return (unsigned)floorf(v * 255.0f + 0.5f);
}

__global__ void present_kernel(const float4* __restrict__ frag, uint32_t* __restrict__ bgra, int n)
{
    int i = blockIdx.x * blockDim.x + threadIdx.x;
    if (i >= n) return;
    float4 s = frag[i];
    float a = s.w;
    float r = s.x * a + 1.0f * (1.0f - a);
    float g = s.y * a + 1.0f * (1.0f - a);
    float b = s.z * a + 1.0f * (1.0f - a);
    float oa = s.w * a + 1.0f * (1.0f - a);
    bgra[i] = unorm8(b) | (unorm8(g) << 8) | (unorm8(r) << 16) | (unorm8(oa) << 24);
}

__global__ void present_tiles_kernel(const float4* __restrict__ gathered, uint32_t* __restrict__ bgra, int W, int H, int tiles_x,
                                     int world, int tiles_per_rank_max)
{
    int x = blockIdx.x * blockDim.x + threadIdx.x;
    int y = blockIdx.y * blockDim.y + threadIdx.y;
    if (x >= W || y >= H) return;
    int t = (y / kTile) * tiles_x + (x / kTile);
    int r = t % world, n = t / world;
    size_t src = ((size_t)r * tiles_per_rank_max + n) * (kTile * kTile) + (y % kTile) * kTile + (x % kTile);
    float4 s = gathered[src];
    float a = s.w;
    float rr = s.x * a + 1.0f * (1.0f - a);
    float g = s.y * a + 1.0f * (1.0f - a);
    float b = s.z * a + 1.0f * (1.0f - a);
    float oa = s.w * a + 1.0f * (1.0f - a);
    bgra[(size_t)y * W + x] = unorm8(b) | (unorm8(g) << 8) | (unorm8(rr) << 16) | (unorm8(oa) << 24);
}

__global__ void unpack_tiles_kernel(const float4* __restrict__ gathered, float4* __restrict__ frame, int W, int H,
                                    int tiles_x, int world, int tiles_per_rank_max)
{
    int x = blockIdx.x * blockDim.x + threadIdx.x;
    int y = blockIdx.y * blockDim.y + threadIdx.y;
    if (x >= W || y >= H) return;
    int t = (y / kTile) * tiles_x + (x / kTile);
    int r = t % world, n = t / world;
    size_t src = ((size_t)r * tiles_per_rank_max + n) * (kTile * kTile) + (y % kTile) * kTile + (x % kTile);
    frame[(size_t)y * W + x] = gathered[src];
}

__global__ void unpack_tiles_u32_kernel(const uint32_t* __restrict__ gathered, uint32_t* __restrict__ frame, int W, int H, int tiles_x,
                                        int world, int tiles_per_rank_max)
{
    int x = blockIdx.x * blockDim.x + threadIdx.x;
    int y = blockIdx.y * blockDim.y + threadIdx.y;
    if (x >= W || y >= H) return;
    int t = (y / kTile) * tiles_x + (x / kTile);
    int r = t % world, n = t / world;
    size_t src = ((size_t)r * tiles_per_rank_max + n) * (kTile * kTile) + (y % kTile) * kTile + (x % kTile);
    frame[(size_t)y * W + x] = gathered[src];
}

__global__ __launch_bounds__(256) void sum_block_counts_kernel(const unsigned long long* __restrict__ in, int n_blocks,
                                                               unsigned long long* __restrict__ out)
{
    __shared__ unsigned long long part[4][3];
    unsigned long long a = 0, b = 0, f = 0;
    for (int i = threadIdx.x; i < n_blocks; i += 256) {
        a += in[(size_t)i * kBlockRecord];
        b += in[(size_t)i * kBlockRecord + 1];
        f += in[(size_t)i * kBlockRecord + 2];
    }
#pragma unroll
    for (int off = 32; off > 0; off >>= 1) {
        a += __shfl_down(a, off, 64);
        b += __shfl_down(b, off, 64);
        f += __shfl_down(f, off, 64);
    }
    if ((threadIdx.x & 63) == 0) {
        part[threadIdx.x >> 6][0] = a;
        part[threadIdx.x >> 6][1] = b;
        part[threadIdx.x >> 6][2] = f;
    }
    __syncthreads();
    if (threadIdx.x < 3) out[threadIdx.x] = part[0][threadIdx.x] + part[1][threadIdx.x] + part[2][threadIdx.x] + part[3][threadIdx.x];
}

__global__ __launch_bounds__(64) void spin_kernel(unsigned long long ticks, unsigned* __restrict__ sink)
{
    const unsigned long long t0 = wall_clock64();
    unsigned n = 0;
    while (wall_clock64() - t0 < ticks && n < 4000000u) {
        __builtin_amdgcn_s_sleep(8);
        ++n;
    }
    if (sink && threadIdx.x == 0 && n == 0xFFFFFFFFu) *sink = n;
}

constexpr int kOrderMaxBlocks = 192 * 1024;
__global__ __launch_bounds__(1024) void order_blocks_kernel(const unsigned long long* __restrict__ in, int n_blocks,
                                                            unsigned* __restrict__ order, unsigned* __restrict__ longest_chain,
                                                            unsigned long long* __restrict__ span_ticks,
                                                            unsigned* __restrict__ pw_heads,
                                                            unsigned long long* __restrict__ end_tick = nullptr)
{
    if (pw_heads != nullptr && threadIdx.x < 8) pw_heads[threadIdx.x * 64] = 0u;
    __shared__ unsigned hist[1024];
    __shared__ unsigned base[1024];
    __shared__ unsigned chain_max;
    __shared__ unsigned long long t_first, t_last;
    const int t = threadIdx.x;
    hist[t] = 0;
    if (t == 0) {
        chain_max = 0;
        t_first = ~0ull;
        t_last = 0ull;
    }
    unsigned my_chain = 0;
    unsigned long long my_first = ~0ull, my_last = 0ull;
    __syncthreads();
    unsigned short bk[kOrderMaxBlocks / 1024];
    for (int k = 0; k * 1024 < n_blocks; ++k) {
        const int b = t + k * 1024;
        if (b < n_blocks) {
            const unsigned long long crit = in[(size_t)b * kBlockRecord + 5] >> 40;
            const unsigned long long b0 = in[(size_t)b * kBlockRecord + 3], b1 = in[(size_t)b * kBlockRecord + 4];
            my_first = b0 < my_first ? b0 : my_first;
            my_last = b1 > my_last ? b1 : my_last;
            my_chain = crit > my_chain ? (unsigned)crit : my_chain;
            const unsigned q = (unsigned)(crit >> 5);
            bk[k] = (unsigned short)(((unsigned)b & 7u) * 128u + (127u - (q > 127u ? 127u : q)));
            atomicAdd(&hist[bk[k]], 1u);
        }
    }
    __syncthreads();
    {
        const unsigned mine = hist[t];
        unsigned incl = mine;
#pragma unroll
        for (int off = 1; off < 64; off <<= 1) {
            const unsigned up = (unsigned)__shfl_up((int)incl, off, 64);
            if ((t & 63) >= off) incl += up;
        }
        __shared__ unsigned wave_total[16];
        if ((t & 63) == 63) wave_total[t >> 6] = incl;
        __syncthreads();
        const unsigned before = ((t >> 6) & 1) ? wave_total[(t >> 6) - 1] : 0u;
        base[t] = before + incl - mine;
    }
    __syncthreads();
    if (longest_chain) {
        atomicMax(&chain_max, my_chain);
        __syncthreads();
        if (t == 0) *longest_chain = chain_max + 1u;
    }
    if (span_ticks) {
        atomicMin(&t_first, my_first);
        atomicMax(&t_last, my_last);
        __syncthreads();
        if (t == 0) {
            if (end_tick) *end_tick = t_last | 1ull;
            __threadfence_system();
            *span_ticks = t_last >= t_first ? t_last - t_first + 1ull : 1ull;
        }
    }
    for (int k = 0; k * 1024 < n_blocks; ++k) {
        const int b = t + k * 1024;
        if (b < n_blocks) order[8u * atomicAdd(&base[bk[k]], 1u) + ((unsigned)b & 7u)] = (unsigned)b;
    }
}

__global__ void brick_active_kernel(const float2* __restrict__ rec, unsigned char* __restrict__ dist, int n, int use_rgb,
                                    int zero_prefix, int res_o)
{
    int i = blockIdx.x * blockDim.x + threadIdx.x;
    if (i >= n) return;
    const float2 r = rec[i];
    bool inert;
    if (use_rgb && !(r.y <= 0.0f)) inert = false;
    else if (r.x <= 0.0f) inert = zero_prefix >= 0;
    else inert = floorf(r.x * (float)res_o - 0.5f) + 2.0f <= (float)zero_prefix;
    dist[i] = inert ? 255 : 0;
}
constexpr int kDistHalo = kDistMax - 1;
constexpr int kDistCols = 128;
constexpr int kDistRows = 64;

__global__ void brick_dist_x_kernel(unsigned char* __restrict__ dist, int bnx, int rows)
{
    const int lane = (int)(threadIdx.x & 63u);
    const long long segs = (bnx + 63) >> 6, w = ((long long)blockIdx.x * blockDim.x + threadIdx.x) >> 6;
    if (w >= segs * rows) return;
    const int x0 = (int)(w % segs) * 64;
    unsigned char* line = dist + (size_t)(w / segs) * (size_t)bnx;
    unsigned long long m[5];
#pragma unroll
    for (int k = 0; k < 5; ++k) {
        const int x = x0 - 128 + 64 * k + lane;
        m[k] = vr_ballot(x >= 0 && x < bnx && line[x] == 0);
    }
    const unsigned long long le = m[2] & ((2ull << lane) - 1ull), ri = m[2] & ~((1ull << lane) - 1ull);
    int d = kDistMax;
    if (le) d = lane - (63 - __clzll((long long)le));
    else if (m[1]) d = lane + 64 - (63 - __clzll((long long)m[1]));
    else if (m[0]) d = lane + 128 - (63 - __clzll((long long)m[0]));
    int e = kDistMax;
    if (ri) e = __ffsll((long long)ri) - 1 - lane;
    else if (m[3]) e = 64 + __ffsll((long long)m[3]) - 1 - lane;
    else if (m[4]) e = 128 + __ffsll((long long)m[4]) - 1 - lane;
    d = min(min(d, e), kDistMax);
    if (x0 + lane < bnx) line[x0 + lane] = (unsigned char)d;
}

struct SkipSumDev {
    unsigned count, done;
    unsigned lo[3], hi[3];
};

template <bool LAST>
__global__ void __launch_bounds__(256) brick_dist_axis_kernel(const unsigned char* __restrict__ in, unsigned char* __restrict__ out,
                                                               int bnx, int n_axis, size_t axis_stride, size_t other_stride,
                                                               SkipSumDev* __restrict__ sum, SkipSummary* __restrict__ host,
                                                               unsigned long long gen)
{
    constexpr int kTileRows = kDistRows + 2 * kDistHalo;
    __shared__ unsigned char tile[kTileRows][kDistCols];
    const int t = (int)threadIdx.x;
    const int x0 = (int)blockIdx.x * kDistCols, a0 = (int)blockIdx.y * kDistRows;
    const size_t base = (size_t)blockIdx.z * other_stride;
    for (int idx = t; idx < kTileRows * kDistCols; idx += 256) {
        const int r = idx / kDistCols, cx = idx % kDistCols, x = x0 + cx, a = a0 - kDistHalo + r;
        tile[r][cx] = (x < bnx && a >= 0 && a < n_axis) ? in[base + (size_t)a * axis_stride + (size_t)x] : (unsigned char)kDistMax;
    }
    __syncthreads();
    __shared__ unsigned char col_min[kDistCols];
    if (t < kDistCols) {
        int m = kDistMax;
        for (int r = 0; r < kTileRows; ++r) m = min(m, (int)tile[r][t]);
        col_min[t] = (unsigned char)m;
    }
    __syncthreads();
    const int cx = t % kDistCols, x = x0 + cx, floor_c = col_min[cx];
    unsigned cnt = 0;
    int lo[3] = {0x7fffffff, 0x7fffffff, 0x7fffffff}, hi[3] = {-1, -1, -1};
    for (int i = t / kDistCols; i < kDistRows; i += 256 / kDistCols) {
        const int a = a0 + i;
        if (x >= bnx || a >= n_axis) continue;
        const int R = i + kDistHalo, reach = max(a, n_axis - 1 - a);
        int best = tile[R][cx];
        for (int k = 1; k < best && best > floor_c && k <= reach; ++k) best = min(best, max(k, (int)min(tile[R - k][cx], tile[R + k][cx])));
        out[base + (size_t)a * axis_stride + (size_t)x] = (unsigned char)best;
        if constexpr (LAST) {
            if (best == 0) {
                const int p[3] = {x, (int)blockIdx.z, a};
                ++cnt;
#pragma unroll
                for (int q = 0; q < 3; ++q) {
                    lo[q] = min(lo[q], p[q]);
                    hi[q] = max(hi[q], p[q]);
                }
            }
        }
    }
    if constexpr (LAST) {
        for (int off = 32; off > 0; off >>= 1) {
            cnt += __shfl_down(cnt, off, 64);
#pragma unroll
            for (int q = 0; q < 3; ++q) {
                lo[q] = min(lo[q], __shfl_down(lo[q], off, 64));
                hi[q] = max(hi[q], __shfl_down(hi[q], off, 64));
            }
        }
        __shared__ int red[4][7];
        __shared__ bool last;
        const int wv = t >> 6;
        if ((t & 63) == 0) {
            red[wv][0] = (int)cnt;
            for (int q = 0; q < 3; ++q) {
                red[wv][1 + q] = lo[q];
                red[wv][4 + q] = hi[q];
            }
        }
        __syncthreads();
        if (t == 0) {
            for (int v = 1; v < 4; ++v) {
                red[0][0] += red[v][0];
                for (int q = 0; q < 3; ++q) {
                    red[0][1 + q] = min(red[0][1 + q], red[v][1 + q]);
                    red[0][4 + q] = max(red[0][4 + q], red[v][4 + q]);
                }
            }
            if (red[0][0] != 0) {
                atomicAdd(&sum->count, (unsigned)red[0][0]);
                for (int q = 0; q < 3; ++q) {
                    atomicMax(&sum->lo[q], 0x7fffffffu - (unsigned)red[0][1 + q]);
                    atomicMax(&sum->hi[q], (unsigned)(red[0][4 + q] + 1));
                }
            }
            __threadfence();
            last = atomicAdd(&sum->done, 1u) == gridDim.x * gridDim.y * gridDim.z - 1u;
        }
        __syncthreads();
        if (last && t == 0) {
            __threadfence();
            volatile SkipSumDev* v = sum;
            host->count = v->count;
            for (int q = 0; q < 3; ++q) {
                host->box[q] = (int)(0x7fffffffu - v->lo[q]);
                host->box[3 + q] = (int)v->hi[q] - 1;
            }
            __threadfence_system();
            host->gen = gen;
            v->count = 0;
            v->done = 0;
            for (int q = 0; q < 3; ++q) v->lo[q] = v->hi[q] = 0;
        }
    }
}

__global__ void merge_bricks_kernel(const float2* __restrict__ density_vol, const float2* __restrict__ mask_vol,
                                    float2* __restrict__ out, int n)
// ... 132 lines not shown
```

volumerendering_amd/csrc/vr_p2.h:

```cpp
#pragma once
#include "vr_pw.h"

namespace VR_KNS {
using namespace vr;

#ifndef VR_P2_JUMP_MAX
#define VR_P2_JUMP_MAX 1024
#endif
constexpr int kP2JumpMax = VR_P2_JUMP_MAX;
#ifndef VR_P2_EXIT
#define VR_P2_EXIT 1
#endif
constexpr bool kP2Exit = VR_P2_EXIT != 0;
constexpr int kP2Threads = 768;
constexpr int kP2ThreadsUnlit = 1024;


struct P2Lds {
    unsigned off_x, off_y, off_z;
    int mx, my, mz;
    unsigned win_last;
    unsigned win_slabs;
    unsigned win_slots;
};
// ... 9 lines not shown
    for (int e = (int)threadIdx.x; e <= v.nx; e += (int)blockDim.x) {
        const unsigned i0 = (unsigned)max(e - 1, 0), i1 = (unsigned)min(e, v.nx - 1);
        *reinterpret_cast<uint2*>(lds + L.off_x + (unsigned)e * 8u) =
            make_uint2((i0 >> kVbS) * kVbN + (i0 & kVbM), (i1 >> kVbS) * kVbN + (i1 & kVbM));
    }
    for (int e = (int)threadIdx.x; e <= v.ny; e += (int)blockDim.x) {
        const unsigned j0 = (unsigned)max(e - 1, 0), j1 = (unsigned)min(e, v.ny - 1);
        *reinterpret_cast<uint2*>(lds + L.off_y + (unsigned)e * 8u) =
            make_uint2((j0 >> kVbS) * v.brick_row + ((j0 & kVbM) << kVbS), (j1 >> kVbS) * v.brick_row + ((j1 & kVbM) << kVbS));
    }
    for (int e = (int)threadIdx.x; e <= v.nz; e += (int)blockDim.x) {
        const unsigned k0 = (unsigned)max(e - 1, 0), k1 = (unsigned)min(e, v.nz - 1);
        *reinterpret_cast<uint2*>(lds + L.off_z + (unsigned)e * 8u) =
            make_uint2((k0 >> kVbS) * v.brick_slab + ((k0 & kVbM) << (2u * kVbS)), (k1 >> kVbS) * v.brick_slab + ((k1 & kVbM) << (2u * kVbS)));
    }
}

struct P2Win {
    unsigned long long ptr;
    unsigned records;
    unsigned base;
};

template <int V>
__device__ __forceinline__ void p2_set_window(P2Win& win, const DevVolume& vol, unsigned first_slot, unsigned n_slots)
{
    const char* b = (V == V_BASIC) ? vol.a_base + (size_t)first_slot * 4u : reinterpret_cast<const char*>(vol.data) + (size_t)first_slot * 16u;
    win.ptr = (unsigned long long)reinterpret_cast<size_t>(b);
    win.records = n_slots;
    win.base = first_slot;
}
template <int V>
__device__ __forceinline__ __amdgpu_buffer_rsrc_t p2_descriptor(const P2Win& win)
{
    const unsigned lo = (unsigned)__builtin_amdgcn_readfirstlane((int)(unsigned)win.ptr), hi = (unsigned)__builtin_amdgcn_readfirstlane((int)(unsigned)(win.ptr >> 32));
    void* p = reinterpret_cast<void*>((size_t)(((unsigned long long)hi << 32) | lo));
    return __builtin_amdgcn_make_buffer_rsrc(p, V == V_BASIC ? 4 : 16, __builtin_amdgcn_readfirstlane((int)win.records), 0x00020000);
}
template <int V>
constexpr unsigned p2_window_slots() { return V == V_BASIC ? 0x3fffffffu : 0x0fffffffu; }

struct P2Addr {
    uint2 ex, ey, ez;
    float fx, fy, fz;
    int tz;
};
__device__ __forceinline__ P2Addr p2_address(const DevVolume& vol, const P2Lds& L, f3 q)
{
    P2Addr a;
    const float x = mad(q.x, (float)vol.nx, -0.5f), y = mad(q.y, (float)vol.ny, -0.5f), z = mad(q.z, (float)vol.nz, -0.5f);
    const float x0 = floorf(x), y0 = floorf(y), z0 = floorf(z);
    a.fx = x - x0;
    a.fy = y - y0;
    a.fz = z - z0;
    const int tx = min(max((int)x0, -1), L.mx), ty = min(max((int)y0, -1), L.my);
    a.tz = min(max((int)z0, -1), L.mz);
    a.ex = lds_pair(L.off_x + ((unsigned)(tx + 1) << 3));
    a.ey = lds_pair(L.off_y + ((unsigned)(ty + 1) << 3));
    a.ez = lds_pair(L.off_z + ((unsigned)(a.tz + 1) << 3));
    return a;
}
template <int V, bool MASKED, bool WIN, typename T>
__device__ __forceinline__ void p2_issue(const MarchParams& P0, const DevVolume& vol, const P2Lds& L, P2Win& win, int& n_in_w, const P2Addr& a, T (&X)[8],
                                         float& fx, float& fy, float& fz, unsigned long long keep, bool need, unsigned& dbyte, float& mrec)
{
    fx = a.fx;
    fy = a.fy;
    fz = a.fz;
    const uint2 ex = a.ex, ey = a.ey, ez = a.ez;
    const int tz = a.tz;
    unsigned az0 = ez.x, az1 = ez.y;
    if constexpr (WIN) {
        az0 -= win.base;
        az1 -= win.base;
        unsigned chk = need ? az0 : 0u;
        asm volatile("" : "+v"(chk));
        const unsigned long long out = vr_ballot(chk > L.win_last);
        if (out != 0) {
            const int kb = __builtin_amdgcn_readlane(max(tz, 0) >> kVbS, (int)__builtin_ctzll(out));
            const int span = (int)L.win_slabs - 2;
            const unsigned first = (unsigned)max(0, kb - span / 2) * vol.brick_slab, total = vol.brick_slab * (((unsigned)vol.nz + kVbM) >> kVbS);
            p2_set_window<V>(win, vol, first, min(total - first, L.win_slots));
            az0 = ez.x - win.base;
            az1 = ez.y - win.base;
            unsigned chk2 = need ? az0 : 0u;
            asm volatile("" : "+v"(chk2));
            if (vr_ballot(chk2 > L.win_last) != 0) n_in_w = 0;
        }
    }
    const unsigned r00 = ey.x + az0, r10 = ey.y + az0, r01 = ey.x + az1, r11 = ey.y + az1;
    unsigned o[8] = {r00 + ex.x, r00 + ex.y, r10 + ex.x, r10 + ex.y, r01 + ex.x, r01 + ex.y, r11 + ex.x, r11 + ex.y};
    if constexpr (MASKED) {
        static_assert(kBrickShift == (int)kVbS, "the skipping's bricks are the layout's bricks");
        const unsigned bid = (WIN ? o[0] + win.base : o[0]) >> (3u * kVbS);
        dbyte = dist_at(P0, (int)bid);
        if constexpr (V == V_VOLUME_MASK) mrec = brick_record(P0, (int)bid).y;
    }
    const __amdgpu_buffer_rsrc_t rsrc = p2_descriptor<V>(win);
    unsigned long long exec_saved = 0;
    if constexpr (MASKED) {
        asm volatile("" : "+v"(o[0]), "+v"(o[1]), "+v"(o[2]), "+v"(o[3]), "+v"(o[4]), "+v"(o[5]), "+v"(o[6]), "+v"(o[7]));
        __builtin_amdgcn_sched_barrier(0);
        asm volatile("s_mov_b64 %0, exec\n\ts_and_b64 exec, exec, %1" : "=&s"(exec_saved) : "s"(keep) : "scc");
    }
#pragma unroll
    for (int k = 0; k < 8; ++k) {
        if constexpr (V == V_BASIC) X[k] = __builtin_bit_cast(float, vr_struct_load_b32(rsrc, (int)o[k], 0, 0, 0));
        else X[k] = __builtin_bit_cast(vr_f4, vr_struct_load_b128(rsrc, (int)o[k], 0, 0, 0));
    }
    if constexpr (MASKED) {
        __builtin_amdgcn_sched_barrier(0);
        asm volatile("s_mov_b64 exec, %0" : : "s"(exec_saved));
        __builtin_amdgcn_sched_barrier(0);
    }
}

template <int V, bool MASKED, bool WIN, typename T>
__device__ __forceinline__ void p2_request(const MarchParams& P0, const DevVolume& vol, const P2Lds& L, P2Win& win, int& n_in_w, f3 q, T (&X)[8], float& fx,
                                           float& fy, float& fz, unsigned long long keep, bool need, unsigned& dbyte, float& mrec)
{
    const P2Addr a = p2_address(vol, L, q);
    p2_issue<V, MASKED, WIN>(P0, vol, L, win, n_in_w, a, X, fx, fy, fz, keep, need, dbyte, mrec);
}

__device__ __forceinline__ int wave_min_i32(int v)
{
    v = min(v, __builtin_amdgcn_update_dpp(v, v, 0xB1, 0xF, 0xF, false));
    v = min(v, __builtin_amdgcn_update_dpp(v, v, 0x4E, 0xF, 0xF, false));
    v = min(v, __builtin_amdgcn_update_dpp(v, v, 0x141, 0xF, 0xF, false));
    v = min(v, __builtin_amdgcn_update_dpp(v, v, 0x140, 0xF, 0xF, false));
    return min(min(__builtin_amdgcn_readlane(v, 0), __builtin_amdgcn_readlane(v, 16)), min(__builtin_amdgcn_readlane(v, 32), __builtin_amdgcn_readlane(v, 48)));
}

__device__ __forceinline__ bool p2_vote(const MarchParams& P0, bool sampled, float d, bool masked = false)
{
    int j = padded_texel(floorf(mad(d, (float)P0.tf[0].res_o, -0.5f)), P0.tf[0].res_o);
    j = (d - d == 0.0f) ? j : 0x7fffffff;
    j = masked ? 0x7fffffff : j;
    j = sampled ? j : (int)0x80000000;
    asm volatile("" : "+v"(j));
    return vr_ballot(j > P0.tf_zero_prefix) != 0;
}

template <int V, bool SKIP, bool WIN, bool BATCH>
__global__ __launch_bounds__(V == V_BASIC ? kP2ThreadsUnlit : kP2Threads) void march_p2_kernel(const MarchBatch B, const PwQueue Q)
{
    static_assert(V == V_LIGHT || V == V_BASIC || (V == V_VOLUME_MASK && SKIP), "lit / unlit shader; the three-volume composite with its brick records");
    constexpr int kSrc = (V == V_VOLUME_MASK) ? 2 : 0;
    constexpr bool kLit = V != V_BASIC;
    constexpr bool kExit = SKIP && kP2Exit;
    const MarchParams& P0 = B.frame[0];
    const DevVolume& vol = P0.vol[kSrc];
    P2Lds L;
    {
        const unsigned tf_bytes = (unsigned)(P0.tf[0].res_o + 2) * 16u;
        L.off_x = tf_bytes;
        L.off_y = L.off_x + (unsigned)(vol.nx + 1) * 8u;
        L.off_z = L.off_y + (unsigned)(vol.ny + 1) * 8u;
        L.mx = vol.nx - 1;
        L.my = vol.ny - 1;
        L.mz = vol.nz - 1;
        L.win_slots = WIN ? (Q.p2_window ? Q.p2_window : p2_window_slots<V>()) : 0u;
        L.win_slabs = WIN ? L.win_slots / vol.brick_slab : 0u;
        L.win_last = WIN ? (L.win_slabs - 2u) * vol.brick_slab + (kVbM << (2u * kVbS)) : 0u;
        const int n = P0.tf[0].res_o + 2;
        constexpr int kU = 6;
        for (int base = (int)threadIdx.x; base < n; base += kU * (int)blockDim.x) {
            float4 c[kU];
            float o[kU];
#pragma unroll
            for (int u = 0; u < kU; ++u) {
                const int j = min(base + u * (int)blockDim.x, n - 1);
                c[u] = P0.tf[0].color[j];
                o[u] = P0.tf[0].opacity[j];
            }
#pragma unroll
            for (int u = 0; u < kU; ++u) {
                const int j = base + u * (int)blockDim.x;
                if (j < n) vr_lds_tf[j] = make_float4(c[u].x, c[u].y, c[u].z, o[u]);
            }
        }
        p2_fill_tables(vol, L);
        __syncthreads();
    }
    const unsigned total_slots = vol.brick_slab * (((unsigned)vol.nz + kVbM) >> kVbS);
    const unsigned cls = blockIdx.x & 7u;
    const unsigned groups = (gridDim.x - cls + 7u) >> 3;
    const unsigned wib = (unsigned)__builtin_amdgcn_readfirstlane((int)(threadIdx.x >> 6));
    const unsigned wpb = blockDim.x >> 6;
    const unsigned nf = B.n_frames;
    const unsigned n_c = (Q.n_items >> 3) * nf;
    unsigned idx = wib * groups + (blockIdx.x >> 3);
    typedef typename std::conditional<kLit, vr_f4, float>::type Elem;
    const unsigned cur = cls;
    for (;;) {
        if (idx >= n_c) break;
        const unsigned item = batch_group(idx, nf), frame = idx - item * nf;
        const MarchParams& P = B.frame[(unsigned)__builtin_amdgcn_readfirstlane((int)frame)];
        const f3 light_pos = mk3(P.light_pos[0], P.light_pos[1], P.light_pos[2]), light_dif = mk3(P.light_dif[0], P.light_dif[1], P.light_dif[2]),
                 light_amb = mk3(P.light_amb[0], P.light_amb[1], P.light_amb[2]);
        const int steps_count = P.steps_count;
        const unsigned pos = (item << 3) | cur;
        int lb = (int)pos;
        if (P0.order != nullptr) lb = __builtin_amdgcn_readfirstlane((int)P0.order[pos]);
        const unsigned long long t_start = wall_clock64();
        const PixelSlot slot = map_pixel_at(P0, lb, 1, 0);
        const float bx0 = P.bmin[0], by0 = P.bmin[1], bz0 = P.bmin[2];
        const float bx1 = P.bmax[0], by1 = P.bmax[1], bz1 = P.bmax[2];
        float4 dst = make_float4(0.0f, 0.0f, 0.0f, 0.0f);
        unsigned blends = 0, covered = 0, fetched = 0;
#if VR_P2_DEBUG
        unsigned dbg_trips = 0, dbg_sampled = 0, dbg_shaded = 0, dbg_jumps = 0;
        unsigned long long dbg_wait_corners = 0, dbg_wait_bytes = 0, dbg_loop = 0;
        unsigned long long dbg_tail = 0;
        const unsigned long long dbg_pkt0 = __builtin_readcyclecounter();
#endif
        bool alive = false;
        f3 p = mk3(0.0f, 0.0f, 0.0f), w = p, step = p, wstep = p;
        int n_inside = 0;
        if (slot.active && slot.px >= P.rect[0] && slot.px <= P.rect[2] && slot.py >= P.rect[1] && slot.py <= P.rect[3]) {
            Ray ray = setup_ray(P, slot.px, slot.py);
            if (ray.hit) {
                covered = 1;
                f3 diff = mk3(ray.end.x - ray.start.x, ray.end.y - ray.start.y, ray.end.z - ray.start.z);
                f3 dir = normalize3s(diff);
                float ray_len = length3s(diff);
                if (P.fragment_mode == 1) {
                    dst = make_float4(fabsf(dir.x), fabsf(dir.y), fabsf(dir.z), 1.0f);
                } else if (P.fragment_mode == 2) {
                    dst = make_float4(ray.start.x, ray.start.y, ray.start.z, 1.0f);
                } else if (P.fragment_mode == 3) {
                    dst = make_float4(ray.end.x, ray.end.y, ray.end.z, 1.0f);
                } else if (P.fragment_mode == 4) {
                    dst = make_float4(0.5f * (ray.world0.x / 1.0f) + 0.5f, -0.5f * (ray.world0.y / 1.0f) + 0.5f, 0.0f, 1.0f);
                } else {
                    float step_size = P.step_size;
                    if constexpr (V == V_LIGHT) {
                        wstep = mk3(dir.x * (step_size * 1.0f), dir.y * (step_size * 1.0f), dir.z * (step_size * 0.5f));
                        wstep.z = wstep.z * (-1.0f);
                    }
                    if (P.toggle_varstep == 1) step_size = ray_len / (float)steps_count;
                    p = ray.start;
                    if (P.toggle_jitter == 1) {
                        float jt = jitter((float)slot.px + 0.5f, (float)slot.py + 0.5f);
                        p = mk3(p.x + (dir.x * step_size) * jt, p.y + (dir.y * step_size) * jt, p.z + (dir.z * step_size) * jt);
                    }
                    step = mk3(dir.x * step_size, dir.y * step_size, dir.z * step_size);
                    if constexpr (V == V_VOLUME_MASK) wstep = step;
                    w = ray.world0;
                    n_inside = steps_inside(p, step, bx0, by0, bz0, bx1, by1, bz1);
                    alive = steps_count > 0;
                }
            }
        }
        if (vr_ballot(alive) != 0) {
            Elem A[8], Bq[8];
#pragma unroll
            for (int k = 0; k < 8; ++k) {
                if constexpr (kLit) {
                    A[k] = vr_f4{0.0f, 0.0f, 0.0f, 0.0f};
                    Bq[k] = vr_f4{0.0f, 0.0f, 0.0f, 0.0f};
                } else {
                    A[k] = 0.0f;
                    Bq[k] = 0.0f;
                }
            }
            float afx = 0.0f, afy = 0.0f, afz = 0.0f, bfx = 0.0f, bfy = 0.0f, bfz = 0.0f;
            f3 pA = p, pB = p;
            int i = 0;
            int n_in_w = wave_min_i32(alive ? min(n_inside, steps_count) : 0x7fffffff);
            P2Win win;
            p2_set_window<V>(win, vol, 0u, WIN ? min(total_slots, L.win_slots) : total_slots);
            unsigned DA = 0, DB = 0;
            float MA = 0.0f, MB = 0.0f;
            float leap_c = 0.0f;
            int lim = 0;
            if constexpr (SKIP) {
                const float vmax = fmaxf(fmaxf(fabsf(step.x) * P0.bsx, fabsf(step.y) * P0.bsy), fabsf(step.z) * P0.bsz);
                leap_c = 0.999f / vmax;
                lim = min(n_inside, steps_count);
            }
            bool idle_a = false, idle_b = false;
            bool idle_ra = false, idle_rb = false;
            int mw = 0;
            auto one_step = [&](Elem (&X)[8], float& xfx, float& xfy, float& xfz, f3& pX, const f3& pY, int jump, bool idle_con, bool idle_rq, unsigned& DX,
                                float& MX) {
                const bool inb = alive;
                const bool sampled = SKIP ? (inb && !idle_con) : inb;
                f3 pN = mk3(pY.x + step.x, pY.y + step.y, pY.z + step.z);
                for (int k = 0; k < jump; ++k) pN = mk3(pN.x + step.x, pN.y + step.y, pN.z + step.z);
                const P2Addr ad = p2_address(vol, L, pN);
                v2f zw = v2f{0.0f, 0.0f}, gxy = zw;
                TfFetch tq;
                float4 mask = make_float4(0.0f, 0.0f, 0.0f, 0.0f);
                float rt = 0.0f;
                bool any_masked = false, masked = false;
                bool shaded = !SKIP || vr_ballot(!idle_con) != 0;
#if VR_P2_DEBUG
                if (shaded) ++dbg_sampled;
#endif
                if (shaded) {
#if VR_P2_DEBUG >= 2
                    const unsigned long long c0 = __builtin_readcyclecounter();
#endif
                    if constexpr (kLit) asm volatile("" : "+v"(X[0]), "+v"(X[1]), "+v"(X[2]), "+v"(X[3]), "+v"(X[4]), "+v"(X[5]), "+v"(X[6]), "+v"(X[7]));
                    else asm volatile("" : "+v"(X[0]), "+v"(X[1]), "+v"(X[2]), "+v"(X[3]), "+v"(X[4]), "+v"(X[5]), "+v"(X[6]), "+v"(X[7]));
#if VR_P2_DEBUG >= 2
                    dbg_wait_corners += __builtin_readcyclecounter() - c0;
#endif
                }
                if (!shaded) {
                } else if constexpr (kLit) {
                    Fetch4 q;
                    q.a = make_float4(X[0].x, X[0].y, X[0].z, X[0].w); q.b = make_float4(X[1].x, X[1].y, X[1].z, X[1].w);
                    q.d = make_float4(X[2].x, X[2].y, X[2].z, X[2].w); q.e = make_float4(X[3].x, X[3].y, X[3].z, X[3].w);
                    q.f = make_float4(X[4].x, X[4].y, X[4].z, X[4].w); q.g = make_float4(X[5].x, X[5].y, X[5].z, X[5].w);
                    q.h = make_float4(X[6].x, X[6].y, X[6].z, X[6].w); q.i = make_float4(X[7].x, X[7].y, X[7].z, X[7].w);
                    zw = interp_zw(q, xfx, xfy, xfz);
                    if constexpr (V == V_VOLUME_MASK) {
                        gxy = interp_xy(q, xfx, xfy, xfz);
                        asm volatile("" : "+v"(zw.x), "+v"(zw.y), "+v"(gxy.x), "+v"(gxy.y));
                        any_masked = vr_ballot(sampled && !(MX <= 0.0f)) != 0;
                        if (any_masked) {
                            mask = tex3_rgba<!WIN>(P0.vol[0], pX);
                            rt = tex3_a<!WIN>(P0.vol[1], pX);
                            asm volatile("" : "+v"(mask.x), "+v"(mask.y), "+v"(mask.z), "+v"(rt));
                            masked = mask.x > 0.0f || mask.y > 0.0f || mask.z > 0.0f;
                        }
                        shaded = p2_vote(P0, sampled, zw.y, masked);
                        if (shaded) tq = tf_fetch_lds(P0.tf[0], zw.y);
                    } else {
                        if constexpr (SKIP) shaded = p2_vote(P0, sampled, zw.y);
                        if (shaded) {
                            tq = tf_fetch_lds(P0.tf[0], zw.y);
                            gxy = interp_xy(q, xfx, xfy, xfz);
                        }
                    }
                } else {
                    Fetch1 q;
                    q.a = X[0]; q.b = X[1]; q.d = X[2]; q.e = X[3]; q.f = X[4]; q.g = X[5]; q.h = X[6]; q.i = X[7];
                    zw.y = interp_a(q, xfx, xfy, xfz);
                    if constexpr (SKIP) shaded = p2_vote(P0, sampled, zw.y);
                    if (shaded) tq = tf_fetch_lds(P0.tf[0], zw.y);
                }
                pX = pN;
                if constexpr (kLit) asm volatile("" : "+v"(zw.x), "+v"(zw.y), "+v"(gxy.x), "+v"(gxy.y));
                else asm volatile("" : "+v"(zw.y));
                __builtin_amdgcn_sched_barrier(0);
                const bool rq = alive && !(SKIP && idle_rq);
                p2_issue<V, SKIP, WIN>(P0, vol, L, win, n_in_w, ad, X, xfx, xfy, xfz, vr_ballot(rq), rq, DX, MX);
                __builtin_amdgcn_sched_barrier(0);
#if VR_P2_DEBUG
                if (shaded) ++dbg_shaded;
#endif
                if (sampled) {
                    if (shaded) {
                        if constexpr (V == V_LIGHT) {
// ... 168 lines not shown
```

volumerendering_amd/csrc/vr_pw.h:

```cpp
#pragma once
#include "vr_kernels.h"
#include <type_traits>

namespace VR_KNS {
using namespace vr;

constexpr int kPwThreads = 1024;
constexpr int kPwHeadStride = 64;

template <int V, bool OFF32, bool SKIP, bool LTF, bool PIPE>
__global__ __launch_bounds__(kPwThreads) void march_pw_kernel(const MarchBatch B, const PwQueue Q)
{
    const MarchParams& P = B.frame[0];
    if constexpr (LTF) {
        const int n = P.tf[0].res_o + 2;
        for (int j = (int)threadIdx.x; j < n; j += kPwThreads) {
            float4 c = P.tf[0].color[j];
            c.w = P.tf[0].opacity[j];
            vr_lds_tf[j] = c;
        }
        __syncthreads();
    }
    const unsigned cls = blockIdx.x & 7u;
    const unsigned groups = (gridDim.x - cls + 7u) >> 3;
    const unsigned wib = (unsigned)__builtin_amdgcn_readfirstlane((int)(threadIdx.x >> 6));
    const unsigned wpb = kPwThreads / 64;
    const unsigned n_c = Q.n_items >> 3;
    unsigned idx = wib * groups + (blockIdx.x >> 3);
    const unsigned cur = cls;
    for (;;) {
        if (idx >= n_c) break;
        const unsigned pos = (idx << 3) | cur;
        int lb = (int)pos;
        if (P.order != nullptr) lb = __builtin_amdgcn_readfirstlane((int)P.order[pos]);
        const unsigned long long t_start = wall_clock64();
        const PixelSlot slot = map_pixel_at(P, lb, 1, 0);
        float4 dst = make_float4(0.0f, 0.0f, 0.0f, 0.0f);
        unsigned blends = 0, covered = 0, fetched = 0;
        march_packet<V, OFF32, SKIP, PIPE ? 2 : (SKIP ? 3 : 0), LTF>(P, slot, dst, blends, covered, fetched);
        if (slot.active || (P.packed && slot.in_launch)) P.out[slot.out_index] = dst;
        store_wave_counts(P, lb, blends, covered, fetched, t_start);
        unsigned r = 0;
        if ((threadIdx.x & 63u) == 0) r = atomicAdd(Q.heads + cur * kPwHeadStride, 1u);
        idx = groups * wpb + (unsigned)__builtin_amdgcn_readfirstlane((int)r);
    }
}


}
```

Baseline: 371.5.

## Pick the launch block order on device instead of host stream waits

The render kernel now chooses which previously sorted block order to use at run time. A device-side order board is published by the sort kernel, and each render wave claims a pick word with a CAS so all waves in a launch agree on the newest order. This replaces host-side hipStreamWaitEvent on older sort events, so the render stream no longer blocks on the order stream. Record slots grow from 8 to 16 so a slot is reused only after more launches have passed. The cost is an extra atomic scan and CAS per wave at kernel start, and the risk of using a stale order or none at all. A diagnostic API reports which order age each launch picked.

```diff
diff --git a/include/vr.h b/include/vr.h
--- a/include/vr.h
+++ b/include/vr.h
@@ -129,6 +129,8 @@
 
 int vr_kernel_times(vr_ctx* ctx, float* out_ms, int capacity);
 
+int vr_launch_orders(vr_ctx* ctx, int* order_age, int* stream_waited, int capacity);
+
 #define VR_TIMING_RECORDS 0
 #define VR_TIMING_EVENTS 1
 int vr_set_kernel_timing(vr_ctx* ctx, int mode);
diff --git a/volumerendering_amd/build.py b/volumerendering_amd/build.py
--- a/volumerendering_amd/build.py
+++ b/volumerendering_amd/build.py
@@ -30,7 +30,7 @@
 
 def build_hip(force: bool = False) -> str:
     target = os.path.join(HERE, "libvr_hip.so")
-    hdrs = [os.path.join(CSRC, f) for f in ("vr_kernels.h", "vr_dp.h", "vr_pw.h", "vr_p2.h", "vr_lt.h", "vr_proj.h", "vr_iso.h", "vr_shadow.h", "vr_device.h", "vr_launch.h")]
+    hdrs = [os.path.join(CSRC, f) for f in ("vr_kernels.h", "vr_dp.h", "vr_pw.h", "vr_p2.h", "vr_lt.h", "vr_proj.h", "vr_iso.h", "vr_shadow.h", "vr_device.h", "vr_launch.h", "vr_order.h")]
     hdrs.append(os.path.join(os.path.dirname(HERE), "include", "vr.h"))
     flags = [f for f in HIP_FLAGS if f != "-shared"] + os.environ.get("VR_EXTRA_HIPCC_FLAGS", "").split()
     stamp = os.path.join(CSRC, ".build_flags")
diff --git a/volumerendering_amd/capi.py b/volumerendering_amd/capi.py
--- a/volumerendering_amd/capi.py
+++ b/volumerendering_amd/capi.py
@@ -31,7 +31,7 @@
     "vr_render_batch_async", "vr_render_tiles_batch_async", "vr_unpack_tiles_strided_async",
     "vr_last_timing", "vr_kernel_times", "vr_reset_kernel_times", "vr_frame_device_ptr", "vr_last_covered_pixels", "vr_last_counters", "vr_set_kernel_flavour", "vr_last_block_trace", "vr_last_kernel_flavour",
     "vr_set_volume_layout", "vr_volume_layout", "vr_viewport", "vr_set_arithmetic", "vr_present_async", "vr_stream", "vr_hint_frames_in_flight",
-    "vr_set_kernel_timing", "vr_present_tiles_async", "vr_kernel_choice",
+    "vr_set_kernel_timing", "vr_launch_orders", "vr_present_tiles_async", "vr_kernel_choice",
     "vr_present_packed_async", "vr_unpack_tiles_bgra8_async",
     "vr_tf_upload_opacity_async", "vr_tf_upload_color_async", "vr_skip_field", "vr_unbounded_box_launches",
     "vr_set_iso_value", "vr_set_shadows", "vr_shadow_volume",
@@ -125,6 +125,7 @@
     lib.vr_hint_frames_in_flight.argtypes = [vp, i32]
     lib.vr_present_packed_async.argtypes = [vp, vp, C.c_int, vp, vp]
     lib.vr_unpack_tiles_bgra8_async.argtypes = [vp, vp, C.c_int, C.c_int, vp, vp]
+    lib.vr_launch_orders.argtypes = [vp, C.POINTER(C.c_int), C.POINTER(C.c_int), C.c_int]
     lib.vr_kernel_choice.argtypes = [vp, C.POINTER(C.c_int), C.POINTER(C.c_float), C.POINTER(C.c_int)]
     lib.vr_stream.argtypes = [vp, i32]
     lib.vr_stream.restype = vp
@@ -295,6 +296,12 @@
         out = np.zeros(capacity, dtype=np.float32)
         n = self._chk(self.lib.vr_kernel_times(self.h, out.ctypes.data, capacity))
         return out[:n].copy()
+
+    def launch_orders(self, capacity: int = 256):
+        age = np.zeros(capacity, dtype=np.int32)
+        waited = np.zeros(capacity, dtype=np.int32)
+        n = self._chk(self.lib.vr_launch_orders(self.h, age.ctypes.data_as(C.POINTER(C.c_int)), waited.ctypes.data_as(C.POINTER(C.c_int)), capacity))
+        return age[:n].copy(), waited[:n].copy()
 
     def reset_kernel_times(self):
         self._chk(self.lib.vr_reset_kernel_times(self.h))
diff --git a/volumerendering_amd/csrc/vr_api.hip b/volumerendering_amd/csrc/vr_api.hip
--- a/volumerendering_amd/csrc/vr_api.hip
+++ b/volumerendering_amd/csrc/vr_api.hip
@@ -34,8 +34,10 @@
 }
 
 constexpr int kInFlight = 8;
+constexpr int kSlots = 16;
+static_assert(kSlots >= kInFlight && vr::kPickRing >= kInFlight, "a slot or a pick word is reused only behind the launches in flight");
 constexpr int kStreams = 4;
-constexpr int kOrderRing = 16;
+using vr::kOrderRing;
 constexpr int kGen = 4;
 constexpr int kStage = 8;
 constexpr int kEditSeen = 8;
@@ -44,7 +46,7 @@
 struct GenBuf {
     void* d = nullptr;
     size_t cap = 0;
-    long long reader[kInFlight];
+    long long reader[kSlots];
     GenBuf() { written(); }
     void written()
     {
@@ -116,12 +118,12 @@
     int last_tiles = 0;
     uint32_t* d_present = nullptr;
     unsigned long long* d_counters = nullptr;
-    unsigned long long* d_block_counts[kInFlight] = {};
-    size_t block_counts_cap[kInFlight] = {};
-    hipEvent_t slot_done[kInFlight] = {};
-    bool slot_used[kInFlight] = {};
+    unsigned long long* d_block_counts[kSlots] = {};
+    size_t block_counts_cap[kSlots] = {};
+    hipEvent_t slot_done[kSlots] = {};
+    bool slot_used[kSlots] = {};
     unsigned* d_pw_heads = nullptr;
-    bool pw_heads_dirty[kInFlight] = {};
+    bool pw_heads_dirty[kSlots] = {};
     struct OrderSlot {
         unsigned* buf = nullptr;
         size_t cap = 0;
@@ -134,6 +136,9 @@
     unsigned long long* h_span = nullptr;
     bool ring_events[kRing] = {};
     unsigned long long* h_end = nullptr;
+    vr::OrderBoard* d_board = nullptr;
+    unsigned* h_pick = nullptr;
+    bool ring_waited[kRing] = {};
     unsigned* h_chain = nullptr;
     struct Tune {
         unsigned long long key = 0;
@@ -642,7 +647,7 @@
 
 int reuse_wait(vr_ctx* c, hipStream_t s, const GenBuf& b)
 {
-    for (int k = 0; k < kInFlight; ++k)
+    for (int k = 0; k < kSlots; ++k)
         if (b.reader[k] >= 0 && (unsigned long long)b.reader[k] + kInFlight >= c->order_seq)
             VR_HIP(c, hipStreamWaitEvent(s, c->slot_done[k], 0));
     return VR_OK;
@@ -667,10 +672,10 @@
     for (int i = 0; i < VR_MAX_TFS; ++i)
         for (int k = 0; k < 2; ++k) {
             GenBuf& b = c->tf_buf[i][k][c->tf_cur[i][k]];
-            if (b.d) b.reader[c->order_seq % kInFlight] = (long long)c->order_seq;
-        }
-    if (P.brick_dist) c->field[c->field_cur].reader[c->order_seq % kInFlight] = (long long)c->order_seq;
-    if (c->shadow_cur >= 0) c->shadow[c->shadow_cur].buf.reader[c->order_seq % kInFlight] = (long long)c->order_seq;
+            if (b.d) b.reader[c->order_seq % kSlots] = (long long)c->order_seq;
+        }
+    if (P.brick_dist) c->field[c->field_cur].reader[c->order_seq % kSlots] = (long long)c->order_seq;
+    if (c->shadow_cur >= 0) c->shadow[c->shadow_cur].buf.reader[c->order_seq % kSlots] = (long long)c->order_seq;
 }
 
 int build_field(vr_ctx* c, hipStream_t s, const float2* rec, const int bn[3], int use_rgb, int zero_prefix, int res_o, unsigned char* field,
@@ -1001,19 +1006,30 @@
     }
 }
 
-int take_record_slot(vr_ctx* c, hipStream_t s, size_t n_records, int* cb, const vr_ctx::OrderSlot** slot_sort)
-{
-    const int k = (int)(c->order_seq % (unsigned long long)kInFlight);
+int take_record_slot(vr_ctx* c, hipStream_t s, size_t n_records, int* cb, bool* waited)
+{
+    const unsigned long long j = c->order_seq;
+    const int k = (int)(j % (unsigned long long)kSlots);
     *cb = k;
-    if (c->slot_used[k]) VR_HIP(c, hipEventSynchronize(c->slot_done[k]));
-    *slot_sort = nullptr;
-    if (c->order_seq >= (unsigned long long)kInFlight) {
-        const vr_ctx::OrderSlot& po = c->order_ring[(c->order_seq - kInFlight) % kOrderRing];
-        if (po.valid && po.seq + kInFlight == c->order_seq) *slot_sort = &po;
+    *waited = false;
+    if (j >= (unsigned long long)kInFlight) {
+        const int kb = (int)((j - kInFlight) % (unsigned long long)kSlots);
+        if (c->slot_used[kb]) VR_HIP(c, hipEventSynchronize(c->slot_done[kb]));
+    }
+    if (j >= (unsigned long long)kSlots) {
+        const vr_ctx::OrderSlot& po = c->order_ring[(j - kSlots) % kOrderRing];
+        if (po.valid && po.seq + kSlots == j) {
+            const hipError_t q = hipEventQuery(po.sorted);
+            if (q == hipErrorNotReady) {
+                (void)hipGetLastError();
+                VR_HIP(c, hipStreamWaitEvent(s, po.sorted, 0));
+                *waited = true;
+            } else {
+                VR_HIP(c, q);
+            }
+        }
     }
     if (n_records > c->block_counts_cap[k]) {
-        if (*slot_sort) VR_HIP(c, hipStreamWaitEvent(s, (*slot_sort)->sorted, 0));
-        *slot_sort = nullptr;
         if (c->d_block_counts[k]) (void)hipFree(c->d_block_counts[k]);
         c->d_block_counts[k] = nullptr;
         c->block_counts_cap[k] = 0;
@@ -1021,25 +1037,6 @@
         VR_HIP(c, hipMemsetAsync(c->d_block_counts[k], 0, n_records * kBlockRecord * sizeof(unsigned long long), s));
         c->block_counts_cap[k] = n_records;
     }
-    return VR_OK;
-}
-
-int wait_for_order(vr_ctx* c, hipStream_t s, bool ordered, unsigned long long okey, const vr_ctx::OrderSlot* slot_sort, const unsigned** order)
-{
-    *order = nullptr;
-    if (ordered) {
-        const vr_ctx::OrderSlot* best = nullptr;
-        const unsigned long long age = (unsigned long long)(c->frames_in_flight + 2 > 3 ? c->frames_in_flight + 2 : 3);
-        for (const auto& o : c->order_ring)
-            if (o.valid && o.key == okey && o.seq + age + 1 >= c->order_seq && o.seq + age <= c->order_seq && (!best || o.seq > best->seq))
-                best = &o;
-        if (best) {
-            VR_HIP(c, hipStreamWaitEvent(s, best->sorted, 0));
-            if (slot_sort && best->seq >= slot_sort->seq) slot_sort = nullptr;
-            *order = best->buf;
-        }
-    }
-    if (slot_sort) VR_HIP(c, hipStreamWaitEvent(s, slot_sort->sorted, 0));
     return VR_OK;
 }
 
@@ -1070,7 +1067,8 @@
                            c->h_chain ? c->h_chain + (c->order_seq % kOrderRing) : (unsigned*)nullptr,
                            (c->h_span && !time_with_events) ? c->h_span + ring : (unsigned long long*)nullptr,
                            pw ? c->d_pw_heads + (size_t)cb * 8 * 64 : (unsigned*)nullptr,
-                           (c->h_span && c->h_end && !time_with_events) ? c->h_end + ring : (unsigned long long*)nullptr);
+                           (c->h_span && c->h_end && !time_with_events) ? c->h_end + ring : (unsigned long long*)nullptr, c->d_board,
+                           c->order_seq, okey, c->h_pick ? c->h_pick + ring : (unsigned*)nullptr);
         VR_HIP(c, hipGetLastError());
         if (pw) c->pw_heads_dirty[cb] = false;
         VR_HIP(c, hipEventRecord(o.sorted, c->order_stream));
@@ -1169,17 +1167,21 @@
         if (n_frames > 1 && grid.x % 8u != 0) return fail(c, VR_ERR_INVALID_ARG, "vr_render: launch shape cannot carry several frames");
         const bool pw = form.family == LaunchDesc::kPw || form.family == LaunchDesc::kP2;
         int cb;
-        const vr_ctx::OrderSlot* slot_sort;
-        if (const int rc = take_record_slot(c, s, (size_t)grid.x * (size_t)n_frames, &cb, &slot_sort)) return rc;
+        bool waited;
+        if (const int rc = take_record_slot(c, s, (size_t)grid.x * (size_t)n_frames, &cb, &waited)) return rc;
         P.block_counts = c->d_block_counts[cb];
         c->cnt_buf = cb;
         const unsigned long long okey = ((unsigned long long)grid.x << 32) ^ ((unsigned long long)block.x << 20) ^
                                         ((unsigned long long)variant << 16) ^ ((unsigned long long)world << 8) ^ (unsigned long long)rank ^
                                         (packed ? 1ull << 63 : 0ull);
         const bool ordered = grid.x <= (unsigned)kOrderMaxBlocks && grid.x % 8u == 0;
-        if (const int rc = wait_for_order(c, s, ordered, okey, slot_sort, &P.order)) return rc;
+        P.board = ordered ? c->d_board : nullptr;
+        P.seq = c->order_seq;
+        P.okey = okey;
 
         const int ring = (int)(c->ring.head % kRing);
+        c->ring_waited[ring] = waited;
+        if (c->h_pick) c->h_pick[ring] = ordered ? 0u : 1u;
         if (frame_events) VR_HIP(c, hipEventRecord(c->tm.ev_k0, s));
         const bool time_with_events = !(ordered && c->h_span) || c->event_timing;
         c->ring_events[ring] = time_with_events;
@@ -1491,8 +1493,8 @@
         if (w > 0 && w <= 0x3fffffffll) c->p2_window = (unsigned)w;
     }
     if (const char* e = getenv("VR_EXP_TUNE")) c->tune_mode = atoi(e);
-    if (!hip_ok(hipMalloc(&c->d_pw_heads, (size_t)kInFlight * 8 * 64 * sizeof(unsigned)), "hipMalloc(queue heads)")) return bail(VR_ERR_HIP);
-    if (!hip_ok(hipMemset(c->d_pw_heads, 0, (size_t)kInFlight * 8 * 64 * sizeof(unsigned)), "hipMemset(queue heads)")) return bail(VR_ERR_HIP);
+    if (!hip_ok(hipMalloc(&c->d_pw_heads, (size_t)kSlots * 8 * 64 * sizeof(unsigned)), "hipMalloc(queue heads)")) return bail(VR_ERR_HIP);
+    if (!hip_ok(hipMemset(c->d_pw_heads, 0, (size_t)kSlots * 8 * 64 * sizeof(unsigned)), "hipMemset(queue heads)")) return bail(VR_ERR_HIP);
     if (!hip_ok(hipEventCreate(&c->tm.ev_begin), "hipEventCreate")) return bail(VR_ERR_HIP);
     if (!hip_ok(hipEventCreate(&c->tm.ev_k0), "hipEventCreate")) return bail(VR_ERR_HIP);
     if (!hip_ok(hipEventCreate(&c->tm.ev_k1), "hipEventCreate")) return bail(VR_ERR_HIP);
@@ -1500,7 +1502,7 @@
     for (int i = 0; i < kRing; ++i)
         if (!hip_ok(hipEventCreate(&c->ring.k0[i]), "hipEventCreate") || !hip_ok(hipEventCreate(&c->ring.k1[i]), "hipEventCreate"))
             return bail(VR_ERR_HIP);
-    for (int i = 0; i < kInFlight; ++i)
+    for (int i = 0; i < kSlots; ++i)
         if (!hip_ok(hipEventCreateWithFlags(&c->slot_done[i], hipEventDisableTiming), "hipEventCreate")) return bail(VR_ERR_HIP);
     for (auto& o : c->order_ring)
         if (!hip_ok(hipEventCreateWithFlags(&o.sorted, hipEventDisableTiming), "hipEventCreate")) return bail(VR_ERR_HIP);
@@ -1520,6 +1522,12 @@
         std::memset(c->h_end, 0, kRing * sizeof(unsigned long long));
     else
         c->h_end = nullptr;
+    if (!hip_ok(hipMalloc((void**)&c->d_board, sizeof(vr::OrderBoard)), "hipMalloc(order board)")) return bail(VR_ERR_HIP);
+    if (!hip_ok(hipMemset(c->d_board, 0, sizeof(vr::OrderBoard)), "hipMemset(order board)")) return bail(VR_ERR_HIP);
+    if (hipHostMalloc((void**)&c->h_pick, kRing * sizeof(unsigned), hipHostMallocDefault) == hipSuccess)
+        std::memset(c->h_pick, 0, kRing * sizeof(unsigned));
+    else
+        c->h_pick = nullptr;
     if (hipHostMalloc((void**)&c->h_chain, kOrderRing * sizeof(unsigned), hipHostMallocDefault) == hipSuccess)
         std::memset(c->h_chain, 0, kOrderRing * sizeof(unsigned));
     else
@@ -1604,6 +1612,8 @@
         if (o.buf) (void)hipFree(o.buf);
     }
     if (c->order_stream) (void)hipStreamDestroy(c->order_stream);
+    if (c->d_board) (void)hipFree(c->d_board);
+    if (c->h_pick) (void)hipHostFree(c->h_pick);
     if (c->h_chain) (void)hipHostFree(c->h_chain);
     if (c->h_span) (void)hipHostFree(c->h_span);
     if (c->h_end) (void)hipHostFree(c->h_end);
@@ -2032,6 +2042,23 @@
         }
         VR_HIP(c, hipEventSynchronize(c->ring.k1[slot]));
         VR_HIP(c, hipEventElapsedTime(&out_ms[i], c->ring.k0[slot], c->ring.k1[slot]));
+    }
+    return n;
+}
+
+int vr_launch_orders(vr_ctx* c, int* order_age, int* stream_waited, int capacity)
+{
+    if (!c) return VR_ERR_INVALID_ARG;
+    if (!order_age || !stream_waited || capacity < 0) return fail(c, VR_ERR_INVALID_ARG, "vr_launch_orders: bad arguments");
+    VR_HIP(c, hipSetDevice(c->device));
+    const long long have = c->ring.head < kRing ? c->ring.head : kRing;
+    const int n = (int)(have < capacity ? have : capacity);
+    if (n > 0) VR_HIP(c, hipStreamSynchronize(c->order_stream));
+    for (int i = 0; i < n; ++i) {
+        const int slot = (int)((c->ring.head - n + i) % kRing);
+        const unsigned v = c->h_pick ? *(volatile unsigned*)&c->h_pick[slot] : 0u;
+        order_age[i] = (int)v - 1;
+        stream_waited[i] = c->ring_waited[slot] ? 1 : 0;
     }
     return n;
 }
diff --git a/volumerendering_amd/csrc/vr_device.h b/volumerendering_amd/csrc/vr_device.h
--- a/volumerendering_amd/csrc/vr_device.h
+++ b/volumerendering_amd/csrc/vr_device.h
@@ -1,6 +1,8 @@
 #pragma once
 #include <hip/hip_runtime.h>
 #include <stdint.h>
+
+#include "vr_order.h"
 
 namespace vr {
 
@@ -76,7 +78,8 @@
     int bnx, bny, bnz;
     float bsx, bsy, bsz;
     int tf_zero_prefix;
-    const unsigned* order;
+    OrderBoard* board;
+    unsigned long long seq, okey;
     float4* out;
     unsigned long long* block_counts;
     unsigned batch_n;
diff --git a/volumerendering_amd/csrc/vr_kernels.h b/volumerendering_amd/csrc/vr_kernels.h
--- a/volumerendering_amd/csrc/vr_kernels.h
+++ b/volumerendering_amd/csrc/vr_kernels.h
@@ -902,11 +902,44 @@
     return n == 1 ? g : (n == 2 ? g >> 1 : (n == 3 ? g / 3u : g >> 2));
 }
 
+struct PickWord {
+    unsigned long long* w;
+    __device__ __forceinline__ unsigned long long load() { return __hip_atomic_load(w, __ATOMIC_RELAXED, __HIP_MEMORY_SCOPE_AGENT); }
+    __device__ __forceinline__ bool cas(unsigned long long& expected, unsigned long long desired)
+    {
+        return __hip_atomic_compare_exchange_strong(w, &expected, desired, __ATOMIC_RELAXED, __ATOMIC_RELAXED, __HIP_MEMORY_SCOPE_AGENT);
+    }
+};
+__device__ __forceinline__ const unsigned* launch_order(const MarchParams& P)
+{
+    if (P.board == nullptr) return nullptr;
+    OrderBoard* const board = P.board;
+    const unsigned long long j = P.seq, key = P.okey;
+    PickWord word{&board->pick[j % (unsigned long long)kPickRing]};
+    unsigned age = 0;
+    if ((threadIdx.x & 63u) == 0u)
+        age = pick_once(word, j, [&]() {
+            return newest_order(
+                j, key, [&](int i) { return __hip_atomic_load(&board->pub[i].seq, __ATOMIC_ACQUIRE, __HIP_MEMORY_SCOPE_AGENT); },
+                [&](int i) { return __hip_atomic_load(&board->pub[i].key, __ATOMIC_RELAXED, __HIP_MEMORY_SCOPE_AGENT); });
+        });
+    age = (unsigned)__builtin_amdgcn_readfirstlane((int)age);
+    if (age == 0u) return nullptr;
+    const unsigned long long buf = __hip_atomic_load(reinterpret_cast<const unsigned long long*>(&board->pub[(j - age) % (unsigned long long)kOrderRing].buf),
+                                                     __ATOMIC_RELAXED, __HIP_MEMORY_SCOPE_AGENT);
+    const unsigned lo = (unsigned)__builtin_amdgcn_readfirstlane((int)(unsigned)buf), hi = (unsigned)__builtin_amdgcn_readfirstlane((int)(unsigned)(buf >> 32));
+    return reinterpret_cast<const unsigned*>(((unsigned long long)hi << 32) | lo);
+}
+__device__ __forceinline__ int order_entry(const unsigned* order, unsigned pos)
+{
+    if (order == nullptr) return (int)pos;
+    return __builtin_amdgcn_readfirstlane((int)__hip_atomic_load(order + pos, __ATOMIC_RELAXED, __HIP_MEMORY_SCOPE_AGENT));
+}
+
 __device__ __forceinline__ int logical_block(const MarchParams& P)
 {
     const unsigned b = (batch_group(blockIdx.x >> 3, P.batch_n) << 3) | (blockIdx.x & 7u);
-    if (P.order == nullptr) return (int)b;
-    return (int)__builtin_amdgcn_readfirstlane((int)P.order[b]);
+    return order_entry(launch_order(P), b);
 }
 
 template <bool BATCH>
@@ -1453,8 +1486,11 @@
                                                             unsigned* __restrict__ order, unsigned* __restrict__ longest_chain,
                                                             unsigned long long* __restrict__ span_ticks,
                                                             unsigned* __restrict__ pw_heads,
-                                                            unsigned long long* __restrict__ end_tick = nullptr)
-{
+                                                            unsigned long long* __restrict__ end_tick, OrderBoard* __restrict__ board,
+                                                            unsigned long long seq, unsigned long long okey, unsigned* __restrict__ picked)
+{
+    if (picked != nullptr && threadIdx.x == 8)
+        *picked = pick_report(__hip_atomic_load(&board->pick[seq % (unsigned long long)kPickRing], __ATOMIC_RELAXED, __HIP_MEMORY_SCOPE_AGENT), seq);
     if (pw_heads != nullptr && threadIdx.x < 8) pw_heads[threadIdx.x * 64] = 0u;
     __shared__ unsigned hist[1024];
     __shared__ unsigned base[1024];
@@ -1518,6 +1554,13 @@
     for (int k = 0; k * 1024 < n_blocks; ++k) {
         const int b = t + k * 1024;
         if (b < n_blocks) order[8u * atomicAdd(&base[bk[k]], 1u) + ((unsigned)b & 7u)] = (unsigned)b;
+    }
+    __syncthreads();
+    if (t == 0) {
+        OrderPub& pub = board->pub[seq % (unsigned long long)kOrderRing];
+        pub.key = okey;
+        pub.buf = order;
+        __hip_atomic_store(&pub.seq, seq, __ATOMIC_RELEASE, __HIP_MEMORY_SCOPE_AGENT);
     }
 }
 
diff --git a/volumerendering_amd/csrc/vr_order.h b/volumerendering_amd/csrc/vr_order.h
--- /dev/null
+++ b/volumerendering_amd/csrc/vr_order.h
@@ -0,0 +1,63 @@
+#pragma once
+
+#if defined(__HIPCC__)
+#define VR_ORDER_HD __host__ __device__
+#else
+#define VR_ORDER_HD
+#endif
+
+namespace vr {
+
+#ifndef VR_ORDER_RING
+#define VR_ORDER_RING 16
+#endif
+constexpr int kOrderRing = VR_ORDER_RING;
+constexpr int kPickRing = 16;
+
+struct OrderPub {
+    unsigned long long seq;
+    unsigned long long key;
+    const unsigned* buf;
+    unsigned long long pad;
+};
+
+struct OrderBoard {
+    OrderPub pub[kOrderRing];
+    unsigned long long pick[kPickRing];
+};
+
+VR_ORDER_HD inline unsigned order_age(unsigned long long j, unsigned long long p)
+{
+    const unsigned long long a = j - p;
+    return (a >= 1ull && a <= (unsigned long long)kOrderRing) ? (unsigned)a : 0u;
+}
+
+constexpr unsigned long long kPickDecided = 0x80ull, kPickAgeMask = 0x7full;
+VR_ORDER_HD inline unsigned long long pick_word(unsigned long long j, unsigned age) { return (j << 8) | kPickDecided | (unsigned long long)age; }
+VR_ORDER_HD inline bool pick_is_of(unsigned long long w, unsigned long long j) { return (w & kPickDecided) != 0ull && (w >> 8) == ((j << 8) >> 8); }
+VR_ORDER_HD inline unsigned pick_age(unsigned long long w) { return (unsigned)(w & kPickAgeMask); }
+
+template <class LoadSeq, class LoadKey>
+VR_ORDER_HD inline unsigned newest_order(unsigned long long j, unsigned long long key, LoadSeq load_seq, LoadKey load_key)
+{
+    unsigned best = 0;
+    for (int i = 0; i < kOrderRing; ++i) {
+        const unsigned a = order_age(j, load_seq(i));
+        if (a != 0u && (best == 0u || a < best) && load_key(i) == key) best = a;
+    }
+    return best;
+}
+
+template <class Word, class Propose>
+VR_ORDER_HD inline unsigned pick_once(Word& w, unsigned long long j, Propose propose)
+{
+    unsigned long long cur = w.load();
+    if (pick_is_of(cur, j)) return pick_age(cur);
+    const unsigned long long mine = pick_word(j, propose());
+    if (w.cas(cur, mine)) return pick_age(mine);
+    return pick_is_of(cur, j) ? pick_age(cur) : 0u;
+}
+
+VR_ORDER_HD inline unsigned pick_report(unsigned long long w, unsigned long long j) { return pick_is_of(w, j) ? 1u + pick_age(w) : 0u; }
+
+}
diff --git a/volumerendering_amd/csrc/vr_p2.h b/volumerendering_amd/csrc/vr_p2.h
--- a/volumerendering_amd/csrc/vr_p2.h
+++ b/volumerendering_amd/csrc/vr_p2.h
@@ -185,6 +185,7 @@
     const MarchParams& P0 = B.frame[0];
     const DevVolume& vol = P0.vol[kSrc];
     P2Lds L;
+    const unsigned* const order = launch_order(P0);
     {
         const unsigned tf_bytes = (unsigned)(P0.tf[0].res_o + 2) * 16u;
         L.off_x = tf_bytes;
@@ -234,8 +235,7 @@
                  light_amb = mk3(P.light_amb[0], P.light_amb[1], P.light_amb[2]);
         const int steps_count = P.steps_count;
         const unsigned pos = (item << 3) | cur;
-        int lb = (int)pos;
-        if (P0.order != nullptr) lb = __builtin_amdgcn_readfirstlane((int)P0.order[pos]);
+        const int lb = order_entry(order, pos);
         const unsigned long long t_start = wall_clock64();
         const PixelSlot slot = map_pixel_at(P0, lb, 1, 0);
         const float bx0 = P.bmin[0], by0 = P.bmin[1], bz0 = P.bmin[2];
diff --git a/volumerendering_amd/csrc/vr_pw.h b/volumerendering_amd/csrc/vr_pw.h
--- a/volumerendering_amd/csrc/vr_pw.h
+++ b/volumerendering_amd/csrc/vr_pw.h
@@ -12,6 +12,7 @@
 __global__ __launch_bounds__(kPwThreads) void march_pw_kernel(const MarchBatch B, const PwQueue Q)
 {
     const MarchParams& P = B.frame[0];
+    const unsigned* const order = launch_order(P);
     if constexpr (LTF) {
         const int n = P.tf[0].res_o + 2;
         for (int j = (int)threadIdx.x; j < n; j += kPwThreads) {
@@ -31,8 +32,7 @@
     for (;;) {
         if (idx >= n_c) break;
         const unsigned pos = (idx << 3) | cur;
-        int lb = (int)pos;
-        if (P.order != nullptr) lb = __builtin_amdgcn_readfirstlane((int)P.order[pos]);
+        const int lb = order_entry(order, pos);
         const unsigned long long t_start = wall_clock64();
         const PixelSlot slot = map_pixel_at(P, lb, 1, 0);
         float4 dst = make_float4(0.0f, 0.0f, 0.0f, 0.0f);
```

Result: slower. 229.8, median of 2 (-38.1%).
